# praateekmahajan/moving-mnist-vae

Measured on AMD Instinct MI355X. Metric: frames/sec/GPU VAE train step, 20×64×64 batch; ELBO vs CPU ref, higher is better.
Workload: dtype bf16; 1 GPU; BASELINE configs[1]: 256 clips x 20 frames x 64x64 per GPU per step (=5120 frames), conv-VAE z=128, Gaussian NLL sigma=0.1 + KL (normal_vae_1_kl_0_mmd), Adam, random-init weights, Bernoulli(0.0521) q=2 labels; parallelism=dp1, rccl_ranks=1, grad_exchange=none, bn=per-rank batch statistics

## Files before the change

### include/mmvae.h

```cpp
#ifndef MMVAE_H_
#define MMVAE_H_

#include <stddef.h>
#include <stdint.h>

#ifdef __cplusplus
extern "C" {
#endif

#if defined(__GNUC__)
#define MMVAE_API __attribute__((visibility("default")))
#else
#define MMVAE_API
#endif

#define MMVAE_OK 0
#define MMVAE_ERR_ARG (-1)
#define MMVAE_ERR_HIP (-2)
#define MMVAE_ERR_WORKSPACE (-3)
#define MMVAE_ERR_UNSUPPORTED (-4)

#define MMVAE_F32 0
#define MMVAE_BF16 1
#define MMVAE_FP8 2
// ... 56 lines not shown
MMVAE_API int mmvae_kl_fwd_ex(const float* mu, const float* logvar, int64_t n, double* acc, double* partials, void* stream);
MMVAE_API int mmvae_kl_bwd(const float* mu, const float* logvar, float coef, const float* gscale, float* d_mu, float* d_logvar, int64_t n,
                 void* stream);
MMVAE_API int mmvae_gauss_nll_fwd(const float* recon, const float* target, int64_t n, float sigma, double* acc, void* stream);
MMVAE_API int mmvae_gauss_nll_fwd_ex(const float* recon, const float* target, int64_t n, float sigma, double* acc, double* partials,
                                     void* stream);
MMVAE_API int mmvae_gauss_nll_bwd(const float* recon, const float* target, int64_t n, float sigma, float coef, const float* gscale,
                        float* d_recon, void* stream);
MMVAE_API int mmvae_ce_fwd(const float* recon, const int64_t* target, const float* weight, int N, int Q, int HW, double* acc, void* stream);
MMVAE_API int mmvae_ce_fwd_ex(const float* recon, const int64_t* target, const float* weight, int N, int Q, int HW, double* acc,
                              double* partials, void* stream);
MMVAE_API int mmvae_ce_bwd(const float* recon, const int64_t* target, const float* weight, int N, int Q, int HW, float coef,
                 const float* gscale, float* d_recon, void* stream);
MMVAE_API int mmvae_mmd_fwd(const float* x, const float* y, int n, int d, float* scratch, double* acc, void* stream);
MMVAE_API int mmvae_mmd_fwd_ex(const float* x, const float* y, int n, int d, float* scratch, double* acc, double* partials, void* stream);
MMVAE_API int mmvae_mmd_bwd(const float* x, const float* y, int n, int d, float coef, const float* gscale, float* d_y, void* stream);
MMVAE_API int mmvae_rbf_kernel(const float* x, const float* y, int n, int m, int d, float* out, void* stream);
MMVAE_API int mmvae_loss_finish(const double* acc, float* out, float nll, float kl_coef, float mmd_coef, float n, void* stream);

MMVAE_API int mmvae_normalise_labels(const int64_t* labels, int64_t n, float mean, float stdv, float* image, void* stream);
MMVAE_API int mmvae_quantise_normalise(const uint8_t* frames, int64_t n, const float* centres, int q, float mean, float stdv,
                             int64_t* labels, float* image, void* stream);
MMVAE_API int mmvae_adam_step(float* params, const float* grads, float* exp_avg, float* exp_avg_sq, int64_t n, float lr, float beta1,
                    float beta2, float eps, float weight_decay, float bc1, float bc2_sqrt, float grad_scale, void* stream);

MMVAE_API int mmvae_adam_step_dev(float* params, const float* grads, float* exp_avg, float* exp_avg_sq, int64_t n, float lr, float beta1,
                        float beta2, float eps, float weight_decay, double* step_dev, float grad_scale, void* stream);

MMVAE_API int mmvae_conv2d_fwd(int dtype, int transposed, const void* x, const float* weight, void* y, int N, int H, int W, int Cin, int Cout,
                     int k, int stride, int pad, const float* pro_scale, const float* pro_shift, int pro_relu, float* stats,
                     void* scratch, void* stream);
MMVAE_API int mmvae_conv2d_dgrad(int dtype, int transposed, const void* dy, const float* weight, void* dx, int N, int H, int W, int Cin,
                       int Cout, int k, int stride, int pad, void* scratch, void* stream);
#define MMVAE_WGRAD_SCRATCH_BYTES (64u << 20)
MMVAE_API int mmvae_conv2d_wgrad(int dtype, int transposed, const void* x, const void* dy, float* dweight, int N, int H, int W, int Cin,
                       int Cout, int k, int stride, int pad, const float* pro_scale, const float* pro_shift, int pro_relu,
                       void* scratch, void* stream);
MMVAE_API int mmvae_conv2d_wgrad_pair(int dtype, const void* x, const void* dy, const void* dy_shortcut, float* dweight, float* dweight_sc, int N,
                            int H, int W, int Cin, int Cout, const float* pro_scale, const float* pro_shift, int pro_relu, void* scratch,
                            void* stream);
#define MMVAE_BN_SCRATCH_BYTES (16u << 20)
MMVAE_API int mmvae_batchnorm_fwd(int dtype, const void* y, int64_t npix, int C, const float* gamma, const float* beta, float* running_mean,
                        float* running_var, int64_t* nbt, float momentum, float eps, int relu, void* out, float* save_mean, float* save_istd,
                        void* scratch, void* stream);
MMVAE_API int mmvae_batchnorm_bwd(int dtype, const void* dout, const void* y, const void* out, int64_t npix, int C, const float* gamma,
                        const float* save_mean, const float* save_istd, void* dy, float* dgamma, float* dbeta, void* scratch, void* stream);
MMVAE_API int mmvae_stem_fwd(int dtype, const void* x, const float* weight, void* y, int N, int S, float* stats, void* scratch, void* stream);
MMVAE_API int mmvae_stem_bwd(int dtype, const void* g, const void* y0, const void* x, const float* weight, const float* gamma,
                   const float* bn_scale, const float* bn_shift, const float* save_mean, const float* save_istd, float* dweight,
                   float* dgamma, float* dbeta, int N, int S, void* scratch, void* stream);
MMVAE_API int mmvae_convT_bwd_fused(int dtype, const void* x, const void* dy, const float* weight, float* dweight, void* dx, int N, int H, int W,
                          int Cin, int Cout, int k, int stride, int pad, const float* pro_scale, const float* pro_shift, int pro_relu,
                          const void* x2, const float* w2, float* dw2, void* scratch, void* wscratch, void* stream);
MMVAE_API int mmvae_tail_join_fwd(int dtype, const void* y2, const float* s2, const float* b2, const void* ys, const float* ss, const float* bs,
                        const float* weight, const float* bias, float* r_raw, float* stats, int N, int H, int W, void* stream);
MMVAE_API int mmvae_tail_join_fwd_stream(int dtype, const void* y2, const float* s2, const float* b2, const void* ys, const float* ss, const float* bs,
                               const float* weight, const float* bias, float* r_raw, float* stats, int N, int H, int W, void* stream);
MMVAE_API int mmvae_tail_join_bwd_reduce(int dtype, const float* d_raw, const float* weight, int out_planes, const void* y2, const float* s2,
                               const float* b2, const void* ys, const float* ss, const float* bs, float* partials, float* wpartials,
                               int N, int H, int W, void* stream);
MMVAE_API int mmvae_tail_join_bwd_apply(int dtype, const float* d_raw, const float* weight, int out_planes, const void* y2, const float* s2,
                              const float* b2, const void* ys, const float* ss, const float* bs, const float* A2, const float* B2,
                              const float* C2, const float* As, const float* Bs, const float* Cs, void* dy2, void* dys, int N, int H, int W,
                              void* stream);
MMVAE_API int mmvae_upblock_bwd_fused(const float* d_raw, const float* tail_weight, const void* y2, const float* s2, const float* b2,
                            const void* ys, const float* ss, const float* bs, const float* A2, const float* B2, const float* C2,
// ... 33 lines not shown
```

### moving-mnist-vae_amd/_lib.py

```python
from __future__ import annotations

import ctypes
import os
from ctypes import POINTER, c_char_p, c_double, c_float, c_int, c_int32, c_int64, c_size_t, c_void_p

_HERE = os.path.dirname(os.path.abspath(__file__))
LIB_PATH = os.environ.get("MMVAE_LIB_PATH") or os.path.join(_HERE, "libmmvae_hip.so")
_lib = None
ABI_VERSION = 3
SUM_PARTIALS = 1025

P = c_void_p

PROTOTYPES = {
    "mmvae_abi_version": (c_int, []),
    "mmvae_last_error": (c_char_p, []),
    "mmvae_net_create": (c_int, [POINTER(c_void_p), c_int, c_int, c_int, c_int, c_int, c_int]),
    "mmvae_net_create_ex": (c_int, [POINTER(c_void_p), c_int, c_int, c_int, c_int, c_int, c_int, c_int]),
    "mmvae_net_destroy": (None, [P]),
    "mmvae_net_sizes": (c_int, [P, POINTER(c_int64), POINTER(c_int64), POINTER(c_int32), POINTER(c_int64), POINTER(c_int32)]),
    "mmvae_net_num_entries": (c_int, [P]),
    "mmvae_net_entry": (c_int, [P, c_int, c_char_p, c_int, POINTER(c_int32), POINTER(c_int32), POINTER(c_int32), POINTER(c_int64)]),
    "mmvae_net_workspace_bytes": (c_size_t, [P, c_int]),
    "mmvae_encoder_fwd": (c_int, [P, c_int, P, P, P, P, P, c_size_t, P, P, c_int, P]),
    "mmvae_net_stage_labels": (c_int, [P, c_int, P, c_int, c_float, c_float, P, P, c_size_t, P]),
    "mmvae_encoder_fwd_staged": (c_int, [P, c_int, P, P, P, P, P, c_size_t, P, P, c_int, P]),
    "mmvae_encoder_bwd": (c_int, [P, c_int, P, P, P, P, P, c_size_t, P]),
    "mmvae_decoder_fwd": (c_int, [P, c_int, P, P, P, P, P, c_size_t, P, c_int, P]),
    "mmvae_decoder_bwd": (c_int, [P, c_int, P, P, P, P, c_size_t, P, P]),
    "mmvae_decoder_bwd_gauss": (c_int, [P, c_int, P, c_float, c_float, P, P, P, P, c_size_t, P, P]),
    "mmvae_net_defer_join": (c_int, [P, c_int]),
    "mmvae_net_join": (c_int, [P, P]),
    "mmvae_net_fork": (P, [P, P]),
    "mmvae_net_side_stream": (P, [P]),
    "mmvae_net_set_join_grad": (c_int, [P, c_int]),
    "mmvae_net_set_sync_bn": (c_int, [P, P, P, c_int]),
    "mmvae_rsample_fwd": (c_int, [P, P, P, P, c_int64, P]),
    "mmvae_rsample_bwd": (c_int, [P, P, P, P, P, c_int64, P]),
    "mmvae_kl_fwd": (c_int, [P, P, c_int64, P, P]),
    "mmvae_kl_fwd_ex": (c_int, [P, P, c_int64, P, P, P]),
    "mmvae_kl_bwd": (c_int, [P, P, c_float, P, P, P, c_int64, P]),
    "mmvae_gauss_nll_fwd": (c_int, [P, P, c_int64, c_float, P, P]),
    "mmvae_gauss_nll_fwd_ex": (c_int, [P, P, c_int64, c_float, P, P, P]),
    "mmvae_gauss_nll_bwd": (c_int, [P, P, c_int64, c_float, c_float, P, P, P]),
    "mmvae_ce_fwd": (c_int, [P, P, P, c_int, c_int, c_int, P, P]),
    "mmvae_ce_fwd_ex": (c_int, [P, P, P, c_int, c_int, c_int, P, P, P]),
    "mmvae_ce_bwd": (c_int, [P, P, P, c_int, c_int, c_int, c_float, P, P, P]),
    "mmvae_mmd_fwd": (c_int, [P, P, c_int, c_int, P, P, P]),
    "mmvae_mmd_fwd_ex": (c_int, [P, P, c_int, c_int, P, P, P, P]),
    "mmvae_mmd_bwd": (c_int, [P, P, c_int, c_int, c_float, P, P, P]),
    "mmvae_loss_finish": (c_int, [P, P, c_float, c_float, c_float, c_float, P]),
    "mmvae_normalise_labels": (c_int, [P, c_int64, c_float, c_float, P, P]),
    "mmvae_quantise_normalise": (c_int, [P, c_int64, P, c_int, c_float, c_float, P, P, P]),
    "mmvae_adam_step": (c_int, [P, P, P, P, c_int64, c_float, c_float, c_float, c_float, c_float, c_float, c_float, c_float, P]),
    "mmvae_adam_step_dev": (c_int, [P, P, P, P, c_int64, c_float, c_float, c_float, c_float, c_float, P, c_float, P]),
    "mmvae_conv2d_fwd": (c_int, [c_int, c_int, P, P, P, c_int, c_int, c_int, c_int, c_int, c_int, c_int, c_int, P, P, c_int, P, P, P]),
    "mmvae_conv2d_dgrad": (c_int, [c_int, c_int, P, P, P, c_int, c_int, c_int, c_int, c_int, c_int, c_int, c_int, P, P]),
    "mmvae_conv2d_wgrad": (c_int, [c_int, c_int, P, P, P, c_int, c_int, c_int, c_int, c_int, c_int, c_int, c_int, P, P, c_int, P, P]),
    "mmvae_conv2d_wgrad_pair": (c_int, [c_int, P, P, P, P, P, c_int, c_int, c_int, c_int, c_int, P, P, c_int, P, P]),
    "mmvae_rbf_kernel": (c_int, [P, P, c_int, c_int, c_int, P, P]),
    "mmvae_comm_unique_id": (c_int, [P]),
    "mmvae_comm_init": (c_int, [POINTER(c_void_p), c_int, c_int, P]),
    "mmvae_comm_allreduce": (c_int, [P, P, c_int64, P]),
    "mmvae_comm_destroy": (c_int, [P]),
    "mmvae_net_set_sync_bn_comm": (c_int, [P, P]),
    "mmvae_net_set_sync_bn_comm2": (c_int, [P, P, P]),
    "mmvae_convT_bwd_fused": (c_int, [c_int, P, P, P, P, P, c_int, c_int, c_int, c_int, c_int, c_int, c_int, c_int, P, P, c_int, P, P, P, P, P, P]),
    "mmvae_batchnorm_fwd": (c_int, [c_int, P, c_int64, c_int, P, P, P, P, P, c_float, c_float, c_int, P, P, P, P, P]),
    "mmvae_batchnorm_bwd": (c_int, [c_int, P, P, P, c_int64, c_int, P, P, P, P, P, P, P, P]),
    "mmvae_stem_fwd": (c_int, [c_int, P, P, P, c_int, c_int, P, P, P]),
    "mmvae_stem_bwd": (c_int, [c_int, P, P, P, P, P, P, P, P, P, P, P, P, c_int, c_int, P, P]),
    "mmvae_tail_join_fwd": (c_int, [c_int, P, P, P, P, P, P, P, P, P, P, c_int, c_int, c_int, P]),
    "mmvae_tail_join_fwd_stream": (c_int, [c_int, P, P, P, P, P, P, P, P, P, P, c_int, c_int, c_int, P]),
    "mmvae_tail_join_bwd_reduce": (c_int, [c_int, P, P, c_int, P, P, P, P, P, P, P, P, c_int, c_int, c_int, P]),
    "mmvae_tail_join_bwd_apply": (c_int, [c_int, P, P, c_int, P, P, P, P, P, P, P, P, P, P, P, P, P, P, c_int, c_int, c_int, P]),
    "mmvae_upblock_bwd_fused": (c_int, [P] * 27 + [c_int, P, P]),
    "mmvae_join_conv1x1_fwd": (c_int, [P, P, P, P, P, P, P, c_int, P, P, P, c_int64, P, P]),
    "mmvae_conv1x1_bwd_fused": (c_int, [P] * 13 + [c_int64, P, P]),
    "mmvae_upblock_tail_fwd": (c_int, [P] * 16 + [c_int, P, P]),
    "mmvae_pixelcnn_create": (c_int, [POINTER(c_void_p), c_int, c_int, c_int, c_int, c_int]),
    "mmvae_pixelcnn_destroy": (None, [P]),
    "mmvae_pixelcnn_num_params": (c_int64, [P]),
    "mmvae_pixelcnn_workspace_bytes": (c_size_t, [P, c_int, c_int]),
    "mmvae_pixelcnn_fwd": (c_int, [P, c_int, c_int, P, P, P, c_size_t, P, P]),
    "mmvae_pixelcnn_bwd": (c_int, [P, c_int, c_int, P, P, P, P, P, c_size_t, P, P]),
    "mmvae_pixelcnn_sample_workspace_bytes": (c_size_t, [P, c_int, c_int]),
    "mmvae_pixelcnn_sample": (c_int, [P, c_int, c_int, P, c_int, P, c_int, P, c_float, c_float, P, P, c_size_t, P, P, P, P]),
    "mmvae_convert": (c_int, [c_int, c_int, P, P, c_int64, P]),
}

# ... 52 lines not shown
```

### moving-mnist-vae_amd/csrc/capi.cpp

```cpp
#include <cstring>
#include <new>

#include "../../include/mmvae.h"
#include "conv_ops.hpp"
#include "pixel_net.hpp"
#include "vae_net.hpp"

namespace mmvae { const char* last_error(); }
using namespace mmvae;

struct mmvae_net { Net* net; };
struct mmvae_comm { Comm* c; };

static inline hipStream_t S(void* s) { return static_cast<hipStream_t>(s); }
static inline hipStream_t S_(void* s) { return static_cast<hipStream_t>(s); }

extern "C" {

int mmvae_abi_version(void) { return MMVAE_ABI_VERSION; }
const char* mmvae_last_error(void) { return last_error(); }

int mmvae_net_create(mmvae_net** out, int in_channels, int z, int out_channels, int image_size, int need_logvar, int dtype) {
  return mmvae_net_create_ex(out, in_channels, z, out_channels, image_size, need_logvar, dtype, 1);
}
// ... 290 lines not shown
    q.wfrag = op_deep2_down_ok(dt, g, H, W);
    if (w) { int rc = op_pack_down(dt, g, w, scratch, S(st), 1.f, 0, q.wfrag); if (rc < 0) return rc; }
    return op_run_down(dt, dt, g, scratch, N, x, H, W, y, Ho, Wo, ps, pb, relu, stats, 0, S(st), q);
  }
  if (convT4_stream_ok(dt, Cin, Cout, k, s, p, H, W)) {
    if (w) { int rc = op_pack_up(dt, g, w, scratch, S(st)); if (rc < 0) return rc; }
    return launch_convT4_stream(dt, x, scratch, y, ps, pb, relu, stats, N, H, S(st));
  }
  q.wfrag = op_deep2_up_ok(dt, g, Ho, Wo);
  if (w) { int rc = op_pack_up(dt, g, w, scratch, S(st), 1.f, 0, q.wfrag); if (rc < 0) return rc; }
  return op_run_up(dt, g, scratch, N, x, H, W, y, Ho, Wo, ps, pb, relu, stats, 0, S(st), q);
}
int mmvae_conv2d_dgrad(int dt, int transposed, const void* dy, const float* w, void* dx, int N, int H, int W, int Cin, int Cout, int k,
                       int s, int p, void* scratch, void* st) {
  const ConvGeom g = geom_for(transposed, Cin, Cout, k, s, p);
  const int Ho = out_size(transposed, H, k, s, p), Wo = out_size(transposed, W, k, s, p);
  SecondSrc q;
  if (!transposed && s == 1 && conv3_stream_ok(dt, Cin, Cout, k, s, p, H, W)) {
    PackArgs pf; std::memset(&pf, 0, sizeof(pf));
    pf.src = w; pf.dst = scratch; pf.cols = Cin; pf.K = Cout; pf.ntaps = 9; pf.s_col = 9; pf.s_k = Cin * 9; pf.scale = 1.f;
    for (int t = 0; t < 9; ++t) pf.tap_off[t] = 8 - t;
    int rc = launch_pack(dt, pf, S(st)); if (rc < 0) return rc;
    rc = launch_conv3_stream(dt, 1, dy, scratch, nullptr, dx, nullptr, nullptr, nullptr, 0, nullptr, nullptr, N, H, S(st));
    return rc < 0 ? rc : MMVAE_OK;
  }
  if (!transposed) {
    q.wfrag = op_deep2_up_ok(dt, g, H, W);
    int rc = op_pack_up(dt, g, w, scratch, S(st), 1.f, 0, q.wfrag); if (rc < 0) return rc;
    return op_run_up(dt, g, scratch, N, dy, Ho, Wo, dx, H, W, nullptr, nullptr, 0, nullptr, 0, S(st), q);
  }
  q.wfrag = op_deep2_down_ok(dt, g, Ho, Wo);
  int rc = op_pack_down(dt, g, w, scratch, S(st), 1.f, 0, q.wfrag); if (rc < 0) return rc;
  return op_run_down(dt, dt, g, scratch, N, dy, Ho, Wo, dx, H, W, nullptr, nullptr, 0, nullptr, 0, S(st), q);
}
int mmvae_conv2d_wgrad(int dt, int transposed, const void* x, const void* dy, float* dw, int N, int H, int W, int Cin, int Cout, int k,
                       int s, int p, const float* ps, const float* pb, int relu, void* scratch, void* st) {
  const ConvGeom g = geom_for(transposed, Cin, Cout, k, s, p);
  const int Ho = out_size(transposed, H, k, s, p), Wo = out_size(transposed, W, k, s, p);
  if (!scratch) { set_error("conv2d_wgrad: scratch (MMVAE_WGRAD_SCRATCH_BYTES) required"); return MMVAE_ERR_ARG; }
  static_assert(MMVAE_WGRAD_SCRATCH_BYTES == kWgradScratchBytes, "public scratch size out of sync");
  float* sc = static_cast<float*>(scratch);
  if (!transposed) return op_run_wgrad(dt, g, N, dy, Ho, Wo, nullptr, nullptr, 0, x, H, W, ps, pb, relu, dw, S(st), sc);
  return op_run_wgrad(dt, g, N, x, H, W, ps, pb, relu, dy, Ho, Wo, nullptr, nullptr, 0, dw, S(st), sc);
}
int mmvae_conv2d_wgrad_pair(int dt, const void* x, const void* dy, const void* dy_sc, float* dw, float* dw_sc, int N, int H, int W, int Cin, int Cout,
                            const float* ps, const float* pb, int relu, void* scratch, void* st) {
  if (!scratch || !x || !dy || !dy_sc || !dw || !dw_sc || N < 1) { set_error("conv2d_wgrad_pair: bad argument"); return MMVAE_ERR_ARG; }
  const ConvGeom g = geom_for(0, Cin, Cout, 3, 2, 1), gs = geom_for(0, Cin, Cout, 1, 2, 0);
  const int Ho = out_size(0, H, 3, 2, 1), Wo = out_size(0, W, 3, 2, 1);
  const int rc = op_run_wgrad_pair(dt, g, gs, N, dy, dy_sc, Ho, Wo, x, H, W, ps, pb, relu, dw, dw_sc, S(st), static_cast<float*>(scratch), 1.f, 1.f);
  if (rc == 0) { set_error("conv2d_wgrad_pair: shape not supported (bf16, 32 -> 32 channels, 32x32 -> 16x16)"); return MMVAE_ERR_UNSUPPORTED; }
  return rc < 0 ? rc : MMVAE_OK;
}
int mmvae_convT_bwd_fused(int dt, const void* x, const void* dy, const float* w, float* dw, void* dx, int N, int H, int W, int Cin, int Cout, int k,
                          int s, int p, const float* ps, const float* pb, int relu, const void* x2, const float* w2, float* dw2, void* scratch,
                          void* wscratch, void* st) {
  const ConvGeom g = geom_for(1, Cin, Cout, k, s, p);
  const int Ho = out_size(1, H, k, s, p), Wo = out_size(1, W, k, s, p);
  if (!scratch || !wscratch) { set_error("convT_bwd_fused: scratch buffers required"); return MMVAE_ERR_ARG; }
  if (!op_bwd_fusable(dt, g, N, H, W, Ho, Wo)) { set_error("convT_bwd_fused: shape not supported (bf16, 16 / 32 -> 16 channels, k4 s2 p1, 32x32 -> 64x64 or 16x16 -> 32x32)"); return MMVAE_ERR_UNSUPPORTED; }
  char* sc = static_cast<char*>(scratch);
  int rc = op_pack_down(dt, g, w, sc, S(st)); if (rc < 0) return rc;
  const void* w2p = nullptr;
  if (x2 && w2) {
    PackArgs pa; std::memset(&pa, 0, sizeof(pa));
    pa.src = w2; pa.dst = sc + (size_t)Cin * Cout * k * k * dtype_size(dt); pa.cols = Cin; pa.K = 16; pa.ntaps = 1; pa.s_col = 16; pa.s_k = 1; pa.scale = 1.f; pa.tap_off[0] = 0;
// ... 163 lines not shown
```

### moving-mnist-vae_amd/csrc/conv_deep2.inc

```
#include "kernels.hpp"
#include "tile_common.hpp"

namespace mmvae {

template <typename T, typename TO, int NPT, int CPT, bool ACC, bool LITE, bool F8 = false>
__device__ __forceinline__ void deep2_conv_body(const DeepArgs& a) {
  static_assert(!F8 || (sizeof(T) == 2 && !ACC), "fp8 MFMA: bf16 storage, forward convolutions");
  constexpr int VE = Elem<T>::kVec;
  constexpr int ES = sizeof(T);
  constexpr int TPX = NPT * 16;
  constexpr int kSV = 8;
  constexpr int G = CPT < (LITE ? 2 : 4) ? CPT : (LITE ? 2 : 4);
  constexpr int NB = LITE ? 2 : NPT >= 8 ? 3 : 4;
  constexpr int UPT = CPT / G;
  extern __shared__ __attribute__((aligned(16))) char smem[];
  const int t = threadIdx.x, nthr = blockDim.x, lane = t & 63, wv = __builtin_amdgcn_readfirstlane(t >> 6), gq = lane >> 4, r = lane & 15;
  const int c0 = (blockIdx.y * a.nw + wv) * 32;
  const int cin_vecs = a.Cin / VE;
  constexpr int LES = F8 ? 1 : ES;
  const int pitch = F8 ? a.Cin + 16 : a.Cin * ES + 32;
  const int npix_in = a.ipt * a.Hi * a.Wi;
  char* sPatch = smem;
  unsigned* sOpix = reinterpret_cast<unsigned*>(sPatch + (size_t)(npix_in + 1) * pitch);
  float* sStat = reinterpret_cast<float*>(sOpix + TPX) + wv * 64;
  unsigned short* sTab = reinterpret_cast<unsigned short*>(sOpix + TPX + 64 * a.nw);
  const T* __restrict__ X = reinterpret_cast<const T*>(a.x);
  TO* __restrict__ Y = reinterpret_cast<TO*>(a.y);
  const bool has_pro = a.pro_scale != nullptr, has_bias = a.bias != nullptr, has_stats = a.stats != nullptr;
  const float relu_lo = a.pro_relu ? 0.f : -__builtin_inff();
  const int HqWq = a.Hq * a.Wq;

  const int cv = t % cin_vecs, pix0 = t / cin_vecs, PS = nthr / cin_vecs;
  for (int p = t; p < TPX; p += nthr) {
    unsigned o = ~0u;
    int img = 0, hq = 0, wq = 0;
    const bool live = p < a.ipt * HqWq;
    if (live) {
      img = p / HqWq;
      const int rem = p - img * HqWq;
      hq = rem / a.Wq; wq = rem - hq * a.Wq;
      o = ((unsigned)img << 16) | ((unsigned)hq << 8) | (unsigned)wq;
    }
    sOpix[p] = o;
    const int hb = hq * a.SI, wb = wq * a.SI, ib = img * a.Hi;
#pragma unroll
    for (int tap = 0; tap < kMaxTaps; ++tap)
      if (tap < a.ntaps_all) {
        const int hi = hb + a.taps[tap].dh, wi = wb + a.taps[tap].dw;
        const bool in = live && hi >= 0 && hi < a.Hi && wi >= 0 && wi < a.Wi;
        sTab[tap * TPX + p] = (unsigned short)(in ? (ib + hi) * a.Wi + wi : npix_in);
      }
  }
  for (int i = t; i < pitch / 16; i += nthr) reinterpret_cast<Vec16*>(sPatch + (size_t)npix_in * pitch)[i] = Vec16{{0, 0, 0, 0}};
  sStat[lane] = 0.f;

  for (int tile = blockIdx.x; tile < a.ntiles; tile += gridDim.x) {
    const int n0 = tile * a.ipt;
    const int nimg = min(a.ipt, a.N - n0);
    __syncthreads();
    {
      const T* src = X + (long)n0 * a.Hi * a.Wi * a.Cin + cv * VE;
      const int nvalid = nimg * a.Hi * a.Wi;
      float psc[VE], psh[VE];
// ... 86 lines not shown
#pragma unroll
            for (int pt = 0; pt < NPT; ++pt) bf[pt] = *reinterpret_cast<const Vec16*>(sPatch + pb[pt] + (cc0 + g) * 64);
#pragma unroll
            for (int pt = 0; pt < NPT; ++pt) {
              acc[0][pt] = mma_vec<T>(buf[g][0], bf[pt], acc[0][pt]);
              acc[1][pt] = mma_vec<T>(buf[g][1], bf[pt], acc[1][pt]);
            }
          }
        }
      };
      Vec16 buf[NB][G][2];
      unsigned pb[NPT];
#pragma unroll
      for (int b = 0; b < NB - 1; ++b) load_unit(buf[b], b);
      for (int u = 0; u < nunits; u += NB) {
#pragma unroll
        for (int b = 0; b < NB; ++b) {
          const int uu = u + b;
          load_unit(buf[(b + NB - 1) % NB], uu + NB - 1);
          __builtin_amdgcn_sched_barrier(0);
          if (uu < nunits) {
            if (UPT == 1 || (uu & (UPT - 1)) == 0) tap_pixels(pb, uu / UPT);
            mul_unit(buf[b], pb, (uu & (UPT - 1)) * G);
          }
          __builtin_amdgcn_sched_barrier(0);
        }
      }
      float bv[8], st1[8], st2[8];
#pragma unroll
      for (int j = 0; j < 8; ++j) {
        bv[j] = has_bias ? a.bias[c0 + 8 * gq + j] : 0.f;
        st1[j] = 0.f; st2[j] = 0.f;
      }
#pragma unroll
      for (int pt = 0; pt < NPT; ++pt) {
        const unsigned op = sOpix[pt * 16 + r];
        const int img = (int)(op >> 16), hq = (int)((op >> 8) & 255u), wq = (int)(op & 255u);
        if (op != ~0u && img < nimg && hq < P.Hq && wq < P.Wq) {
          const unsigned ob = ((((unsigned)(n0 + img) * a.Ho + (unsigned)(hq * a.SO + P.ph)) * a.Wo + (unsigned)(wq * a.SO + P.pw)) * (unsigned)a.Cout) +
                              (unsigned)(c0 + 8 * gq);
          float v[8];
#pragma unroll
          for (int j = 0; j < 8; ++j) v[j] = acc[j >> 2][pt][j & 3] + bv[j];
#pragma unroll
          for (int j = 0; j < 8; ++j) { st1[j] += v[j]; st2[j] += v[j] * v[j]; }
          dstore8<TO>(Y + ob, v, ACC);
        }
      }
      if (has_stats) {
#pragma unroll
        for (int j = 0; j < 8; ++j) { st1[j] = row16_sum(st1[j]); st2[j] = row16_sum(st2[j]); }
        if (r == 0) {
#pragma unroll
          for (int j = 0; j < 8; ++j) {
            sStat[8 * gq + j] += st1[j];
            sStat[32 + 8 * gq + j] += st2[j];
          }
        }
      }
    }
  }
  if (has_stats) {
    a.stats[(long)blockIdx.x * 2 * a.Cout + (long)(lane >> 5) * a.Cout + c0 + (lane & 31)] = sStat[lane];
  }
}

template <typename T, typename TO, int NPT, int CPT, bool ACC>
__global__ __launch_bounds__(512, 2) void deep2_conv_kernel(DeepArgs a) { deep2_conv_body<T, TO, NPT, CPT, ACC, false>(a); }
template <typename T, typename TO, int NPT, int CPT, bool ACC>
__global__ __launch_bounds__(512, 3) void deep2_conv_lite_kernel(DeepArgs a) { deep2_conv_body<T, TO, NPT, CPT, ACC, true>(a); }
template <typename T, typename TO, int NPT, int CPT, bool ACC>
__global__ __launch_bounds__(512, 2) void deep2_conv_f8_kernel(DeepArgs a) { deep2_conv_body<T, TO, NPT, CPT, false, false, true>(a); }
template <typename T, typename TO, int NPT, int CPT, bool ACC>
__global__ __launch_bounds__(512, 3) void deep2_conv_f8_lite_kernel(DeepArgs a) { deep2_conv_body<T, TO, NPT, CPT, false, true, true>(a); }

template <typename T, typename TO>
static int launch_deep2_t(const DeepArgs& a, int dt, int gx, hipStream_t s) {
  const size_t lds = deep2_conv_lds_bytes(a, dt);
  dim3 grid(gx, a.Cout / (32 * a.nw)), block(64 * a.nw);
#define MMVAE_D2K(K_, N_, C_, A_) do { \
    static bool attr_set = false; \
    if (!attr_set) { \
      const hipError_t e = hipFuncSetAttribute(reinterpret_cast<const void*>(&K_<T, TO, N_, C_, A_>), hipFuncAttributeMaxDynamicSharedMemorySize, 160 * 1024); \
      if (e != hipSuccess) { set_error("deep2_conv: hipFuncSetAttribute: %s", hipGetErrorString(e)); return MMVAE_ERR_HIP; } \
      attr_set = true; \
    } \
    hipLaunchKernelGGL((K_<T, TO, N_, C_, A_>), grid, block, lds, s, a); } while (0)
#define MMVAE_D2(N_, C_, A_) do { if (a.nw >= 4) MMVAE_D2K(deep2_conv_lite_kernel, N_, C_, A_); else MMVAE_D2K(deep2_conv_kernel, N_, C_, A_); } while (0)
#define MMVAE_D2C(N_, C_) do { if (a.accumulate) MMVAE_D2(N_, C_, true); else MMVAE_D2(N_, C_, false); } while (0)
#define MMVAE_D2N(N_) do { \
    constexpr int kC0 = sizeof(T) == 2 ? 1 : 2;       \
    if (cpt == kC0) MMVAE_D2C(N_, kC0); else if (cpt == 2 * kC0) MMVAE_D2C(N_, 2 * kC0); else if (cpt == 4 * kC0) MMVAE_D2C(N_, 4 * kC0); \
    else if (cpt == 8 * kC0) MMVAE_D2C(N_, 8 * kC0); \
    else { set_error("deep2_conv: Cin=%d unsupported", a.Cin); return MMVAE_ERR_UNSUPPORTED; } } while (0)
  const int cpt = 1 << a.cpt_log2;
  if (a.fp8) {
    if constexpr (sizeof(T) == 2 && sizeof(TO) == 2) {
      if (a.accumulate || !a.wfrag) { set_error("deep2_conv: fp8 needs fragment-major weights and no accumulate"); return MMVAE_ERR_UNSUPPORTED; }
#define MMVAE_D2F(N_, C_) do { if (a.nw >= 4 && N_ < 8) MMVAE_D2K(deep2_conv_f8_lite_kernel, N_, C_, false); else MMVAE_D2K(deep2_conv_f8_kernel, N_, C_, false); } while (0)
#define MMVAE_D2FN(N_) do { if (cpt == 1) MMVAE_D2F(N_, 1); else if (cpt == 2) MMVAE_D2F(N_, 2); else if (cpt == 4) MMVAE_D2F(N_, 4); \
      else { set_error("deep2_conv: fp8 Cin=%d unsupported", a.Cin); return MMVAE_ERR_UNSUPPORTED; } } while (0)
      if (a.npt == 8) MMVAE_D2FN(8); else if (a.npt == 4) MMVAE_D2FN(4); else if (a.npt == 2) MMVAE_D2FN(2);
      else { set_error("deep2_conv: npt=%d unsupported", a.npt); return MMVAE_ERR_UNSUPPORTED; }
#undef MMVAE_D2FN
#undef MMVAE_D2F
      const int rc8 = check_launch("deep2_conv_f8");
      return rc8 ? rc8 : gx;
    } else { set_error("deep2_conv: fp8 needs bf16 storage"); return MMVAE_ERR_UNSUPPORTED; }
  }
  if (a.npt == 8) MMVAE_D2N(8);
  else if (a.npt == 4) MMVAE_D2N(4);
  else if (a.npt == 2) MMVAE_D2N(2);
  else { set_error("deep2_conv: npt=%d unsupported", a.npt); return MMVAE_ERR_UNSUPPORTED; }
#undef MMVAE_D2N
#undef MMVAE_D2C
#undef MMVAE_D2
#undef MMVAE_D2K
  const int rc = check_launch("deep2_conv");
  return rc ? rc : gx;
}

// ... 10 lines not shown
```

### moving-mnist-vae_amd/csrc/conv_gemm.hip

```cpp
#include <stdlib.h>
#include <string.h>

#include <vector>

#include "kernels.hpp"

namespace mmvae {

constexpr int KV = 8;

__device__ __forceinline__ int lds_slot(int row, int kv) { return row * KV + (kv ^ ((row >> 1) & 7)); }

template <typename T> struct Mma;
template <> struct Mma<bf16_t> {
  __device__ static __forceinline__ f32x4 run(const Vec16& a, const Vec16& b, f32x4 c) {
    return __builtin_amdgcn_mfma_f32_16x16x32_bf16(__builtin_bit_cast(bf16x8, a), __builtin_bit_cast(bf16x8, b), c, 0, 0, 0);
  }
};
template <> struct Mma<float> {
  __device__ static __forceinline__ f32x4 run(const Vec16& a, const Vec16& b, f32x4 c) {
#pragma unroll
    for (int j = 0; j < 4; ++j)
      c = __builtin_amdgcn_mfma_f32_16x16x4f32(__uint_as_float(a.w[j]), __uint_as_float(b.w[j]), c, 0, 0, 0);
    return c;
// ... 327 lines not shown
  gx = 256 * occ;
  if (gx > b.g.ntiles) gx = b.g.ntiles;
  if (gx > kGatherMaxGridX) gx = kGatherMaxGridX;
  if (gx >= 8) gx &= ~7;
  b.x_bytes = a.x_planar ? 0u : (unsigned)((long)a.N * a.Hi * a.Wi * a.Cin * (long)dtype_size(dt));
  if (a.x2) {
    if (ct16 > 2) return 0;
    patch_conv_x2_carve(b, dt);
    if (occ > 2 && ct16 == 1 && slots <= 4) { occ = occ_regs - 1 > 1 ? occ_regs - 1 : 1; gx = 256 * occ; if (gx > b.g.ntiles) gx = b.g.ntiles; if (gx > kGatherMaxGridX) gx = kGatherMaxGridX; if (gx >= 8) gx &= ~7; }
  }
  return launch_patch_conv(dt, out_dt, b, gx, s);
}

static size_t deep2_lds_for(int dt, int Cin, int Cout, int hw, int HiWi, int ntaps_all, int npt, int fp8 = 0) {
  DeepArgs b; memset(&b, 0, sizeof(b));
  b.fp8 = fp8;
  b.Cin = Cin; b.Hi = HiWi; b.Wi = 1; b.ipt = npt * 16 / hw; b.npt = npt; b.ntaps_all = ntaps_all; b.nw = Cout / 32 < 8 ? Cout / 32 : 8;
  return deep2_conv_lds_bytes(b, dt);
}
bool deep2_shape_ok(int dt, int Cin, int Cout, int Hq, int Wq, int Hi, int Wi, int ntaps_all, int fp8) {
  if (fp8 && dt != DT_BF16) return false;
  const int ES = fp8 ? 1 : dt == DT_F32 ? 4 : 2;
  const int cpt = Cin * ES / 64;
  const int c0 = ES == 4 ? 2 : 1;
  if (Cin < (fp8 ? 64 : 32) || (Cin * ES) % 64 != 0 || (cpt != c0 && cpt != 2 * c0 && cpt != 4 * c0 && cpt != 8 * c0)) return false;
  if (Cout < 32 || Cout % 32 != 0 || (Cout > 256 && Cout % 256 != 0)) return false;
  if (Cin < 64 && Cout < 64) return false;
  const int hw = Hq * Wq;
  if (hw < 1 || hw > 128 || Hq > 255 || Wq > 255 || ntaps_all < 1 || ntaps_all > kMaxTaps) return false;
  const int npt_min = hw > 64 ? 8 : hw > 32 ? 4 : 2;
  if (fp8 && cpt > 4) return false;
  return deep2_lds_for(dt, Cin, Cout, hw, Hi * Wi, ntaps_all, npt_min, fp8) <= 150 * 1024;
}
static int try_deep2(int dt, int out_dt, const GatherArgs& a, hipStream_t s) {
  if (a.x_planar || a.y_planes || a.x2) return 0;
  if (a.fp8 && (!a.wfrag || a.accumulate || dt != DT_BF16 || out_dt != DT_BF16)) return 0;
  int Hq = 0, Wq = 0, ntaps_all = 0;
  for (int p = 0; p < a.nphase; ++p) {
    const Phase& ph = a.phases[p];
    if (ph.ntaps <= 0) return 0;
    Hq = ph.Hq > Hq ? ph.Hq : Hq; Wq = ph.Wq > Wq ? ph.Wq : Wq;
    ntaps_all = ph.tap0 + ph.ntaps > ntaps_all ? ph.tap0 + ph.ntaps : ntaps_all;
  }
  if (!deep2_shape_ok(dt, a.Cin, a.Cout, Hq, Wq, a.Hi, a.Wi, ntaps_all, a.fp8)) return 0;
  if ((long)a.N * a.Ho * a.Wo * a.Cout >= (1L << 32)) return 0;
  const int ES = dt == DT_F32 ? 4 : 2, VE = 16 / ES;
  const int cpt = a.Cin * (a.fp8 ? 1 : ES) / 64;
  DeepArgs b; memset(&b, 0, sizeof(b));
  b.fp8 = a.fp8;
  b.x = a.x; b.w = a.w; b.y = a.y; b.pro_scale = a.pro_scale; b.pro_shift = a.pro_shift; b.pro_relu = a.pro_relu;
  b.bias = a.bias; b.stats = a.stats; b.accumulate = a.accumulate; b.wfrag = a.wfrag;
  b.N = a.N; b.Hi = a.Hi; b.Wi = a.Wi; b.Cin = a.Cin; b.Ho = a.Ho; b.Wo = a.Wo; b.Cout = a.Cout; b.SI = a.SI; b.SO = a.SO;
  b.nphase = a.nphase; b.Hq = Hq; b.Wq = Wq; b.ntaps_all = ntaps_all;
  for (int p = 0; p < a.nphase; ++p) {
    const Phase& ph = a.phases[p];
    b.phases[p] = DeepPhase{ph.ph, ph.pw, ph.Hq, ph.Wq, ph.ntaps, ph.tap0, ph.w_off};
  }
  for (int t = 0; t < kMaxTaps; ++t) b.taps[t] = a.taps[t];
  for (b.cpt_log2 = 0; (1 << b.cpt_log2) < cpt; ++b.cpt_log2) {}
  b.nw = a.Cout / 32 < 8 ? a.Cout / 32 : 8;
  if ((64 * b.nw) % (a.Cin / VE) != 0) return 0;
  const int gy = a.Cout / (32 * b.nw);
  const int hw = Hq * Wq;
  int best = 0;
  for (int pass = 0; pass < 2 && !best; ++pass)
    for (int npt = 8; npt >= 2 && !best; npt >>= 1) {
      if (hw > npt * 16) break;
      const size_t lds = deep2_lds_for(dt, a.Cin, a.Cout, hw, a.Hi * a.Wi, ntaps_all, npt, a.fp8);
      int ipt = npt * 16 / hw; if (ipt > a.N) ipt = a.N;
      const long ntiles = (a.N + ipt - 1) / ipt;
      if (pass == 0) {
        if (lds > 80 * 1024) continue;
        if (npt > 2 && ntiles * gy * b.nw < 256 * 4) continue;
      } else if (lds > 150 * 1024) continue;
      best = npt;
    }
  if (!best) return 0;
  b.npt = best; b.ipt = best * 16 / hw;
  if (b.ipt > a.N) b.ipt = a.N;
  b.ntiles = (a.N + b.ipt - 1) / b.ipt;
  int gx = b.ntiles < kGatherMaxGridX ? b.ntiles : kGatherMaxGridX;
  return launch_deep2_conv(dt, out_dt, b, gx, s);
}

static int try_pos(int dt, int out_dt, const GatherArgs& a, hipStream_t s) {
  if (dt != DT_BF16 || out_dt != DT_BF16 || !a.wfrag || a.fp8 || a.gup == 0) return 0;
  if (a.x_planar || a.y_planes || a.x2 || a.bias || a.Hi != a.Wi || a.Ho != a.Wo || a.Cout % 32 != 0) return 0;
  const int up = a.gup == 2 ? 1 : 0;
  if (!pos_conv_takes(a.gk, a.gs, a.gp, up, a.Hi, a.Ho, a.Cin)) return 0;
  if (up && a.gs > 1 && a.gk < a.gs && !a.accumulate) return 0;
  if (a.Hi >= 8 && a.Cout < 128) return 0;
  if ((long)a.N * a.Ho * a.Wo * a.Cout >= (1L << 32)) return 0;
  PosArgs b; memset(&b, 0, sizeof(b));
  b.x = a.x; b.w = a.w; b.y = a.y; b.pro_scale = a.pro_scale; b.pro_shift = a.pro_shift; b.pro_relu = a.pro_relu;
  b.stats = a.stats; b.accumulate = a.accumulate; b.N = a.N; b.Cout = a.Cout;
  b.nw = a.Cout / 32 < 8 ? a.Cout / 32 : 8;
  if ((a.Cout / 32) % b.nw != 0 || (64 * b.nw) % (a.Cin / 8) != 0) return 0;
  return launch_pos_conv(a.gk, a.gs, a.gp, up, a.Hi, a.Ho, a.Cin, b, s);
}

static int launch_x2_separately(int dt, int out_dt, const GatherArgs& a, hipStream_t s) {
  GatherArgs b; memset(&b, 0, sizeof(b));
  int Hq = 0, Wq = 0;
  for (int p = 0; p < a.nphase; ++p) if (a.phases[p].ph == a.x2_ph && a.phases[p].pw == a.x2_pw) { Hq = a.phases[p].Hq; Wq = a.phases[p].Wq; }
  if (Hq <= 0) { set_error("gather_gemm: the second source's phase (%d,%d) is not part of the launch", a.x2_ph, a.x2_pw); return MMVAE_ERR_ARG; }
  b.x = a.x2; b.w = a.w2; b.y = a.y; b.accumulate = 1; b.wfrag = a.wfrag2;
  b.N = a.N; b.Hi = Hq; b.Wi = Wq; b.Cin = a.Cin2; b.Ho = a.Ho; b.Wo = a.Wo; b.Cout = a.Cout; b.SI = 1; b.SO = a.SO;
  b.nphase = 1; b.phases[0] = Phase{a.x2_ph, a.x2_pw, Hq, Wq, 1, 0, 0}; b.taps[0] = Tap{0, 0};
  b.gk = 1; b.gs = a.SO; b.gp = 0; b.gup = 2;
  return launch_gather_gemm(dt, out_dt, b, s);
}

int launch_gather_gemm(int dt, int out_dt, GatherArgs a, hipStream_t s) {
  const int VE = dt == DT_F32 ? 4 : 8;
  note_launch_bytes((double)a.N * ((double)a.Hi * a.Wi * (a.x_planar ? a.x_planes : a.Cin) * (a.x_planar == 1 ? 4 : dtype_size(dt)) +
                                   (double)a.Ho * a.Wo * (a.y_planes > 0 ? a.y_planes : a.Cout) * (a.y_planes > 0 ? 4 : dtype_size(out_dt)) +
                                   (a.x2 ? (double)a.phases[0].Hq * a.phases[0].Wq * a.Cin2 * dtype_size(dt) : 0.0)));
  if (a.fp8) {
    if (dt != DT_BF16 || out_dt != DT_BF16 || a.x2 || a.accumulate) { set_error("gather_gemm: fp8 needs the bf16 forward path"); return MMVAE_ERR_UNSUPPORTED; }
    a.cin_vecs = a.Cin / VE;
    const int rc2 = try_deep2(dt, out_dt, a, s);
    if (rc2 != 0) return rc2;
    if (a.wfrag) { set_error("gather_gemm: fragment-major fp8 weights (Cin=%d Cout=%d) need the deep2 kernel", a.Cin, a.Cout); return MMVAE_ERR_UNSUPPORTED; }
    set_error("gather_gemm: fp8 layer Cin=%d Cout=%d is not eligible for the deep-layer kernel", a.Cin, a.Cout); return MMVAE_ERR_UNSUPPORTED;
  }
  if (a.x2) {
    int rc = (!a.wfrag && !a.wfrag2) ? try_patch(dt, out_dt, a, s) : 0;
    if (rc != 0) return rc;
    GatherArgs m = a; m.x2 = nullptr; m.w2 = nullptr; m.Cin2 = 0; m.wfrag2 = 0;
    rc = launch_gather_gemm(dt, out_dt, m, s);
    if (rc < 0) return rc;
    const int rc2 = launch_x2_separately(dt, out_dt, a, s);
    return rc2 < 0 ? rc2 : rc;
  }
  if (a.Cin % VE != 0 || a.Cout % 4 != 0 || a.nphase < 1 || a.nphase > kMaxPhases) {
    set_error("gather_gemm: unsupported Cin=%d Cout=%d nphase=%d", a.Cin, a.Cout, a.nphase);
    return MMVAE_ERR_UNSUPPORTED;
  }
  if (a.pro_scale && a.Cin > 512) { set_error("gather_gemm: prologue needs Cin<=512"); return MMVAE_ERR_UNSUPPORTED; }
  a.cin_vecs = a.Cin / VE;
  int max_tiles = 0, ntap = 0;
  for (int p = 0; p < a.nphase; ++p) {
    const long M = (long)a.N * a.phases[p].Hq * a.phases[p].Wq;
    if (M > 0x7fffffffL / 2) { set_error("gather_gemm: too many pixels"); return MMVAE_ERR_UNSUPPORTED; }
    const int tiles = (int)((M + 127) / 128);
    if (tiles > max_tiles) max_tiles = tiles;
    ntap += a.phases[p].ntaps;
  }
  if (ntap > kMaxTaps) { set_error("gather_gemm: %d taps > %d", ntap, kMaxTaps); return MMVAE_ERR_UNSUPPORTED; }
  if (max_tiles <= 0) return 1;
  const int rcp = a.wfrag ? 0 : try_patch(dt, out_dt, a, s);
  if (rcp != 0) return rcp;
  const int rcq = try_pos(dt, out_dt, a, s);
  if (rcq != 0) return rcq;
  const int rcd2 = try_deep2(dt, out_dt, a, s);
  if (rcd2 != 0) return rcd2;
  if (a.wfrag) { set_error("gather_gemm: fragment-major weights (Cin=%d Cout=%d) need the deep2 kernel, which does not take this launch", a.Cin, a.Cout); return MMVAE_ERR_UNSUPPORTED; }
  {
    constexpr int g3_maxk = 160;
    int maxk = 0;
    for (int p = 0; p < a.nphase; ++p) if (a.phases[p].ntaps * a.Cin > maxk) maxk = a.phases[p].ntaps * a.Cin;
    const bool fits32 = (long)a.N * a.Hi * a.Wi * a.Cin < (1L << 31) && (long)a.N * a.Ho * a.Wo * a.Cout < (1L << 31);
    if (!a.x_planar && !a.y_planes && !a.bias && out_dt == dt && a.Cout <= 64 && maxk <= g3_maxk && fits32) {
      int ct16 = (a.Cout + 15) / 16; if (ct16 == 3) ct16 = 4;
      if (gather3_lds_bytes(a, dt, ct16 * 16) <= kV2MaxLds) {
        long wt = 0;
        for (int p = 0; p < a.nphase; ++p) { const long m = (long)a.N * a.phases[p].Hq * a.phases[p].Wq; if ((m + 31) / 32 > wt) wt = (m + 31) / 32; }
        long gx3 = (wt + 3) / 4; if (gx3 > 2048 / a.nphase) gx3 = 2048 / a.nphase; if (gx3 < 1) gx3 = 1;
        if (gx3 > kGatherMaxGridX) gx3 = kGatherMaxGridX;
        return launch_gather3(dt, out_dt, a, (int)gx3, s);
      }
    }
    if (a.x_planar || a.y_planes) { set_error("gather_gemm: planar boundary layouts need the patch-tile kernel"); return MMVAE_ERR_UNSUPPORTED; }
  }
  const int gx = max_tiles < kGatherMaxGridX ? max_tiles : kGatherMaxGridX;
  if (dt == DT_F32) return launch_gather_t<float, float>(a, gx, s);
  if (out_dt == DT_F32) return launch_gather_t<bf16_t, float>(a, gx, s);
  return launch_gather_t<bf16_t, bf16_t>(a, gx, s);
}

template <typename T>
__global__ __launch_bounds__(256) void wgrad_kernel(WgradArgs a) {
  constexpr int VE = Elem<T>::kVec;
  constexpr int PK = KV * VE;
  __shared__ Vec16 sP[64 * KV];
  __shared__ Vec16 sG[256 * KV];
  __shared__ int sPix[PK * 3];
  __shared__ float sProP[2 * 256];
  __shared__ float sProG[2 * 256];
// ... 364 lines not shown
```

### moving-mnist-vae_amd/csrc/conv_ops.cpp

```cpp
#include "conv_ops.hpp"

#include <cstdlib>
#include <cstring>

namespace mmvae {

#define MM_TRY(expr)            \
  do {                          \
    int rc__ = (expr);          \
    if (rc__ < 0) return rc__;  \
  } while (0)

struct UpPhase { int ph, pw; int ntaps; int kh[16], kw[16], dh[16], dw[16]; };
static int up_phases(int k, int s, int p, UpPhase* out) {
  int n = 0;
  for (int ph = 0; ph < s; ++ph)
    for (int pw = 0; pw < s; ++pw) {
      UpPhase& u = out[n++];
      u.ph = ph; u.pw = pw; u.ntaps = 0;
      for (int kh = 0; kh < k; ++kh) {
        const int th = ph + p - kh;
        if (((th % s) + s) % s != 0) continue;
        for (int kw = 0; kw < k; ++kw) {
          const int tw = pw + p - kw;
// ... 32 lines not shown
    a.cols = g.D1; a.K = g.D0; a.ntaps = ph[i].ntaps; a.s_col = kk; a.s_k = g.D1 * kk; a.scale = scale; a.fp8 = fp8; a.frag = frag;
    for (int t = 0; t < ph[i].ntaps; ++t) a.tap_off[t] = ph[i].kh[t] * g.k + ph[i].kw[t];
    MM_TRY(launch_pack(dt, a, s));
    off += (long)g.D1 * ph[i].ntaps * g.D0;
  }
  return MMVAE_OK;
}

int op_deep2_down_ok(int dt, const ConvGeom& g, int Hl, int Wl, int fp8) {
  const int Hs = conv_down_size(Hl, g.k, g.s, g.p), Ws = conv_down_size(Wl, g.k, g.s, g.p);
  return deep2_shape_ok(dt, g.D1, g.D0, Hs, Ws, Hl, Wl, g.k * g.k, fp8) ? 1 : 0;
}
int op_deep2_up_ok(int dt, const ConvGeom& g, int Hl, int Wl, int allow_empty_phases, int fp8) {
  if (g.s > 2 || g.k * g.k > kMaxTaps) return 0;
  const int Hs = conv_down_size(Hl, g.k, g.s, g.p), Ws = conv_down_size(Wl, g.k, g.s, g.p);
  UpPhase ph[4];
  const int np = up_phases(g.k, g.s, g.p, ph);
  int ntaps = 0;
  for (int i = 0; i < np; ++i) { if (ph[i].ntaps == 0 && !allow_empty_phases) return 0; ntaps += ph[i].ntaps; }
  return deep2_shape_ok(dt, g.D0, g.D1, (Hl + g.s - 1) / g.s, (Wl + g.s - 1) / g.s, Hs, Ws, ntaps, fp8) ? 1 : 0;
}
bool op_pos_fwd_takes(const ConvGeom& g, int Hl, bool transposed) {
  const int Hs = conv_down_size(Hl, g.k, g.s, g.p);
  const int Hi = transposed ? Hs : Hl, Ho = transposed ? Hl : Hs;
  const int Cin = transposed ? g.D0 : g.D1, Cout = transposed ? g.D1 : g.D0;
  if (Cout % 32 != 0 || Cin % 8 != 0 || (Hi >= 8 && Cout < 128)) return false;
  if (transposed && g.s > 1 && g.k < g.s) return false;
  const int nw = Cout / 32 < 8 ? Cout / 32 : 8;
  if ((Cout / 32) % nw != 0 || (64 * nw) % (Cin / 8) != 0) return false;
  return pos_conv_takes(g.k, g.s, g.p, transposed ? 1 : 0, Hi, Ho, Cin);
}

int op_run_down(int dt, int out_dt, const ConvGeom& g, const void* packed, int N, const void* L, int Hl, int Wl, void* S, int Hs, int Ws,
                const float* pro_s, const float* pro_b, int relu, float* stats, int accumulate, hipStream_t s, const SecondSrc& x2) {
  GatherArgs a; std::memset(&a, 0, sizeof(a));
  if (g.k * g.k > kMaxTaps) { set_error("run_down: k=%d too large", g.k); return MMVAE_ERR_UNSUPPORTED; }
  if (x2.x2) { a.x2 = x2.x2; a.w2 = x2.w2; a.Cin2 = x2.Cin2; a.x2_ph = 0; a.x2_pw = 0; }
  a.fp8 = x2.fp8; a.wfrag = x2.wfrag; a.wfrag2 = x2.wfrag2;
  a.x = L; a.w = packed; a.y = S;
  a.pro_scale = pro_s; a.pro_shift = pro_b; a.pro_relu = relu; a.stats = stats; a.accumulate = accumulate;
  a.N = N; a.Hi = Hl; a.Wi = Wl; a.Cin = g.D1; a.Ho = Hs; a.Wo = Ws; a.Cout = g.D0; a.SI = g.s; a.SO = 1;
  a.gk = g.k; a.gs = g.s; a.gp = g.p; a.gup = 1;
  a.nphase = 1;
  a.phases[0] = Phase{0, 0, Hs, Ws, g.k * g.k, 0, 0};
  for (int kh = 0; kh < g.k; ++kh)
    for (int kw = 0; kw < g.k; ++kw) a.taps[kh * g.k + kw] = Tap{kh - g.p, kw - g.p};
  return launch_gather_gemm(dt, out_dt, a, s);
}

int op_run_up(int dt, const ConvGeom& g, const void* packed, int N, const void* S, int Hs, int Ws, void* L, int Hl, int Wl,
              const float* pro_s, const float* pro_b, int relu, float* stats, int accumulate, hipStream_t s, const SecondSrc& x2) {
  if (g.s > 2 || g.k * g.k > kMaxTaps) { set_error("run_up: k=%d s=%d unsupported", g.k, g.s); return MMVAE_ERR_UNSUPPORTED; }
  GatherArgs a; std::memset(&a, 0, sizeof(a));
  if (x2.x2) { a.x2 = x2.x2; a.w2 = x2.w2; a.Cin2 = x2.Cin2; a.x2_ph = 0; a.x2_pw = 0; }
  a.fp8 = x2.fp8; a.wfrag = x2.wfrag; a.wfrag2 = x2.wfrag2;
  a.x = S; a.w = packed; a.y = L;
  a.pro_scale = pro_s; a.pro_shift = pro_b; a.pro_relu = relu; a.stats = stats; a.accumulate = accumulate;
  a.N = N; a.Hi = Hs; a.Wi = Ws; a.Cin = g.D0; a.Ho = Hl; a.Wo = Wl; a.Cout = g.D1; a.SI = 1; a.SO = g.s;
  a.gk = g.k; a.gs = g.s; a.gp = g.p; a.gup = 2;
  UpPhase ph[4];
  const int np = up_phases(g.k, g.s, g.p, ph);
  long off = 0; int tap0 = 0; a.nphase = 0;
  for (int i = 0; i < np; ++i) {
    const int Hq = Hl > ph[i].ph ? (Hl - ph[i].ph + g.s - 1) / g.s : 0;
    const int Wq = Wl > ph[i].pw ? (Wl - ph[i].pw + g.s - 1) / g.s : 0;
    const bool skip = (ph[i].ntaps == 0 && accumulate) || Hq == 0 || Wq == 0;
    if (!skip) {
      a.phases[a.nphase++] = Phase{ph[i].ph, ph[i].pw, Hq, Wq, ph[i].ntaps, tap0, off};
      for (int t = 0; t < ph[i].ntaps; ++t) a.taps[tap0 + t] = Tap{ph[i].dh[t], ph[i].dw[t]};
      tap0 += ph[i].ntaps;
    }
    off += (long)g.D1 * ph[i].ntaps * g.D0;
  }
  if (a.nphase == 0) return 1;
  return launch_gather_gemm(dt, dt, a, s);
}

int op_run_wgrad(int dt, const ConvGeom& g, int N, const void* P, int Hs, int Ws, const float* proP_s, const float* proP_b, int proP_relu,
                 const void* G, int Hl, int Wl, const float* proG_s, const float* proG_b, int proG_relu, float* dW, hipStream_t s,
                 float* scratch, float scale, WgradReduceArgs* defer) {
  WgradArgs a; std::memset(&a, 0, sizeof(a));
  const int kk = g.k * g.k;
  if (kk > 25) { set_error("wgrad: k=%d too large", g.k); return MMVAE_ERR_UNSUPPORTED; }
  if (defer) defer->nparts = 0;
  a.P = P; a.G = G; a.dW = dW; a.scratch = scratch; a.defer = defer;
  a.proP_scale = proP_s; a.proP_shift = proP_b; a.proP_relu = proP_relu;
  a.proG_scale = proG_s; a.proG_shift = proG_b; a.proG_relu = proG_relu;
  a.N = N; a.Hp = Hs; a.Wp = Ws; a.Ca = g.D0; a.Hg = Hl; a.Wg = Wl; a.Cb = g.D1; a.Cb_valid = g.D1;
  a.stride = g.s; a.pad = g.p; a.ksz = g.k; a.sA = g.D1 * kk; a.sB = kk; a.ntaps = kk; a.scale = scale;
  for (int t = 0; t < kk; ++t) a.tap_off[t] = t;
  return launch_wgrad(dt, a, s);
}

static void wgrad_args(WgradArgs& a, const ConvGeom& g, int N, const void* P, int Hs, int Ws, const float* proP_s, const float* proP_b, int proP_relu,
                       const void* G, int Hl, int Wl, const float* proG_s, const float* proG_b, int proG_relu, float* dW, float* scratch, float scale) {
  std::memset(&a, 0, sizeof(a));
  const int kk = g.k * g.k;
  a.P = P; a.G = G; a.dW = dW; a.scratch = scratch;
  a.proP_scale = proP_s; a.proP_shift = proP_b; a.proP_relu = proP_relu;
  a.proG_scale = proG_s; a.proG_shift = proG_b; a.proG_relu = proG_relu;
  a.N = N; a.Hp = Hs; a.Wp = Ws; a.Ca = g.D0; a.Hg = Hl; a.Wg = Wl; a.Cb = g.D1; a.Cb_valid = g.D1; a.Ca_valid = g.D0;
  a.stride = g.s; a.pad = g.p; a.ksz = g.k; a.sA = g.D1 * kk; a.sB = kk; a.ntaps = kk; a.scale = scale;
  for (int t = 0; t < kk && t < 25; ++t) a.tap_off[t] = t;
}

int op_run_wgrad_pair(int dt, const ConvGeom& g, const ConvGeom& gs, int N, const void* P, const void* P2, int Hs, int Ws, const void* G, int Hl, int Wl,
                      const float* proG_s, const float* proG_b, int proG_relu, float* dW, float* dW2, hipStream_t s, float* scratch, float scale,
                      float scale2) {
// ... 43 lines not shown
```

### moving-mnist-vae_amd/csrc/conv_ops.hpp

```cpp
#pragma once
#include "kernels.hpp"

namespace mmvae {

struct ConvGeom { int D0, D1, k, s, p; };

inline int conv_down_size(int H, int k, int s, int p) { return (H + 2 * p - k) / s + 1; }
int op_pack_down(int dt, const ConvGeom& g, const float* w, void* dst, hipStream_t s, float scale = 1.f, int fp8 = 0, int frag = 0);
int op_pack_up(int dt, const ConvGeom& g, const float* w, void* dst, hipStream_t s, float scale = 1.f, int fp8 = 0, int frag = 0);
int op_deep2_down_ok(int dt, const ConvGeom& g, int Hl, int Wl, int fp8 = 0);
int op_deep2_up_ok(int dt, const ConvGeom& g, int Hl, int Wl, int allow_empty_phases = 0, int fp8 = 0);
struct SecondSrc {
  const void* x2 = nullptr; const void* w2 = nullptr; int Cin2 = 0;
  int fp8 = 0;
  int wfrag = 0, wfrag2 = 0;
};
int op_run_down(int dt, int out_dt, const ConvGeom& g, const void* packed, int N, const void* L, int Hl, int Wl, void* S, int Hs, int Ws,
                const float* pro_s, const float* pro_b, int relu, float* stats, int accumulate, hipStream_t s, const SecondSrc& x2 = SecondSrc());
int op_run_up(int dt, const ConvGeom& g, const void* packed, int N, const void* S, int Hs, int Ws, void* L, int Hl, int Wl,
              const float* pro_s, const float* pro_b, int relu, float* stats, int accumulate, hipStream_t s, const SecondSrc& x2 = SecondSrc());
int op_run_wgrad(int dt, const ConvGeom& g, int N, const void* P, int Hs, int Ws, const float* proP_s, const float* proP_b, int proP_relu,
                 const void* G, int Hl, int Wl, const float* proG_s, const float* proG_b, int proG_relu, float* dW, hipStream_t s,
                 float* scratch = nullptr, float scale = 1.f, WgradReduceArgs* defer = nullptr);
bool op_wgrad_is_stream(int dt, const ConvGeom& g, int N, int Hs, int Ws, int Hl, int Wl, bool proP, bool proG);
int op_run_wgrad_pair(int dt, const ConvGeom& g, const ConvGeom& gs, int N, const void* P, const void* P2, int Hs, int Ws, const void* G, int Hl, int Wl,
                      const float* proG_s, const float* proG_b, int proG_relu, float* dW, float* dW2, hipStream_t s, float* scratch, float scale,
                      float scale2);

bool op_pos_fwd_takes(const ConvGeom& g, int Hl, bool transposed);
bool op_bwd_fusable(int dt, const ConvGeom& g, int N, int Hs, int Ws, int Hl, int Wl);
int op_run_bwd_fused(int dt, const ConvGeom& g, int N, const void* P, int Hs, int Ws, const float* proP_s, const float* proP_b, int proP_relu,
                     const void* G, int Hl, int Wl, const void* packed_down, void* dP, const void* x2, const void* w2_packed, float* dW,
                     hipStream_t s, float* scratch, float scale = 1.f, float* bn_part = nullptr, float* dW2 = nullptr, float scale2 = 1.f,
                     const JoinGrad* jg = nullptr);
bool op_bwd_fusable_jg(int dt, const ConvGeom& g, int N, int Hs, int Ws, int Hl, int Wl, bool proP, bool has_x2, bool bn_sums);

}
```

### moving-mnist-vae_amd/csrc/conv_pos.inc

```
#include <type_traits>
#include <utility>

#include "kernels.hpp"
#include "tile_common.hpp"

namespace mmvae {

template <int I0, int I1, typename F>
__device__ __forceinline__ void static_for(F&& f) {
  if constexpr (I0 < I1) {
    f(std::integral_constant<int, I0>{});
    static_for<I0 + 1, I1>(f);
  }
}

template <int K, int S, int P, bool UP>
struct PosTaps {
  static constexpr bool hit(int ph, int k) { return !UP || (((ph + P - k) % S) + S) % S == 0; }
  static constexpr int count(int ph) { int n = 0; for (int k = 0; k < K; ++k) if (hit(ph, k)) ++n; return n; }
  static constexpr int kth(int ph, int i) { int n = 0; for (int k = 0; k < K; ++k) if (hit(ph, k)) { if (n == i) return k; ++n; } return -1; }
  static constexpr int delta(int ph, int k) { return UP ? (ph + P - k) / S : k - P; }
  static constexpr int taps_before(int pi) { int n = 0; for (int q = 0; q < pi; ++q) n += count(q / (UP ? S : 1)) * count(q % (UP ? S : 1)); return n; }
};

// ... 1 lines not shown
template <int K, int S, int P, bool UP, int HI, int HO, int CIN, int IG, int PI>
struct PosPlan {
  using TP = PosTaps<K, S, P, UP>;
  static constexpr int NPH1 = UP ? S : 1, ph = PI / NPH1, pw = PI % NPH1;
  static constexpr int HQ = UP ? HO / S : HO, NPOS = HQ * HQ, NCF = NPOS * IG, CPT = CIN / 32;
  static constexpr int SI = UP ? 1 : S;
  static constexpr int NTH = TP::count(ph), NTW = TP::count(pw), NT = NTH * NTW, NU = NT * CPT;
  static constexpr int pix(int tap, int pos) {
    const int kh = TP::kth(ph, tap / NTW), kw = TP::kth(pw, tap % NTW);
    const int hi = (pos / HQ) * SI + TP::delta(ph, kh), wi = (pos % HQ) * SI + TP::delta(pw, kw);
    return (hi >= 0 && hi < HI && wi >= 0 && wi < HI) ? hi * HI + wi : -1;
  }
  static constexpr int count_items() {
    int n = 0;
    for (int tap = 0; tap < NT; ++tap) for (int pos = 0; pos < NPOS; ++pos) if (pix(tap, pos) >= 0) n += IG * CPT;
    return n;
  }
  static constexpr int W = count_items();
  struct Tab { PosItem it[W > 0 ? W : 1]; };
  static constexpr Tab make() {
    Tab t{};
    int n = 0;
    for (int u = 0; u < NU; ++u)
      for (int cf = 0; cf < NCF; ++cf) {
        const int px = pix(u / CPT, cf / IG);
        if (px >= 0) { t.it[n].u = (short)u; t.it[n].cf = (short)cf; t.it[n].off = px * CIN * 2 + (u % CPT) * 64; ++n; }
      }
    return t;
  }
  static constexpr Tab tab = make();
  static constexpr int first_of(int u) { for (int w = 0; w < W; ++w) if (tab.it[w].u >= u) return w; return W; }
};

template <int K, int S, int P, bool UP, int HI, int HO, int CIN, int IG, int NB, int RB>
__global__ __launch_bounds__(512, 2) void pos_conv_kernel(PosArgs a) {
  using TP = PosTaps<K, S, P, UP>;
  constexpr int NPH1 = UP ? S : 1;
  constexpr int HQ = UP ? HO / S : HO;
  constexpr int NPOS = HQ * HQ, NCF = NPOS * IG, CPT = CIN / 32, IPT = 16 * IG;
  constexpr int SO = UP ? S : 1;
  constexpr int IMGB = HI * HI * CIN * 2, IP = IMGB + 32;
  constexpr int CV = CIN / 8, VPI = HI * HI * CV;
  static_assert(NCF <= 16 && CIN % 32 == 0 && (UP ? HO % S == 0 : true), "pos_conv: geometry");
  static_assert(IMGB < 65536, "pos_conv: ds_read immediate range");
  extern __shared__ __attribute__((aligned(16))) char smem[];
  const int t = threadIdx.x, nthr = blockDim.x, lane = t & 63, wv = __builtin_amdgcn_readfirstlane(t >> 6), gq = lane >> 4, r = lane & 15;
  const int nw = nthr >> 6;
  const int c0 = (blockIdx.y * nw + wv) * 32;
  char* sPatch = smem;
  float* sStat = reinterpret_cast<float*>(smem + IPT * IP) + wv * 64;
  const bf16_t* __restrict__ X = reinterpret_cast<const bf16_t*>(a.x);
  bf16_t* __restrict__ Y = reinterpret_cast<bf16_t*>(a.y);
  const bool has_pro = a.pro_scale != nullptr, has_stats = a.stats != nullptr, accum = a.accumulate != 0;
  const float relu_lo = a.pro_relu ? 0.f : -__builtin_inff();
  const char* lb[IG];
#pragma unroll
  for (int ig = 0; ig < IG; ++ig) lb[ig] = sPatch + (ig * 16 + r) * IP + gq * 16;
  sStat[lane] = 0.f;

  for (int tile = blockIdx.x; tile < a.ntiles; tile += gridDim.x) {
    const int n0 = tile * IPT;
    const int nimg = min(IPT, a.N - n0);
    __syncthreads();
    {
      const int cv = t % CV;
      float psc[8], psh[8];
#pragma unroll
      for (int j = 0; j < 8; j += 4) {
        const float4 sc = has_pro ? *reinterpret_cast<const float4*>(a.pro_scale + cv * 8 + j) : make_float4(1.f, 1.f, 1.f, 1.f);
        const float4 sh = has_pro ? *reinterpret_cast<const float4*>(a.pro_shift + cv * 8 + j) : make_float4(0.f, 0.f, 0.f, 0.f);
        psc[j] = sc.x; psc[j + 1] = sc.y; psc[j + 2] = sc.z; psc[j + 3] = sc.w;
        psh[j] = sh.x; psh[j + 1] = sh.y; psh[j + 2] = sh.z; psh[j + 3] = sh.w;
      }
      const Vec16* src = reinterpret_cast<const Vec16*>(X + (long)n0 * (HI * HI * CIN));
      const int nvalid = nimg * VPI;
      constexpr int kSV = 8;
      for (int v0 = t; v0 < IPT * VPI; v0 += kSV * nthr) {
        Vec16 q[kSV];
#pragma unroll
        for (int k = 0; k < kSV; ++k) {
          const int v = v0 + k * nthr;
          q[k] = Vec16{{0, 0, 0, 0}};
          if (v < nvalid) q[k] = src[v];
        }
#pragma unroll
        for (int k = 0; k < kSV; ++k) {
// ... 30 lines not shown
#pragma unroll
        for (int m = 0; m < 2; ++m)
#pragma unroll
          for (int cf = 0; cf < NCF; ++cf) acc[m][cf] = (f32x4){0, 0, 0, 0};
        using PL = PosPlan<K, S, P, UP, HI, HO, CIN, IG, pi>;
        constexpr int W = PL::W;
        Vec16 abuf[NB][2];
        Vec16 bbuf[RB];
        static_for<0, (NB - 1 < NU ? NB - 1 : NU)>([&](auto U) {
          constexpr int u = decltype(U)::value;
          load_a(abuf[u % NB], u);
        });
        static_for<0, (RB - 1 < W ? RB - 1 : W)>([&](auto I) {
          constexpr int w = decltype(I)::value;
          bbuf[w % RB] = *reinterpret_cast<const Vec16*>(lb[PL::tab.it[w].cf % IG] + PL::tab.it[w].off);
        });
        static_for<0, NU>([&](auto U) {
          constexpr int u = decltype(U)::value;
          constexpr int w0 = PL::first_of(u), w1 = PL::first_of(u + 1);
          if constexpr (u + NB - 1 < NU) load_a(abuf[(u + NB - 1) % NB], u + NB - 1);
          __builtin_amdgcn_sched_barrier(0);
          static_for<w0, w1>([&](auto I) {
            constexpr int w = decltype(I)::value, cf = PL::tab.it[w].cf;
            if constexpr (w + RB - 1 < W)
              bbuf[(w + RB - 1) % RB] = *reinterpret_cast<const Vec16*>(lb[PL::tab.it[w + RB - 1].cf % IG] + PL::tab.it[w + RB - 1].off);
            acc[0][cf] = mma_bf16(abuf[u % NB][0], bbuf[w % RB], acc[0][cf]);
            acc[1][cf] = mma_bf16(abuf[u % NB][1], bbuf[w % RB], acc[1][cf]);
            __builtin_amdgcn_sched_barrier(0);
          });
        });
        float st1[8], st2[8];
#pragma unroll
        for (int j = 0; j < 8; ++j) { st1[j] = 0.f; st2[j] = 0.f; }
        static_for<0, NCF>([&](auto CF) {
          constexpr int cf = decltype(CF)::value, pos = cf / IG, ig = cf % IG;
          constexpr int ho = (pos / HQ) * SO + ph, wo = (pos % HQ) * SO + pw;
          if (ig * 16 + r < nimg) {
            const unsigned ob = ((unsigned)(n0 + ig * 16 + r) * (HO * HO) + (unsigned)(ho * HO + wo)) * (unsigned)a.Cout + (unsigned)(c0 + 8 * gq);
            float v[8];
#pragma unroll
            for (int j = 0; j < 8; ++j) v[j] = acc[j >> 2][cf][j & 3];
#pragma unroll
            for (int j = 0; j < 8; ++j) { st1[j] += v[j]; st2[j] += v[j] * v[j]; }
            dstore8<bf16_t>(Y + ob, v, accum);
          }
        });
        if (has_stats) {
#pragma unroll
          for (int j = 0; j < 8; ++j) { st1[j] = row16_sum(st1[j]); st2[j] = row16_sum(st2[j]); }
          if (r == 0) {
#pragma unroll
            for (int j = 0; j < 8; ++j) {
              sStat[8 * gq + j] += st1[j];
              sStat[32 + 8 * gq + j] += st2[j];
            }
          }
        }
      }
    });
  }
  if (has_stats) a.stats[(long)blockIdx.x * 2 * a.Cout + (long)(lane >> 5) * a.Cout + c0 + (lane & 31)] = sStat[lane];
}

#ifndef POS_NB16
#define POS_NB16 4
#endif
#ifndef POS_NB8
#define POS_NB8 4
#endif
#ifndef POS_RB16
#define POS_RB16 6
#endif
#ifndef POS_RB8
#define POS_RB8 6
#endif
template <int K, int S, int P, bool UP, int HI, int HO, int CIN, int IG>
static int pos_launch(const PosArgs& a, hipStream_t s) {
  constexpr int IP = HI * HI * CIN * 2 + 32;
  constexpr int HQ = UP ? HO / S : HO, NCF = HQ * HQ * IG;
  constexpr int NB = NCF > 8 ? POS_NB16 : POS_NB8, RB = NCF > 8 ? POS_RB16 : POS_RB8;
  auto* kern = &pos_conv_kernel<K, S, P, UP, HI, HO, CIN, IG, NB, RB>;
  const size_t lds = (size_t)16 * IG * IP + (size_t)a.nw * 256;
  static bool attr_set = false;
  if (!attr_set) {
    const hipError_t e = hipFuncSetAttribute(reinterpret_cast<const void*>(kern), hipFuncAttributeMaxDynamicSharedMemorySize, 160 * 1024);
    if (e != hipSuccess) { set_error("pos_conv: hipFuncSetAttribute: %s", hipGetErrorString(e)); return MMVAE_ERR_HIP; }
    attr_set = true;
  }
  if (lds > 160 * 1024 || (64 * a.nw) % (CIN / 8) != 0) { set_error("pos_conv: tile does not fit (lds %zu, nw %d)", lds, a.nw); return MMVAE_ERR_UNSUPPORTED; }
  const int ntiles = (a.N + 16 * IG - 1) / (16 * IG);
  PosArgs b = a; b.ntiles = ntiles;
  const int gx = ntiles < kGatherMaxGridX ? ntiles : kGatherMaxGridX;
  dim3 grid(gx, a.Cout / (32 * a.nw)), block(64 * a.nw);
  hipLaunchKernelGGL(kern, grid, block, lds, s, b);
  const int rc = check_launch("pos_conv");
  return rc ? rc : gx;
}

}
```

### moving-mnist-vae_amd/csrc/kernels.hpp

```cpp
#pragma once
#include "common.hpp"

namespace mmvae {

enum DType : int { DT_F32 = 0, DT_BF16 = 1 };
inline size_t dtype_size(int dt) { return dt == DT_F32 ? 4 : 2; }

struct Tap { int dh, dw; };
constexpr int kMaxTaps = 25;
constexpr int kMaxPhases = 4;
struct Phase { int ph, pw, Hq, Wq, ntaps, tap0; long w_off;  };
struct GatherArgs {
  const void* x; const void* w; void* y;
  const float* pro_scale; const float* pro_shift; int pro_relu;
  const float* bias;
  float* stats;
  int accumulate;
  int N, Hi, Wi, Cin, Ho, Wo, Cout;
  int SI, SO;
  int nphase; Phase phases[kMaxPhases]; Tap taps[kMaxTaps];
  int cin_vecs;
  int x_planar, x_planes;
  int y_planes;
  const void* x2; const void* w2; int Cin2, x2_ph, x2_pw;
  int fp8;
  int wfrag, wfrag2;
  int gk, gs, gp, gup;
};
bool deep2_shape_ok(int dt, int Cin, int Cout, int Hq, int Wq, int Hi, int Wi, int ntaps_all, int fp8 = 0);
int launch_gather_gemm(int dt, int out_dt, GatherArgs a, hipStream_t s);
constexpr int kGatherMaxGridX = 1024;

struct WgradArgs {
  const void* P; const void* G; float* dW;
  const float* proP_scale; const float* proP_shift; int proP_relu;
  const float* proG_scale; const float* proG_shift; int proG_relu;
  int N, Hp, Wp, Ca, Hg, Wg, Cb;
  int Cb_valid;
  int Ca_valid;
  int P_planar, P_planes;
  float* scratch;
  int stride, pad, ksz;
  int sA, sB; int ntaps; int tap_off[25];
  float scale;
  int M, pix_per_block;
  int TA16, TB16, TG;
  struct WgradReduceArgs* defer;
};
int launch_wgrad(int dt, WgradArgs a, hipStream_t s);
int try_wgrad_pos(int dt, const WgradArgs& a, hipStream_t s);
bool wgrad_stream_shape(int dt, const WgradArgs& a);
int try_wgrad_stream(int dt, const WgradArgs& a, hipStream_t s);
int try_wgrad_stream_pair(int dt, const WgradArgs& a, const void* P2, float* dW2, float scale2, hipStream_t s);
bool dgrad_wgrad_stream_shape(int dt, const WgradArgs& a);
struct JoinGrad { const void* y; const float* A; const float* B; const float* C; };
bool dgrad_wgrad_stream_jg_shape(int dt, const WgradArgs& a, bool has_x2, bool bn_sums);
int try_dgrad_wgrad_stream(int dt, const WgradArgs& a, const void* wd, void* dx, const void* x2, const void* w2, float* bn_part, hipStream_t s,
                           float* dW2 = nullptr, float scale2 = 1.f, const JoinGrad* jg = nullptr);

struct JoinBwdLaunch {
  const float* d_raw; const float* w_tail; const void* y2; const void* ys;
  const float* ms2; const float* mb2; const float* mss; const float* mbs;
  const float* A2; const float* B2; const float* C2; const float* As; const float* Bs; const float* Cs;
// ... 41 lines not shown
struct PatchPhase { int ph, pw, Hq, Wq, ntaps, tap0; long w_off; int w_vec0, koff0; };
struct PatchArgs {
  const void* x; const void* w; void* y;
  const float* pro_scale; const float* pro_shift; int pro_relu;
  const float* bias; float* stats; int accumulate;
  int Cin, Cout, Ho, Wo, SO;
  TileGeom g;
  int nphase; PatchPhase phases[kMaxPhases]; Tap taps[kMaxTaps];
  int w_vecs, koff_total;
  int x_planar, x_planes, y_planes;
  int npt, wq_shift;
  int uni, out_wave_bytes;
  int phase_of[4];
  unsigned x_bytes;
  const void* x2; const void* w2; int Cin2, x2_phase, kvp2, w2_vec0, x2_vec0, x2_slots; unsigned x2_bytes;
};
size_t patch_conv_lds_bytes(const PatchArgs& a, int dt);
void patch_conv_x2_carve(PatchArgs& a, int dt);
int patch_conv_slots(const PatchArgs& a, int dt);
int launch_patch_conv(int dt, int out_dt, const PatchArgs& a, int gx, hipStream_t s);
struct DeepPhase { int ph, pw, Hq, Wq, ntaps, tap0; long w_off; };
struct DeepArgs {
  const void* x; const void* w; void* y;
  const float* pro_scale; const float* pro_shift; int pro_relu;
  const float* bias; float* stats; int accumulate;
  int N, Hi, Wi, Cin, Ho, Wo, Cout, SI, SO;
  int Hq, Wq;
  int nphase; DeepPhase phases[kMaxPhases]; Tap taps[kMaxTaps]; int ntaps_all;
  int ipt, ntiles;
  int ct16, npt;
  int fp8;
  int nw, cpt_log2;
  int wfrag;
};
size_t deep2_conv_lds_bytes(const DeepArgs& a, int dt);
int launch_deep2_conv(int dt, int out_dt, const DeepArgs& a, int gx, hipStream_t s);
struct PosArgs {
  const void* x; const void* w; void* y;
  const float* pro_scale; const float* pro_shift; int pro_relu;
  float* stats; int accumulate;
  int N, Cout;
  int nw;
  int ntiles;
};
int launch_pos_conv(int K, int S, int P, int up, int HI, int HO, int CIN, const PosArgs& a, hipStream_t s);
bool pos_conv_takes(int K, int S, int P, int up, int HI, int HO, int CIN);

struct PackArgs {
  const float* src; void* dst; int cols, K, ntaps; int s_col, s_k; int tap_off[kMaxTaps]; float scale;
  int cols_valid, K_valid;
  int fp8;
  int frag;
};
int launch_pack(int dt, const PackArgs& a, hipStream_t s);
void pack_batch_begin();
int pack_batch_flush(int dt, hipStream_t s);

int launch_stem_im2col(int dt, const void* x, void* col, int N, int H, int W, int Ho, int Wo, hipStream_t s);

bool stem_bwd_fusable(int S);
bool conv3_stream_ok(int dt, int Cin, int Cout, int k, int s, int p, int Hin, int Win);
int launch_conv3_stream_bwd(int dt, const void* dy, const void* w_flipped, void* dx, const void* ym, const float* ms, const float* mb, float* sums,
                            int N, int H, hipStream_t s);
int launch_conv3_stream(int dt, int stride, const void* x, const void* w, const void* wsc, void* y, void* ysc, const float* pro_scale,
                        const float* pro_shift, int pro_relu, float* stats, float* stats_sc, int N, int Ho, hipStream_t s);
bool convT4_stream_ok(int dt, int Cin, int Cout, int k, int s, int p, int Hin, int Win);
int launch_convT4_stream(int dt, const void* x, const void* w_up, void* y, const float* pro_scale, const float* pro_shift, int pro_relu, float* stats,
                         int N, int Hin, hipStream_t s, int f8out = 0);
bool tail_fwd_stream_ok(int dt, int OC, int H, int W);
int launch_tail_fwd_stream(int dt, const void* y2, const float* s2, const float* b2, const void* ys, const float* ss, const float* bs, const float* w,
                           const float* bias, float* r_raw, float* stats, int N, int H, int W, hipStream_t s, int f8in = 0);
bool up5_tail_fwd_ok(int dt, int OC, int C, int Cin, int Hin, int Hout);
int launch_up5_tail_fwd(const void* y1, const float* p1s, const float* p1b, const void* w2_up, const void* xin, const float* pxs, const float* pxb,
                        const void* wu_up, const float* s2, const float* b2, const float* ss, const float* bs, const float* w, const float* bias,
                        float* r_raw, float* stats, int N, hipStream_t s);
bool stem_fwd_stream_ok(int dt, int S);
// ... 114 lines not shown
```

### moving-mnist-vae_amd/csrc/tile_common.hpp

```cpp
#pragma once
#include "kernels.hpp"

namespace mmvae {

typedef __attribute__((ext_vector_type(4))) short s16x4;

__device__ __forceinline__ f32x4 mma_bf16(const Vec16& a, const Vec16& b, f32x4 c) {
  return __builtin_amdgcn_mfma_f32_16x16x32_bf16(__builtin_bit_cast(bf16x8, a), __builtin_bit_cast(bf16x8, b), c, 0, 0, 0);
}
__device__ __forceinline__ f32x4 mma_f32v(const Vec16& a, const Vec16& b, f32x4 c) {
#pragma unroll
  for (int j = 0; j < 4; ++j)
    c = __builtin_amdgcn_mfma_f32_16x16x4f32(__uint_as_float(a.w[j]), __uint_as_float(b.w[j]), c, 0, 0, 0);
  return c;
}
template <typename T> __device__ __forceinline__ f32x4 mma_vec(const Vec16& a, const Vec16& b, f32x4 c);
template <> __device__ __forceinline__ f32x4 mma_vec<bf16_t>(const Vec16& a, const Vec16& b, f32x4 c) { return mma_bf16(a, b, c); }
template <> __device__ __forceinline__ f32x4 mma_vec<float>(const Vec16& a, const Vec16& b, f32x4 c) { return mma_f32v(a, b, c); }

template <typename TO> __device__ __forceinline__ void dstore4(TO* p, const float* v, bool acc);
template <> __device__ __forceinline__ void dstore4<float>(float* p, const float* v, bool acc) {
  float4 o = make_float4(v[0], v[1], v[2], v[3]);
  if (acc) { const float4 e = *reinterpret_cast<const float4*>(p); o.x += e.x; o.y += e.y; o.z += e.z; o.w += e.w; }
  *reinterpret_cast<float4*>(p) = o;
// ... 26 lines not shown
__device__ __forceinline__ uint32_t pack4_fp8(float f0, float f1, float f2, float f3) {
  uint32_t o = 0;
  o = __builtin_amdgcn_cvt_pk_fp8_f32(fminf(fmaxf(f0, -448.f), 448.f), fminf(fmaxf(f1, -448.f), 448.f), o, false);
  o = __builtin_amdgcn_cvt_pk_fp8_f32(fminf(fmaxf(f2, -448.f), 448.f), fminf(fmaxf(f3, -448.f), 448.f), o, true);
  return o;
}
__device__ __forceinline__ void unpack4_fp8(uint32_t v, float* f) {
  const auto lo = __builtin_amdgcn_cvt_pk_f32_fp8(v, false), hi = __builtin_amdgcn_cvt_pk_f32_fp8(v, true);
  f[0] = lo[0]; f[1] = lo[1]; f[2] = hi[0]; f[3] = hi[1];
}
__device__ __forceinline__ void unpack4_bf16(uint2 v, float* f) {
  f[0] = __uint_as_float(v.x << 16); f[1] = __uint_as_float(v.x & 0xffff0000u); f[2] = __uint_as_float(v.y << 16); f[3] = __uint_as_float(v.y & 0xffff0000u);
}

template <typename TO> __device__ __forceinline__ void dstore8(TO* p, const float* v, bool acc);
template <> __device__ __forceinline__ void dstore8<float>(float* p, const float* v, bool acc) {
  dstore4<float>(p, v, acc);
  dstore4<float>(p + 4, v + 4, acc);
}
template <> __device__ __forceinline__ void dstore8<bf16_t>(bf16_t* p, const float* v, bool acc) {
  float f[8];
#pragma unroll
  for (int j = 0; j < 8; ++j) f[j] = v[j];
  if (acc) {
    const uint4 e = *reinterpret_cast<const uint4*>(p);
    const unsigned w[4] = {e.x, e.y, e.z, e.w};
#pragma unroll
    for (int j = 0; j < 4; ++j) { f[2 * j] += __uint_as_float(w[j] << 16); f[2 * j + 1] += __uint_as_float(w[j] & 0xffff0000u); }
  }
  uint4 o;
  o.x = pack2_bf16(f[0], f[1]); o.y = pack2_bf16(f[2], f[3]); o.z = pack2_bf16(f[4], f[5]); o.w = pack2_bf16(f[6], f[7]);
  *reinterpret_cast<uint4*>(p) = o;
}
__device__ __forceinline__ float row16_sum(float v) {
  v += __builtin_bit_cast(float, __builtin_amdgcn_mov_dpp(__builtin_bit_cast(int, v), 0x128, 0xf, 0xf, true));
  v += __builtin_bit_cast(float, __builtin_amdgcn_mov_dpp(__builtin_bit_cast(int, v), 0x124, 0xf, 0xf, true));
  v += __builtin_bit_cast(float, __builtin_amdgcn_mov_dpp(__builtin_bit_cast(int, v), 0x4e, 0xf, 0xf, true));
  v += __builtin_bit_cast(float, __builtin_amdgcn_mov_dpp(__builtin_bit_cast(int, v), 0xb1, 0xf, 0xf, true));
  return v;
}
template <typename T> struct FragOps;
template <> struct FragOps<bf16_t> {
  __device__ static __forceinline__ Vec16 load(const char* base, int off0, int off1) {
    const s16x4 lo = __builtin_amdgcn_ds_read_tr16_b64_v4i16((__attribute__((address_space(3))) s16x4*)(base + off0));
    const s16x4 hi = __builtin_amdgcn_ds_read_tr16_b64_v4i16((__attribute__((address_space(3))) s16x4*)(base + off1));
    Vec16 v;
    v.w[0] = (uint32_t)(uint16_t)lo[0] | ((uint32_t)(uint16_t)lo[1] << 16);
    v.w[1] = (uint32_t)(uint16_t)lo[2] | ((uint32_t)(uint16_t)lo[3] << 16);
    v.w[2] = (uint32_t)(uint16_t)hi[0] | ((uint32_t)(uint16_t)hi[1] << 16);
    v.w[3] = (uint32_t)(uint16_t)hi[2] | ((uint32_t)(uint16_t)hi[3] << 16);
    return v;
  }
};

__device__ __forceinline__ void tile_origin(const TileGeom& g, int tile, int seg, int& n, int& hq0) {
  if (g.tiles_per_img > 0) {
    n = tile / g.tiles_per_img;
    hq0 = (tile - n * g.tiles_per_img) * g.qr;
  } else {
    n = tile * g.segs + seg;
    hq0 = 0;
  }
}

__device__ __forceinline__ int patch_index(const TileGeom& g, int p) {
  const int per_seg = g.qr * g.Wq;
// ... 16 lines not shown
```

### moving-mnist-vae_amd/csrc/vae_net.cpp

```cpp
#include "vae_net.hpp"

#include <algorithm>
#include <cmath>
#include <cstdlib>
#include <cstring>

#include "conv_ops.hpp"

namespace mmvae {

#define MM_TRY(expr)            \
  do {                          \
    int rc__ = (expr);          \
    if (rc__ < 0) return rc__;  \
  } while (0)

static inline long align_up(long v, long a) { return (v + a - 1) / a * a; }
static inline int down_size(int H, int k, int s, int p) { return conv_down_size(H, k, s, p); }

void Net::add_entry(const std::string& name, std::initializer_list<int> shape, int kind, long off) {
  Entry e; e.name = name; e.ndim = (int)shape.size(); e.kind = kind; e.offset = off;
  int i = 0; for (int d : shape) e.shape[i++] = d;
  for (; i < 4; ++i) e.shape[i] = 1;
  entries.push_back(e);
// ... 173 lines not shown
  P.wscratch = take((long)kWgradScratchBytes);
  P.wscratch2 = take(2L * 1024 * 4096 * 4);
  P.stem_R = take(1024 * 8);
  P.stem_gram = take(1024L * stem_bwd_part_floats() * 4);
  P.bytes = (size_t)cur;
  plan_ = P;
  return plan_;
}

int Net::fill_consts(char* base, hipStream_t s) {
  float* c = reinterpret_cast<float*>(base + plan_.cvec);
  MM_TRY(launch_fill_f32(c, 1.f, 256, s));
  return launch_fill_f32(c + 256, 0.f, 256, s);
}

float* Net::bnf(const Bn& bn, char* base, int which) const {
  return reinterpret_cast<float*>(base + plan_.bnws) + bn.ws + (long)which * align_up(bn.C, 4);
}

static inline ConvGeom geom(const ConvW& w) { return ConvGeom{w.D0, w.D1, w.k, w.s, w.p}; }

int Net::frag_down(const ConvW& w) const { return w.Hl > 0 ? op_deep2_down_ok(dt(), geom(w), w.Hl, w.Hl, (w.fp8 && !w.tr) ? 1 : 0) : 0; }
int Net::frag_up(const ConvW& w) const { return w.Hl > 0 ? op_deep2_up_ok(dt(), geom(w), w.Hl, w.Hl, 1, (w.fp8 && w.tr) ? 1 : 0) : 0; }
int Net::pack_down(const ConvW& w, const float* params, char* base, hipStream_t s) {
  return op_pack_down(dt(), geom(w), params + w.off, base + plan_.packed + w.packD * (long)esz(), s, w.wscale, (w.fp8 && !w.tr) ? 1 : 0,
                      frag_down(w));
}
int Net::pack_up(const ConvW& w, const float* params, char* base, hipStream_t s) {
  return op_pack_up(dt(), geom(w), params + w.off, base + plan_.packed + w.packU * (long)esz(), s, w.wscale, (w.fp8 && w.tr) ? 1 : 0,
                    frag_up(w));
}
int Net::run_down(const ConvW& w, char* base, int N, const void* L, int Hl, int Wl, void* S, int Hs, int Ws,
                  const float* pro_s, const float* pro_b, int relu, float* stats, int accumulate, int out_dt, hipStream_t s,
                  const ConvW* w2, const void* x2) {
  SecondSrc q;
  if (w2) { q.x2 = x2; q.w2 = base + plan_.packed + w2->packU * (long)esz(); q.Cin2 = w2->D0; }
  q.fp8 = (w.fp8 && !w.tr) ? 1 : 0;
  q.wfrag = frag_down(w); q.wfrag2 = w2 ? frag_up(*w2) : 0;
  return op_run_down(dt(), out_dt, geom(w), base + plan_.packed + w.packD * (long)esz(), N, L, Hl, Wl, S, Hs, Ws, pro_s, pro_b, relu,
                     stats, accumulate, s, q);
}
int Net::run_up(const ConvW& w, char* base, int N, const void* S, int Hs, int Ws, void* L, int Hl, int Wl,
                const float* pro_s, const float* pro_b, int relu, float* stats, int accumulate, hipStream_t s,
                const ConvW* w2, const void* x2) {
  SecondSrc q;
  if (w2) { q.x2 = x2; q.w2 = base + plan_.packed + w2->packU * (long)esz(); q.Cin2 = w2->D0; }
  q.fp8 = (w.fp8 && w.tr) ? 1 : 0;
  q.wfrag = frag_up(w); q.wfrag2 = w2 ? frag_up(*w2) : 0;
  return op_run_up(dt(), geom(w), base + plan_.packed + w.packU * (long)esz(), N, S, Hs, Ws, L, Hl, Wl, pro_s, pro_b, relu, stats,
                   accumulate, s, q);
}
hipStream_t Net::wgrad_stream(hipStream_t s) {
  if (side_state_ == 0) {
    side_state_ = 1;
    bool ok = hipStreamCreateWithFlags(&side_, hipStreamNonBlocking) == hipSuccess;
    for (int i = 0; i < kForkEvents && ok; ++i) ok = hipEventCreateWithFlags(&ev_[i], hipEventDisableTiming) == hipSuccess;
    for (int i = 0; i < 16 && ok; ++i) ok = hipEventCreateWithFlags(&blk_ev_[i], hipEventDisableTiming) == hipSuccess;
    if (ok) ok = hipEventCreateWithFlags(&gram_ev_, hipEventDisableTiming) == hipSuccess;
    if (!ok) { (void)hipGetLastError(); side_state_ = -1; }
  }
  return side_state_ == 1 ? side_ : s;
}
int Net::side_fork(hipStream_t s) {
  if (wgrad_stream(s) == s) return MMVAE_OK;
  hipEvent_t e = ev_[evi_++ % kForkEvents];
  bool ok = hipEventRecord(e, s) == hipSuccess && hipStreamWaitEvent(side_, e, 0) == hipSuccess;
  if (!ok) { set_error("side stream fork failed"); return MMVAE_ERR_HIP; }
  return MMVAE_OK;
}
int Net::side_join(hipStream_t s) {
  if (wgrad_stream(s) == s) return MMVAE_OK;
  hipEvent_t e = ev_[evi_++ % kForkEvents];
  bool ok = hipEventRecord(e, side_) == hipSuccess && hipStreamWaitEvent(s, e, 0) == hipSuccess;
  if (!ok) { set_error("side stream join failed"); return MMVAE_ERR_HIP; }
  return MMVAE_OK;
}

bool Net::stem_bwd_fused() const {
  return cfg.in_ch == 1 && stem_bwd_fusable(cfg.S);
}

int Net::side_mark(int slot) {
  if (side_state_ != 1) return MMVAE_OK;
// ... 69 lines not shown
  auto add = [&](const Bn& bn, float in_scale) {
    BnFoldEntry e;
    e.g_off = (int)bn.g_off; e.b_off = (int)bn.b_off; e.rm_off = (int)bn.rm_off; e.rv_off = (int)bn.rv_off;
    e.scale_off = (int)(bn.ws + 2L * align_up(bn.C, 4)); e.shift_off = (int)(bn.ws + 3L * align_up(bn.C, 4)); e.C = bn.C; e.in_scale = in_scale;
    tab.push_back(e);
  };
  if (which == 0) add(bn0, 1.f); else add(dbn0, dstem.wscale);
  for (const Block& B : which == 0 ? enc : dec) {
    add(B.b1, B.c1.wscale); add(B.b2, B.c2.wscale);
    if (!B.identity) add(B.bs, B.cs.wscale);
  }
  if (which == 1) add(bn_out, 1.f);
  MM_TRY(launch_bn_fold_eval(tab.data(), (int)tab.size(), params, bnbuf, reinterpret_cast<float*>(base + plan_.bnws), 1e-5f, s));
  eval_folded_ = true;
  return MMVAE_OK;
}

int Net::bn_eval(const Bn&, const float*, const float*, char*, hipStream_t, float) {
  if (eval_folded_) return MMVAE_OK;
  set_error("bn_eval: the entry point did not fold its BatchNorms"); return MMVAE_ERR_ARG;
}

BnBwdFinalizeArgs Net::bwd_finalize_args(const Bn& bn, const float* params, float* grads, char* base, const float* partials, int nparts, int ny,
                                         int which, double count) const {
  const Net& net = *this;
  BnBwdFinalizeArgs a;
  a.partials = partials; a.nparts = nparts; a.C = bn.C; a.which = which; a.ny = ny;
  a.count = count; a.gamma = params + bn.g_off; a.mean = net.bnf(bn, base, 0); a.istd = net.bnf(bn, base, 1);
  a.dgamma = grads + bn.g_off; a.dbeta = grads + bn.b_off;
  a.coefA = net.bnf(bn, base, 4); a.coefB = net.bnf(bn, base, 5); a.coefC = net.bnf(bn, base, 6);
  return a;
}
int Net::bn_backward_coefs(const Bn& bn, const float* params, float* grads, char* base, int nparts, int ny, int which, double count,
                           hipStream_t s, float* dbias_conv) {
  const float* part = reinterpret_cast<const float*>(base + plan_.partials);
  BnBwdFinalizeArgs l = bwd_finalize_args(bn, params, grads, base, part, nparts, ny, which, count);
  if (!sync_bn_on()) l.dbias_conv = dbias_conv;
  MM_TRY(launch_bn_bwd_finalize(l, s));
  if (!sync_bn_on()) return MMVAE_OK;
  float* row = nullptr;
  MM_TRY(sync_rows(base, part, nparts, (1 + ny) * bn.C, s, &row));
  BnBwdFinalizeArgs g = bwd_finalize_args(bn, params, grads, base, row, 1, ny, which, count * ar_world_);
  g.dgamma = nullptr; g.dbeta = nullptr;
  g.dbias_conv = dbias_conv; g.dbias_scale = 1.f / (float)ar_world_;
  return launch_bn_bwd_finalize(g, s);
}
int Net::bn_backward_coefs_join(const Bn& b2, const Bn& bs, const float* params, float* grads, char* base, int nparts, double count,
                                hipStream_t s) {
  const float* part = reinterpret_cast<const float*>(base + plan_.partials);
  MM_TRY(launch_bn_bwd_finalize2(bwd_finalize_args(b2, params, grads, base, part, nparts, 2, 0, count),
                                 bwd_finalize_args(bs, params, grads, base, part, nparts, 2, 1, count), s));
  if (!sync_bn_on()) return MMVAE_OK;
  float* row = nullptr;
  MM_TRY(sync_rows(base, part, nparts, 3 * b2.C, s, &row));
  BnBwdFinalizeArgs g2 = bwd_finalize_args(b2, params, grads, base, row, 1, 2, 0, count * ar_world_);
  BnBwdFinalizeArgs gs = bwd_finalize_args(bs, params, grads, base, row, 1, 2, 1, count * ar_world_);
  g2.dgamma = g2.dbeta = gs.dgamma = gs.dbeta = nullptr;
  return launch_bn_bwd_finalize2(g2, gs, s);
}

int Net::packs_enc_fwd(const float* params, char* base, hipStream_t s) {
  const Plan& P = plan_;
  {
    const int cpad = dt() == DT_F32 ? 4 : 8;
    PackArgs pa; std::memset(&pa, 0, sizeof(pa));
    pa.src = params + stem.off; pa.dst = base + P.packed + stem_pack * (long)esz();
    pa.cols = 32; pa.K = cpad; pa.K_valid = cfg.in_ch; pa.ntaps = 25; pa.s_col = 25 * cfg.in_ch; pa.s_k = 25; pa.scale = 1.f;
    for (int t = 0; t < 25; ++t) pa.tap_off[t] = t;
    MM_TRY(launch_pack(dt(), pa, s));
  }
  for (const Block& B : enc) {
    MM_TRY(pack_down(B.c1, params, base, s));
    MM_TRY(pack_down(B.c2, params, base, s));
    if (!B.identity) MM_TRY(pack_down(B.cs, params, base, s));
  }
  const int nt = Hf * Wf;
  for (int h = 0; h < (cfg.need_logvar ? 2 : 1); ++h) {
    const ConvW& hw = h == 0 ? head_mu : head_lv;
    const long poff = h == 0 ? head_pack_mu : head_pack_lv;
    PackArgs pa; std::memset(&pa, 0, sizeof(pa));
    pa.src = params + hw.off; pa.dst = base + P.packed + poff * (long)esz();
    pa.cols = cfg.z; pa.K = 256; pa.ntaps = nt; pa.s_col = 256; pa.s_k = 1; pa.scale = 1.0f / nt;
// ... 170 lines not shown
  const int Ch = cfg.need_logvar ? 2 * cfg.z : cfg.z;
  const int nt = Hf * Wf;
  pack_batch_begin();
  MM_TRY(packs_enc_bwd(params, base, s));
  MM_TRY(pack_batch_flush(dt(), s));
  MM_TRY(launch_concat2_to_t(dt(), d_mu, cfg.need_logvar ? d_logvar : nullptr, N, cfg.z, cfg.need_logvar ? cfg.z : 0, base + P.dh, s));
  {
    WgradArgs a; std::memset(&a, 0, sizeof(a));
    a.P = base + P.dh; a.G = base + enc.back().out; a.dW = grads + head_mu.off; a.proP_relu = a.proG_relu = 0;
    a.N = N; a.Hp = 1; a.Wp = 1; a.Ca = Ch; a.Hg = Hf; a.Wg = Wf; a.Cb = 256; a.Cb_valid = 256;
    a.stride = Hf; a.pad = 0; a.ksz = Hf; a.sA = 256; a.sB = 1; a.ntaps = nt; a.scale = 1.0f / nt;
    a.scratch = wscratch_;
    MM_TRY(side_fork(s));
    MM_TRY(launch_wgrad(dt(), a, wgrad_stream(s)));
    if (stem_bwd_fused() && !(gram_ready_ && gram_fwd_N_ == N && gram_fwd_ws_ == ws)) {
      MM_TRY(launch_stem_gram(dt(), base + P.x_t, reinterpret_cast<float*>(base + P.stem_gram), 1024L * stem_bwd_part_floats(),
                              reinterpret_cast<double*>(base + P.stem_R), N, cfg.S, H1, W1, wgrad_stream(s)));
      if (side_state_ == 1 && hipEventRecord(gram_ev_, side_) != hipSuccess) { set_error("side stream mark failed"); return MMVAE_ERR_HIP; }
    }
    gram_ready_ = false;
    if (!stem_bwd_fused() && cfg.in_ch == 1 && wgrad_stream(s) != s) MM_TRY(launch_stem_im2col(dt(), base + P.x_t, base + P.col, N, cfg.S, cfg.S, H1, W1, wgrad_stream(s)));
    PackArgs pa; std::memset(&pa, 0, sizeof(pa));
    pa.src = params + head_mu.off; pa.dst = base + P.packed + head_pack_dg * (long)esz();
    pa.cols = 256; pa.K = Ch; pa.ntaps = 1; pa.s_col = 1; pa.s_k = 256; pa.scale = 1.0f / nt;
    GatherArgs g; std::memset(&g, 0, sizeof(g));
    g.x = base + P.dh; g.w = pa.dst; g.y = base + P.g[0];
    g.N = N; g.Hi = 1; g.Wi = 1; g.Cin = Ch; g.Ho = Hf; g.Wo = Wf; g.Cout = 256; g.SI = 1; g.SO = Hf;
    g.nphase = nt;
    for (int i = 0; i < nt; ++i) { g.phases[i] = Phase{i / Wf, i % Wf, 1, 1, 1, i, 0}; g.taps[i] = Tap{0, 0}; }
    MM_TRY(launch_gather_gemm(dt(), dt(), g, s));
  }
  int cur = 0;
  const int ne = (int)enc.size();
  for (int i = ne - 1; i >= 0; --i) {
    Block& B = enc[i];
    const long npix = (long)N * B.Hout * B.Wout;
    const double cnt = (double)npix;
    const void* xin = i == 0 ? base + P.y0 : base + enc[i - 1].out;
    const float* xs = i == 0 ? bnf(bn0, base, 2) : nullptr;
    const float* xb = i == 0 ? bnf(bn0, base, 3) : nullptr;
    const int ds = i & 1;
    const bool priv = i >= ne - 2;
    const long dy1o = priv ? P.edy1[i - (ne - 2)] : P.dy1[ds], dy2o = priv ? P.edy2[i - (ne - 2)] : P.dy2[ds];
    const long dyso = B.identity ? P.g[cur ^ 1] : (priv ? P.edys[i - (ne - 2)] : P.dys[ds]);
    if (i + 2 <= ne - 1) MM_TRY(side_wait_mark(i + 2, s));
    const void* ysp = B.identity ? xin : base + B.ys;
    const float* ssc = B.identity ? ones(base) : bnf(B.bs, base, 2);
    const float* ssh = B.identity ? zeros(base) : bnf(B.bs, base, 3);
    int np = launch_bn_bwd_reduce(dt(), base + P.g[cur], nullptr, bnf(B.b2, base, 2), bnf(B.b2, base, 3), base + B.y2, ysp, npix, B.C, part, s, ssc, ssh);
    MM_TRY(np);
    if (B.identity) MM_TRY(bn_backward_coefs(B.b2, params, grads, base, np, 2, 0, cnt, s));
    else MM_TRY(bn_backward_coefs_join(B.b2, B.bs, params, grads, base, np, cnt, s));
    MM_TRY(launch_bn_bwd_apply(dt(), base + P.g[cur], nullptr, bnf(B.b2, base, 2), bnf(B.b2, base, 3), base + B.y2, bnf(B.b2, base, 4), bnf(B.b2, base, 5),
                               bnf(B.b2, base, 6), base + dy2o, ysp, B.identity ? ones(base) : bnf(B.bs, base, 4),
                               B.identity ? zeros(base) : bnf(B.bs, base, 5), B.identity ? zeros(base) : bnf(B.bs, base, 6), base + dyso, npix, B.C, s,
                               ssc, ssh));
    hipStream_t wsm = wgrad_stream(s);
    MM_TRY(side_fork(s));
    WgradReduceArgs late; late.nparts = 0;
    if (i == 0 && wsm != s && !B.c2.fp8 && op_wgrad_is_stream(dt(), geom(B.c2), N, B.Hout, B.Wout, B.Hout, B.Wout, false, true))
      MM_TRY(op_run_wgrad(dt(), geom(B.c2), N, base + dy2o, B.Hout, B.Wout, nullptr, nullptr, 1, base + B.y1, B.Hout, B.Wout, bnf(B.b1, base, 2),
                          bnf(B.b1, base, 3), 1, grads + B.c2.off, wsm, reinterpret_cast<float*>(base + P.wscratch2), B.c2.wscale, &late));
    else
      MM_TRY(run_wgrad(B.c2, N, base + dy2o, B.Hout, B.Wout, nullptr, nullptr, base + B.y1, B.Hout, B.Wout, bnf(B.b1, base, 2),
                       bnf(B.b1, base, 3), grads, wsm));
    const bool pair = !B.identity && !B.c1.fp8 && !B.cs.fp8 && wgrad_pair_ok(dt(), geom(B.c1), geom(B.cs), B.Hout, B.Hin);
    if (!B.identity && !pair) MM_TRY(run_wgrad(B.cs, N, base + dyso, B.Hout, B.Wout, nullptr, nullptr, xin, B.Hin, B.Win, xs, xb, grads, wsm));
    if (i == 0 && l1_dgrad_stream()) {
      np = launch_conv3_stream_bwd(dt(), base + dy2o, base + plan_.packed + l1c2_flip * (long)esz(), base + P.da1, base + B.y1, bnf(B.b1, base, 2),
                                   bnf(B.b1, base, 3), part, N, B.Hout, s);
    } else {
      MM_TRY(run_up(B.c2, base, N, base + dy2o, B.Hout, B.Wout, base + P.da1, B.Hout, B.Wout, nullptr, nullptr, 0, nullptr, 0, s));
      np = launch_bn_bwd_reduce(dt(), base + P.da1, nullptr, bnf(B.b1, base, 2), bnf(B.b1, base, 3), base + B.y1, nullptr, npix, B.C, part, s);
    }
    MM_TRY(np);
    MM_TRY(bn_backward_coefs(B.b1, params, grads, base, np, 1, 0, cnt, s));
    MM_TRY(launch_bn_bwd_apply(dt(), base + P.da1, nullptr, bnf(B.b1, base, 2), bnf(B.b1, base, 3), base + B.y1, bnf(B.b1, base, 4),
                               bnf(B.b1, base, 5), bnf(B.b1, base, 6), base + dy1o, nullptr, nullptr, nullptr, nullptr, nullptr, npix,
                               B.C, s));
    MM_TRY(side_fork(s));
    int taken = 0;
    if (pair) {
      taken = op_run_wgrad_pair(dt(), geom(B.c1), geom(B.cs), N, base + dy1o, base + dyso, B.Hout, B.Wout, xin, B.Hin, B.Win, xs, xb, 1,
                                grads + B.c1.off, grads + B.cs.off, wsm, wscratch_, B.c1.wscale, B.cs.wscale);
      MM_TRY(taken);
      if (!taken) MM_TRY(run_wgrad(B.cs, N, base + dyso, B.Hout, B.Wout, nullptr, nullptr, xin, B.Hin, B.Win, xs, xb, grads, wsm));
    }
    if (!taken) MM_TRY(run_wgrad(B.c1, N, base + dy1o, B.Hout, B.Wout, nullptr, nullptr, xin, B.Hin, B.Win, xs, xb, grads, wsm));
    if (late.nparts > 0) MM_TRY(launch_wgrad_reduce(late, wsm));
    MM_TRY(side_mark(i));
    if (i == 0 && stem_dg_fused()) {
      stem_dy1_ = dy1o; stem_dys_ = dyso;
    } else if (B.identity)
      MM_TRY(run_up(B.c1, base, N, base + dy1o, B.Hout, B.Wout, base + P.g[cur ^ 1], B.Hin, B.Win, nullptr, nullptr, 0, nullptr, 1, s));
    else
      MM_TRY(run_up(B.c1, base, N, base + dy1o, B.Hout, B.Wout, base + P.g[cur ^ 1], B.Hin, B.Win, nullptr, nullptr, 0, nullptr, 0, s, &B.cs,
                    base + dyso));
    cur ^= 1;
  }
  if (stem_bwd_fused()) {
    const long npix = (long)N * H1 * W1;
    const Block& B0 = enc[0];
    const int np = stem_dg_fused()
        ? launch_stem_bwd_dg(base + stem_dy1_, base + stem_dys_, base + P.packed + B0.c1.packU * (long)esz(), base + P.packed + B0.cs.packU * (long)esz(),
                             base + P.y0, base + P.x_t, bnf(bn0, base, 2), bnf(bn0, base, 3), part, kPartialFloats, N, cfg.S, H1, W1, s)
        : launch_stem_bwd(dt(), base + P.g[cur], base + P.y0, base + P.x_t, bnf(bn0, base, 2), bnf(bn0, base, 3), part, kPartialFloats,
                          N, cfg.S, H1, W1, s);
    MM_TRY(np);
    const float* gsum = nullptr; double cnt = (double)npix;
    if (sync_bn_on()) {
      float* row = nullptr;
      MM_TRY(sync_rows(base, part, np, 64, s, &row, stem_bwd_part_floats()));
      gsum = row; cnt *= ar_world_;
    }
    if (side_state_ == 1 && hipStreamWaitEvent(s, gram_ev_, 0) != hipSuccess) { set_error("side stream wait failed"); return MMVAE_ERR_HIP; }
    MM_TRY(launch_stem_bwd_finalize(part, np, reinterpret_cast<const double*>(base + P.stem_R), params + stem.off, gsum, cnt,
                                    params + bn0.g_off, bnf(bn0, base, 0), bnf(bn0, base, 1), grads + bn0.g_off, grads + bn0.b_off,
                                    grads + stem.off, s));
    return side_join(s);
  }
  MM_TRY(side_wait_mark(1, s));
  const int ds = 1;
  {
    const long npix = (long)N * H1 * W1;
    int np = launch_bn_bwd_reduce(dt(), base + P.g[cur], nullptr, bnf(bn0, base, 2), bnf(bn0, base, 3), base + P.y0, nullptr, npix, 32, part, s);
    MM_TRY(np);
    MM_TRY(bn_backward_coefs(bn0, params, grads, base, np, 1, 0, (double)npix, s));
    MM_TRY(launch_bn_bwd_apply(dt(), base + P.g[cur], nullptr, bnf(bn0, base, 2), bnf(bn0, base, 3), base + P.y0, bnf(bn0, base, 4),
                               bnf(bn0, base, 5), bnf(bn0, base, 6), base + P.dy1[ds], nullptr, nullptr, nullptr, nullptr, nullptr, npix, 32, s));
    MM_TRY(side_fork(s));
// ... 159 lines not shown
  if (store8 && !tail_wg_in_reduce) { set_error("fp8 storage of the last up-block needs the fused tail backward"); return MMVAE_ERR_UNSUPPORTED; }
  if (!tail_wg_in_reduce) {
    if (tail_fwd_fused()) { set_error("decoder_bwd: the fused tail forward (no stored join) needs the fused tail backward"); return MMVAE_ERR_UNSUPPORTED; }
    WgradArgs a; std::memset(&a, 0, sizeof(a));
    a.P = d_raw; a.P_planar = 1; a.P_planes = cfg.out_ch; a.G = base + dec.back().out; a.dW = grads + tail.off; a.scratch = wscratch_;
    a.N = N; a.Hp = Sd; a.Wp = Sd; a.Ca = 16; a.Ca_valid = cfg.out_ch; a.Hg = Sd; a.Wg = Sd; a.Cb = 16; a.Cb_valid = 16;
    a.stride = 1; a.pad = 1; a.ksz = 3; a.sA = 16 * 9; a.sB = 9; a.ntaps = 9; a.scale = 1.f;
    for (int t = 0; t < 9; ++t) a.tap_off[t] = t;
    MM_TRY(side_fork(s));
    MM_TRY(launch_wgrad(dt(), a, wgrad_stream(s)));
  }
  int cur = 0;
  if (!tail_fused) {
    PackArgs pa; std::memset(&pa, 0, sizeof(pa));
    pa.src = params + tail.off; pa.dst = base + P.packed + tail_pack_d * (long)esz();
    pa.cols = 16; pa.K = 8; pa.K_valid = cfg.out_ch; pa.ntaps = 9; pa.s_col = 9; pa.s_k = 144; pa.scale = 1.f;
    for (int t = 0; t < 9; ++t) pa.tap_off[t] = t;
    GatherArgs a; std::memset(&a, 0, sizeof(a));
    a.x = d_raw; a.w = pa.dst; a.y = base + P.g[cur]; a.x_planar = 1; a.x_planes = cfg.out_ch;
    a.N = N; a.Hi = Sd; a.Wi = Sd; a.Cin = 8; a.Ho = Sd; a.Wo = Sd; a.Cout = 16; a.SI = 1; a.SO = 1;
    a.nphase = 1; a.phases[0] = Phase{0, 0, Sd, Sd, 9, 0, 0};
    for (int kh = 0; kh < 3; ++kh) for (int kw = 0; kw < 3; ++kw) a.taps[kh * 3 + kw] = Tap{1 - kh, 1 - kw};
    MM_TRY(launch_gather_gemm(dt(), dt(), a, s));
  }
  const int nd = (int)dec.size();
  auto jg_block = [&](int j) {
    if (j < 0 || j >= nd || dt() != DT_BF16 || !join_grad_) return false;
    const Block& Bj = dec[j];
    if (Bj.identity || Bj.C != 16 || Bj.c2.fp8 || Bj.cs.fp8 || Bj.c1.fp8 || (j == 0 && cfg.blocks <= 1)) return false;
    return op_bwd_fusable_jg(dt(), geom(Bj.c2), N, Bj.Hin, Bj.Win, Bj.Hout, Bj.Wout, true, false, true) &&
           op_bwd_fusable_jg(dt(), geom(Bj.cs), N, Bj.Hin, Bj.Win, Bj.Hout, Bj.Wout, false, true, false);
  };
  bool g_masked = false;
  for (int i = nd - 1; i >= 0; --i) {
    Block& B = dec[i];
    const bool jg = g_masked;
    g_masked = false;
    const long npo = (long)N * B.Hout * B.Wout, npi = (long)N * B.Hin * B.Win;
    const void* xin = i == 0 ? (cfg.blocks > 1 ? base + P.act0d : base + P.y0d) : base + dec[i - 1].out;
    const float* xs = (i == 0 && cfg.blocks <= 1) ? bnf(dbn0, base, 2) : nullptr;
    const float* xb = (i == 0 && cfg.blocks <= 1) ? bnf(dbn0, base, 3) : nullptr;
    const int ds = i & 1;
    if (i + 2 <= nd - 1) MM_TRY(side_wait_mark(i + 2, s));
    const bool from_tail = tail_fused && i == nd - 1;
    const void* ysp = B.identity ? xin : base + B.ys;
    const float* ssc = B.identity ? ones(base) : bnf(B.bs, base, 2);
    const float* ssh = B.identity ? zeros(base) : bnf(B.bs, base, 3);
    const long dyso = B.identity ? P.g[cur ^ 1] : P.dys[ds];
    if (from_tail) {
      np = launch_tail_join_bwd_reduce(dt(), d_raw, params + tail.off, cfg.out_ch, N, Sd, Sd, bnf(B.b2, base, 2), bnf(B.b2, base, 3), bnf(B.bs, base, 2),
                                       bnf(B.bs, base, 3), base + B.y2, base + B.ys, part, s, tail_wg_in_reduce ? wscratch_ : nullptr, store8 ? 1 : 0);
      if (tail_wg_in_reduce && np > 0) {
        MM_TRY(side_fork(s));
        MM_TRY(launch_tail_wgrad_finalize(wscratch_, np, grads + tail.off, wgrad_stream(s)));
      }
    } else if (jg)
      np = launch_bn_bwd_reduce(dt(), base + P.g[cur], nullptr, nullptr, nullptr, base + B.y2, ysp, npo, B.C, part, s, nullptr, nullptr);
    else
      np = launch_bn_bwd_reduce(dt(), base + P.g[cur], nullptr, bnf(B.b2, base, 2), bnf(B.b2, base, 3), base + B.y2, ysp, npo, B.C, part, s, ssc, ssh);
    MM_TRY(np);
    if (B.identity) MM_TRY(bn_backward_coefs(B.b2, params, grads, base, np, 2, 0, (double)npo, s));
    else MM_TRY(bn_backward_coefs_join(B.b2, B.bs, params, grads, base, np, (double)npo, s));
    if (from_tail && !B.identity && !B.c2.fp8 && !B.cs.fp8 && !B.c1.fp8 && B.Cin == 16 && join_bwd_stream_ok(dt(), cfg.out_ch, B.C, B.Hin, B.Hout)) {
      float* ws2 = reinterpret_cast<float*>(base + P.wscratch2);
      JoinBwdLaunch L;
      L.d_raw = d_raw; L.w_tail = params + tail.off; L.y2 = base + B.y2; L.ys = base + B.ys;
      L.ms2 = bnf(B.b2, base, 2); L.mb2 = bnf(B.b2, base, 3); L.mss = bnf(B.bs, base, 2); L.mbs = bnf(B.bs, base, 3);
      L.A2 = bnf(B.b2, base, 4); L.B2 = bnf(B.b2, base, 5); L.C2 = bnf(B.b2, base, 6);
      L.As = bnf(B.bs, base, 4); L.Bs = bnf(B.bs, base, 5); L.Cs = bnf(B.bs, base, 6);
      L.y1 = base + B.y1; L.p1s = bnf(B.b1, base, 2); L.p1b = bnf(B.b1, base, 3);
      L.wd2 = base + plan_.packed + B.c2.packD * (long)esz(); L.da1 = base + P.da1; L.part2 = ws2; L.bn_part = part;
      L.xin = xin; L.pxs = xs; L.pxb = xb; L.wds = base + plan_.packed + B.cs.packD * (long)esz(); L.gin = base + P.g[cur ^ 1];
      L.parts = ws2 + 1024L * 4096;
      L.N = N; L.f8in = store8 ? 1 : 0;
      const int nb = launch_join_bwd_stream(L, s);
      MM_TRY(nb);
      auto reduce16 = [&](const float* parts, int nparts, const ConvW& w, int ntaps) {
        WgradReduceArgs u; std::memset(&u, 0, sizeof(u));
        u.part = parts; u.dW = grads + w.off; u.Ca = w.D0; u.Cb = w.D1; u.ntaps = ntaps; u.nparts = nparts;
        u.Ca_valid = w.D0; u.Cb_valid = w.D1; u.sA = w.D1 * ntaps; u.sB = ntaps; u.scale = w.wscale;
        for (int t = 0; t < ntaps; ++t) u.tap_off[t] = t;
        return launch_wgrad_reduce(u, s);
      };
      MM_TRY(reduce16(L.part2, nb, B.c2, 16));
      MM_TRY(reduce16(L.parts, nb, B.cs, 16));
      MM_TRY(bn_backward_coefs(B.b1, params, grads, base, nb, 1, 0, (double)npi, s));
      Conv1BwdLaunch C1;
      C1.da1 = base + P.da1; C1.y1 = base + B.y1; C1.ms = bnf(B.b1, base, 2); C1.mb = bnf(B.b1, base, 3);
      C1.A = bnf(B.b1, base, 4); C1.B = bnf(B.b1, base, 5); C1.C = bnf(B.b1, base, 6);
      C1.xin = xin; C1.pxs = xs; C1.pxb = xb; C1.w1u = base + plan_.packed + B.c1.packU * (long)esz();
      C1.gin = base + P.g[cur ^ 1]; C1.part = ws2; C1.nrows = (long)N * B.Hin;
      C1.mask_out = jg_block(i - 1) ? 1 : 0;
      g_masked = C1.mask_out != 0;
      const int nb1 = launch_conv1_bwd_stream(C1, s);
      MM_TRY(nb1);
      {
        WgradReduceArgs u; std::memset(&u, 0, sizeof(u));
        u.part = ws2; u.dW = grads + B.c1.off; u.Ca = B.c1.D0; u.Cb = B.c1.D1; u.ntaps = 1; u.nparts = nb1;
        u.Ca_valid = B.c1.D0; u.Cb_valid = B.c1.D1; u.sA = B.c1.D1; u.sB = 1; u.scale = B.c1.wscale;
        MM_TRY(launch_wgrad_reduce(u, s));
      }
      MM_TRY(side_mark(i));
      cur ^= 1;
      continue;
    }
    if (store8 && i == nd - 1) { set_error("fp8 storage of the last up-block needs join_bwd_stream"); return MMVAE_ERR_UNSUPPORTED; }
    if (jg) {
    } else if (from_tail)
      MM_TRY(launch_tail_join_bwd_apply(dt(), d_raw, params + tail.off, cfg.out_ch, N, Sd, Sd, bnf(B.b2, base, 2), bnf(B.b2, base, 3), bnf(B.bs, base, 2),
                                        bnf(B.bs, base, 3), base + B.y2, bnf(B.b2, base, 4), bnf(B.b2, base, 5), bnf(B.b2, base, 6), base + P.dy2[ds],
                                        base + B.ys, bnf(B.bs, base, 4), bnf(B.bs, base, 5), bnf(B.bs, base, 6), base + P.dys[ds], s));
    else
      MM_TRY(launch_bn_bwd_apply(dt(), base + P.g[cur], nullptr, bnf(B.b2, base, 2), bnf(B.b2, base, 3), base + B.y2, bnf(B.b2, base, 4), bnf(B.b2, base, 5),
                                 bnf(B.b2, base, 6), base + P.dy2[ds], ysp, B.identity ? ones(base) : bnf(B.bs, base, 4),
                                 B.identity ? zeros(base) : bnf(B.bs, base, 5), B.identity ? zeros(base) : bnf(B.bs, base, 6), base + dyso, npo, B.C, s,
                                 ssc, ssh));
    hipStream_t wsm = wgrad_stream(s);
    MM_TRY(side_fork(s));
    bool fuse_c2 = false, fuse_cs = false;
    int np_b1 = 0;
    if (B.identity) {
      MM_TRY(run_wgrad(B.c2, N, base + P.dy2[ds], B.Hout, B.Wout, nullptr, nullptr, base + B.y1, B.Hin, B.Win, bnf(B.b1, base, 2), bnf(B.b1, base, 3),
                       grads, wsm));
      MM_TRY(run_up(B.c2, base, N, base + P.dy2[ds], B.Hout, B.Wout, base + P.da1, B.Hin, B.Win, nullptr, nullptr, 0, nullptr, 0, s));
    } else {
      fuse_c2 = !B.c2.fp8 && op_bwd_fusable(dt(), geom(B.c2), N, B.Hin, B.Win, B.Hout, B.Wout);
      fuse_cs = !B.cs.fp8 && op_bwd_fusable(dt(), geom(B.cs), N, B.Hin, B.Win, B.Hout, B.Wout) && B.C == 16;
      float* wsc2 = reinterpret_cast<float*>(base + P.wscratch2);
      if (!fuse_c2)
        MM_TRY(run_wgrad(B.c2, N, base + B.y1, B.Hin, B.Win, bnf(B.b1, base, 2), bnf(B.b1, base, 3), base + P.dy2[ds], B.Hout, B.Wout, nullptr,
                         nullptr, grads, wsm));
      if (!fuse_cs) MM_TRY(run_wgrad(B.cs, N, xin, B.Hin, B.Win, xs, xb, base + P.dys[ds], B.Hout, B.Wout, nullptr, nullptr, grads, wsm));
      if (jg && !(fuse_c2 && fuse_cs)) { set_error("decoder_bwd: the join-gradient form needs both fused passes"); return MMVAE_ERR_UNSUPPORTED; }
      if (fuse_c2) {
        const JoinGrad j2{base + B.y2, bnf(B.b2, base, 4), bnf(B.b2, base, 5), bnf(B.b2, base, 6)};
        const int rcf = op_run_bwd_fused(dt(), geom(B.c2), N, base + B.y1, B.Hin, B.Win, bnf(B.b1, base, 2), bnf(B.b1, base, 3), 1,
                                         jg ? base + P.g[cur] : base + P.dy2[ds],
                                         B.Hout, B.Wout, base + plan_.packed + B.c2.packD * (long)esz(), base + P.da1, nullptr, nullptr,
                                         grads + B.c2.off, s, wsc2, B.c2.wscale, B.C == 16 ? part : nullptr, nullptr, 1.f, jg ? &j2 : nullptr);
        if (rcf <= 0) { if (rcf == 0) set_error("decoder_bwd: fused backward of %s not taken", "conv2"); return rcf < 0 ? rcf : MMVAE_ERR_UNSUPPORTED; }
        if (B.C == 16) np_b1 = rcf;
      } else
        MM_TRY(run_down(B.c2, base, N, base + P.dy2[ds], B.Hout, B.Wout, base + P.da1, B.Hin, B.Win, nullptr, nullptr, 0, nullptr, 0, dt(), s));
    }
    np = np_b1 > 0 ? np_b1 : launch_bn_bwd_reduce(dt(), base + P.da1, nullptr, bnf(B.b1, base, 2), bnf(B.b1, base, 3), base + B.y1, nullptr, npi, B.C, part, s);
    MM_TRY(np);
    MM_TRY(bn_backward_coefs(B.b1, params, grads, base, np, 1, 0, (double)npi, s));
    MM_TRY(launch_bn_bwd_apply(dt(), base + P.da1, nullptr, bnf(B.b1, base, 2), bnf(B.b1, base, 3), base + B.y1, bnf(B.b1, base, 4),
                               bnf(B.b1, base, 5), bnf(B.b1, base, 6), base + P.dy1[ds], nullptr, nullptr, nullptr, nullptr, nullptr, npi,
                               B.C, s));
    MM_TRY(side_fork(s));
    if (!fuse_cs) MM_TRY(run_wgrad(B.c1, N, base + P.dy1[ds], B.Hin, B.Win, nullptr, nullptr, xin, B.Hin, B.Win, xs, xb, grads, wsm));
    MM_TRY(side_mark(i));
    if (B.identity)
      MM_TRY(run_up(B.c1, base, N, base + P.dy1[ds], B.Hin, B.Win, base + P.g[cur ^ 1], B.Hin, B.Win, nullptr, nullptr, 0, nullptr, 1, s));
    else if (fuse_cs) {
      const JoinGrad js{base + B.ys, bnf(B.bs, base, 4), bnf(B.bs, base, 5), bnf(B.bs, base, 6)};
      const int rcf = op_run_bwd_fused(dt(), geom(B.cs), N, xin, B.Hin, B.Win, xs, xb, 1, jg ? base + P.g[cur] : base + P.dys[ds], B.Hout, B.Wout,
                                       base + plan_.packed + B.cs.packD * (long)esz(), base + P.g[cur ^ 1], base + P.dy1[ds],
                                       base + plan_.packed + B.c1.packU * (long)esz(), grads + B.cs.off, s,
                                       reinterpret_cast<float*>(base + P.wscratch2), B.cs.wscale, nullptr, grads + B.c1.off, B.c1.wscale, jg ? &js : nullptr);
      if (rcf <= 0) { if (rcf == 0) set_error("decoder_bwd: fused backward of %s not taken", "upsample"); return rcf < 0 ? rcf : MMVAE_ERR_UNSUPPORTED; }
    } else
      MM_TRY(run_down(B.cs, base, N, base + P.dys[ds], B.Hout, B.Wout, base + P.g[cur ^ 1], B.Hin, B.Win, nullptr, nullptr, 0, nullptr, 0, dt(), s,
                      &B.c1, base + P.dy1[ds]));
    cur ^= 1;
  }
  if (dec.size() >= 2) MM_TRY(side_wait_mark(1, s));
  const int ds = 1;
  {
    const long npix = (long)N * 4;
    np = launch_bn_bwd_reduce(dt(), base + P.g[cur], nullptr, bnf(dbn0, base, 2), bnf(dbn0, base, 3), base + P.y0d, nullptr, npix, 128, part, s);
    MM_TRY(np);
    MM_TRY(bn_backward_coefs(dbn0, params, grads, base, np, 1, 0, (double)npix, s));
    MM_TRY(launch_bn_bwd_apply(dt(), base + P.g[cur], nullptr, bnf(dbn0, base, 2), bnf(dbn0, base, 3), base + P.y0d, bnf(dbn0, base, 4),
                               bnf(dbn0, base, 5), bnf(dbn0, base, 6), base + P.dy1[ds], nullptr, nullptr, nullptr, nullptr, nullptr, npix, 128, s));
    MM_TRY(side_fork(s));
    MM_TRY(run_wgrad(dstem, N, base + P.enc_t, 1, 1, nullptr, nullptr, base + P.dy1[ds], 2, 2, nullptr, nullptr, grads, wgrad_stream(s)));
    if (d_enc) {
      MM_TRY(run_down(dstem, base, N, base + P.dy1[ds], 2, 2, base + P.dh, 1, 1, nullptr, nullptr, 0, nullptr, 0, dt(), s));
      MM_TRY(launch_convert(dt(), DT_F32, base + P.dh, d_enc, (long)N * cfg.z, s));
    }
    if (!defer_join_) MM_TRY(side_join(s));
  }
  return MMVAE_OK;
}

}
```

### moving-mnist-vae_amd/csrc/vae_net.hpp

```cpp
#pragma once
#include <string>
#include <vector>

#include "comm.hpp"
#include "conv_ops.hpp"
#include "kernels.hpp"

namespace mmvae {

struct NetCfg { int in_ch, z, out_ch, S, need_logvar, dtype, blocks, fp8; };

enum EntryKind : int { EK_PARAM = 0, EK_BN_F32 = 1, EK_BN_I64 = 2 };
struct Entry { std::string name; int ndim; int shape[4]; int kind; long offset; };

struct ConvW { long off; int D0, D1, k, s, p; long packD, packU; int Hl = 0;  bool tr = false;  bool fp8 = false; float wscale = 1.f; };
struct Bn { long g_off, b_off, rm_off, rv_off; int nbt_idx; int C; long ws;  };

struct Block {
  ConvW c1, c2, cs; Bn b1, b2, bs;
  int Cin, C, Hin, Win, Hmid, Wmid, Hout, Wout;
  long y1, y2, ys, out;
  bool identity = false;
};

// ... 53 lines not shown
  int decoder_bwd(int N, const float* d_recon, const float* params, float* grads, void* ws, size_t ws_bytes, float* d_enc,
                  hipStream_t s, const GaussTail* gauss = nullptr);

 private:
  Plan plan_;
  float* wscratch_ = nullptr;
  static constexpr int kForkEvents = 192;
  hipStream_t side_ = nullptr; hipEvent_t ev_[kForkEvents] = {}; int evi_ = 0; int side_state_ = 0;
  hipStream_t wgrad_stream(hipStream_t s);
  int side_fork(hipStream_t s);
  int side_join(hipStream_t s);
  hipEvent_t gram_ev_ = nullptr;
  bool gram_ready_ = false; int gram_fwd_N_ = 0; const void* gram_fwd_ws_ = nullptr;
  hipEvent_t blk_ev_[16] = {};
  int side_mark(int slot);
  int side_wait_mark(int slot, hipStream_t s);
  int dt() const { return cfg.dtype; }
  size_t esz() const { return dtype_size(cfg.dtype); }
  ConvW add_conv(const std::string& name, int D0, int D1, int k, int s, int p, bool pack, bool transposed = false);
  void settle_fp8(ConvW& w) const;
  Bn add_bn(const std::string& prefix, int C);
  void add_entry(const std::string& name, std::initializer_list<int> shape, int kind, long off);

  int packs_enc_fwd(const float* params, char* base, hipStream_t s);
  int packs_enc_bwd(const float* params, char* base, hipStream_t s);
  int packs_dec_fwd(const float* params, char* base, hipStream_t s);
  int packs_dec_bwd(const float* params, char* base, bool need_denc, hipStream_t s);
  int frag_down(const ConvW& w) const;
  int frag_up(const ConvW& w) const;
  int pack_down(const ConvW& w, const float* params, char* base, hipStream_t s);
  int pack_up(const ConvW& w, const float* params, char* base, hipStream_t s);
  int run_down(const ConvW& w, char* base, int N, const void* L, int Hl, int Wl, void* S, int Hs, int Ws,
               const float* pro_s, const float* pro_b, int relu, float* stats, int accumulate, int out_dt, hipStream_t s,
               const ConvW* w2 = nullptr, const void* x2 = nullptr);
  int run_up(const ConvW& w, char* base, int N, const void* S, int Hs, int Ws, void* L, int Hl, int Wl,
             const float* pro_s, const float* pro_b, int relu, float* stats, int accumulate, hipStream_t s,
             const ConvW* w2 = nullptr, const void* x2 = nullptr);
  int run_wgrad(const ConvW& w, int N, const void* P, int Hs, int Ws, const float* proP_s, const float* proP_b,
                const void* G, int Hl, int Wl, const float* proG_s, const float* proG_b, float* grads, hipStream_t s);
  bool tail_fwd_fused() const;
  bool stem_bwd_fused() const;
  bool stem_dg_fused() const;
  long stem_dy1_ = 0, stem_dys_ = 0;
  bool defer_join_ = false;
  int (*ar_fn_)(float*, long long, void*, void*) = nullptr; void* ar_user_ = nullptr; int ar_world_ = 1;
  Comm* comm_ = nullptr; Comm* comm_side_ = nullptr;
  int sync_rows(char* base, const float* partials, int nparts, int width, hipStream_t s, float** out, int row_stride = 0);
 public:
  void set_defer_join(bool v) { defer_join_ = v; }
  bool join_grad_ = true;
  void set_join_grad(bool v) { join_grad_ = v; }
  typedef int (*AllReduceFn)(float* buf, long long n, void* stream, void* user);
  void set_sync_bn(AllReduceFn fn, void* user, int world) { ar_fn_ = fn; ar_user_ = user; ar_world_ = fn ? world : 1; comm_ = comm_side_ = nullptr; }
  void set_sync_bn_comm(Comm* c, Comm* side = nullptr) { comm_ = c; comm_side_ = c ? side : nullptr; ar_fn_ = nullptr; ar_user_ = nullptr; ar_world_ = c ? comm_world(c) : 1; }
  bool sync_bn_on() const { return ar_fn_ != nullptr || comm_ != nullptr; }
  int join(hipStream_t s) { return side_join(s); }
  hipStream_t side() const { return side_state_ == 1 ? side_ : nullptr; }
  hipStream_t fork(hipStream_t s) { return side_fork(s) == MMVAE_OK ? wgrad_stream(s) : s; }
 private:
  int bn_train(const Bn& bn, const float* params, float* bnbuf, long long* nbt, char* base, int nparts, double count, hipStream_t s, long part_off = 0,
               float in_scale = 1.f);
  int bn_eval(const Bn& bn, const float* params, const float* bnbuf, char* base, hipStream_t s, float in_scale = 1.f);
  int fold_bn_eval(int which, const float* params, const float* bnbuf, char* base, hipStream_t s);
  bool l1_dgrad_stream() const;
  long l1c2_flip = 0;
  bool eval_folded_ = false;
  bool store8 = false;
  float* bnf(const Bn& bn, char* base, int which) const;
  const float* ones(char* base) const { return reinterpret_cast<const float*>(base + plan_.cvec); }
  const float* zeros(char* base) const { return reinterpret_cast<const float*>(base + plan_.cvec) + 256; }
  int fill_consts(char* base, hipStream_t s);
  int bn_backward_coefs(const Bn& bn, const float* params, float* grads, char* base, int nparts, int ny, int which, double count,
                        hipStream_t s, float* dbias_conv = nullptr);
  BnBwdFinalizeArgs bwd_finalize_args(const Bn& bn, const float* params, float* grads, char* base, const float* partials, int nparts, int ny,
                                      int which, double count) const;
  int bn_backward_coefs_join(const Bn& b2, const Bn& bs, const float* params, float* grads, char* base, int nparts, double count, hipStream_t s);
};

}
```

Measured before the change: 852,300 frames/s.

## Fuse BatchNorm-backward partial sums into data-gradient conv epilogues

Adds a BnSums epilogue to the deep2 and position data-gradient convolution kernels so that, while storing dx, they also accumulate the per-channel sums that the next BatchNorm backward needs. The decoder backward then skips the separate launch_bn_bwd_reduce pass over the gradient and saved activations. It uses double-buffered partial slots so the sums for the next block survive. The cost is extra register pressure and global reads of y0/y1 inside the conv epilogue, plus a query pass to check which kernel shapes support the fusion.

Result: no change. 848,900 frames/s (-0.4%).

```diff
diff --git a/include/mmvae.h b/include/mmvae.h
--- a/include/mmvae.h
+++ b/include/mmvae.h
@@ -112,6 +112,9 @@
                      void* scratch, void* stream);
 MMVAE_API int mmvae_conv2d_dgrad(int dtype, int transposed, const void* dy, const float* weight, void* dx, int N, int H, int W, int Cin,
                        int Cout, int k, int stride, int pad, void* scratch, void* stream);
+MMVAE_API int mmvae_conv2d_dgrad_bnsums(int dtype, int transposed, const void* dy, const float* weight, void* dx, int N, int H, int W, int Cin,
+                              int Cout, int k, int stride, int pad, const void* dy2, const float* weight2, const void* y0, const float* s0,
+                              const float* b0, const void* y1, const float* s1, const float* b1, float* part, void* scratch, void* stream);
 #define MMVAE_WGRAD_SCRATCH_BYTES (64u << 20)
 MMVAE_API int mmvae_conv2d_wgrad(int dtype, int transposed, const void* x, const void* dy, float* dweight, int N, int H, int W, int Cin,
                        int Cout, int k, int stride, int pad, const float* pro_scale, const float* pro_shift, int pro_relu,
diff --git a/moving-mnist-vae_amd/_lib.py b/moving-mnist-vae_amd/_lib.py
--- a/moving-mnist-vae_amd/_lib.py
+++ b/moving-mnist-vae_amd/_lib.py
@@ -56,6 +56,8 @@
     "mmvae_adam_step_dev": (c_int, [P, P, P, P, c_int64, c_float, c_float, c_float, c_float, c_float, P, c_float, P]),
     "mmvae_conv2d_fwd": (c_int, [c_int, c_int, P, P, P, c_int, c_int, c_int, c_int, c_int, c_int, c_int, c_int, P, P, c_int, P, P, P]),
     "mmvae_conv2d_dgrad": (c_int, [c_int, c_int, P, P, P, c_int, c_int, c_int, c_int, c_int, c_int, c_int, c_int, P, P]),
+    "mmvae_conv2d_dgrad_bnsums": (c_int, [c_int, c_int, P, P, P, c_int, c_int, c_int, c_int, c_int, c_int, c_int, c_int, P, P, P, P, P, P, P, P, P,
+                                          P, P]),
     "mmvae_conv2d_wgrad": (c_int, [c_int, c_int, P, P, P, c_int, c_int, c_int, c_int, c_int, c_int, c_int, c_int, P, P, c_int, P, P]),
     "mmvae_conv2d_wgrad_pair": (c_int, [c_int, P, P, P, P, P, c_int, c_int, c_int, c_int, c_int, P, P, c_int, P, P]),
     "mmvae_rbf_kernel": (c_int, [P, P, c_int, c_int, c_int, P, P]),
diff --git a/moving-mnist-vae_amd/csrc/capi.cpp b/moving-mnist-vae_amd/csrc/capi.cpp
--- a/moving-mnist-vae_amd/csrc/capi.cpp
+++ b/moving-mnist-vae_amd/csrc/capi.cpp
@@ -346,6 +346,48 @@
   q.wfrag = op_deep2_down_ok(dt, g, Ho, Wo);
   int rc = op_pack_down(dt, g, w, scratch, S(st), 1.f, 0, q.wfrag); if (rc < 0) return rc;
   return op_run_down(dt, dt, g, scratch, N, dy, Ho, Wo, dx, H, W, nullptr, nullptr, 0, nullptr, 0, S(st), q);
+}
+int mmvae_conv2d_dgrad_bnsums(int dt, int transposed, const void* dy, const float* w, void* dx, int N, int H, int W, int Cin, int Cout, int k,
+                              int s, int p, const void* dy2, const float* w2, const void* y0, const float* s0, const float* b0, const void* y1,
+                              const float* s1, const float* b1, float* part, void* scratch, void* st) {
+  const ConvGeom g = geom_for(transposed, Cin, Cout, k, s, p);
+  const int Ho = out_size(transposed, H, k, s, p), Wo = out_size(transposed, W, k, s, p);
+  if ((dy2 != nullptr) != (w2 != nullptr) || (dy2 && transposed)) { set_error("conv2d_dgrad_bnsums: dy2 and weight2 come together, Conv2d only"); return MMVAE_ERR_ARG; }
+  if (part && (!y0 || !s0 || !b0 || (y1 && (!s1 || !b1)))) { set_error("conv2d_dgrad_bnsums: y0 / s0 / b0 (and s1 / b1 with y1) required"); return MMVAE_ERR_ARG; }
+  BnSums q; std::memset(&q, 0, sizeof(q));
+  q.y0 = y0; q.s0 = s0; q.b0 = b0; q.y1 = y1; q.s1 = y1 ? s1 : nullptr; q.b1 = y1 ? b1 : nullptr; q.part = part;
+  auto run = [&](const BnSums* bns, int* rows) -> int {
+    SecondSrc ss;
+    if (!transposed) {
+      ss.wfrag = op_deep2_up_ok(dt, g, H, W);
+      if (dy2) {
+        const ConvGeom g2 = geom_for(0, Cin, Cout, 1, s, 0);
+        char* w2p = static_cast<char*>(scratch) + numel_w(Cin, Cout, k) * (long)dtype_size(dt);
+        ss.wfrag2 = op_deep2_up_ok(dt, g2, H, W, 1);
+        int rc = op_pack_up(dt, g2, w2, w2p, S(st), 1.f, 0, ss.wfrag2); if (rc < 0) return rc;
+        ss.x2 = dy2; ss.w2 = w2p; ss.Cin2 = Cout;
+      }
+      int rc = op_pack_up(dt, g, w, scratch, S(st), 1.f, 0, ss.wfrag); if (rc < 0) return rc;
+      return op_run_up(dt, g, scratch, N, dy, Ho, Wo, dx, H, W, nullptr, nullptr, 0, nullptr, 0, S(st), ss, bns, rows);
+    }
+    ss.wfrag = op_deep2_down_ok(dt, g, Ho, Wo);
+    int rc = op_pack_down(dt, g, w, scratch, S(st), 1.f, 0, ss.wfrag); if (rc < 0) return rc;
+    return op_run_down(dt, dt, g, scratch, N, dy, Ho, Wo, dx, H, W, nullptr, nullptr, 0, nullptr, 0, S(st), ss, bns, rows);
+  };
+  if (!part) { const int rc = run(nullptr, nullptr); return rc < 0 ? rc : 0; }
+  if (!transposed && s == 1 && !dy2 && conv3_stream_ok(dt, Cin, Cout, k, s, p, H, W)) {
+    set_error("conv2d_dgrad_bnsums: this shape runs on the stream kernel (launch_conv3_stream_bwd has its own sums)"); return MMVAE_ERR_UNSUPPORTED;
+  }
+  BnSums probe = q; probe.query = 1;
+  int rows = 0;
+  int rc = run(&probe, &rows);
+  if (rc < 0) return rc;
+  if (rows <= 0) { set_error("conv2d_dgrad_bnsums: the kernel of this shape has no BatchNorm-backward sums epilogue"); return MMVAE_ERR_UNSUPPORTED; }
+  rows = 0;
+  rc = run(&q, &rows);
+  if (rc < 0) return rc;
+  if (rows <= 0) { set_error("conv2d_dgrad_bnsums: sums not taken"); return MMVAE_ERR_UNSUPPORTED; }
+  return rows;
 }
 int mmvae_conv2d_wgrad(int dt, int transposed, const void* x, const void* dy, float* dw, int N, int H, int W, int Cin, int Cout, int k,
                        int s, int p, const float* ps, const float* pb, int relu, void* scratch, void* st) {
diff --git a/moving-mnist-vae_amd/csrc/conv_deep2.inc b/moving-mnist-vae_amd/csrc/conv_deep2.inc
--- a/moving-mnist-vae_amd/csrc/conv_deep2.inc
+++ b/moving-mnist-vae_amd/csrc/conv_deep2.inc
@@ -3,7 +3,7 @@
 
 namespace mmvae {
 
-template <typename T, typename TO, int NPT, int CPT, bool ACC, bool LITE, bool F8 = false>
+template <typename T, typename TO, int NPT, int CPT, bool ACC, bool LITE, bool F8 = false, bool BNS = false>
 __device__ __forceinline__ void deep2_conv_body(const DeepArgs& a) {
   static_assert(!F8 || (sizeof(T) == 2 && !ACC), "fp8 MFMA: bf16 storage, forward convolutions");
   constexpr int VE = Elem<T>::kVec;
@@ -29,6 +29,9 @@
   const bool has_pro = a.pro_scale != nullptr, has_bias = a.bias != nullptr, has_stats = a.stats != nullptr;
   const float relu_lo = a.pro_relu ? 0.f : -__builtin_inff();
   const int HqWq = a.Hq * a.Wq;
+  constexpr bool kBns = BNS && sizeof(T) == 2 && sizeof(TO) == 2 && !F8;
+  [[maybe_unused]] const bool bns2 = a.bns.y1 != nullptr;
+  [[maybe_unused]] float bns_a = 0.f, bns_b = 0.f;
 
   const int cv = t % cin_vecs, pix0 = t / cin_vecs, PS = nthr / cin_vecs;
   for (int p = t; p < TPX; p += nthr) {
@@ -181,6 +184,41 @@
         bv[j] = has_bias ? a.bias[c0 + 8 * gq + j] : 0.f;
         st1[j] = 0.f; st2[j] = 0.f;
       }
+      bool bns_done = false;
+      if constexpr (kBns) {
+        if (!(a.bns.skip && P.ph == a.bns.skip_ph && P.pw == a.bns.skip_pw)) {
+          bns_done = true;
+          const bf16_t* __restrict__ BY0 = reinterpret_cast<const bf16_t*>(a.bns.y0);
+          const bf16_t* __restrict__ BY1 = reinterpret_cast<const bf16_t*>(a.bns.y1);
+          BnSumsCoef bc;
+          bns_load_coef(bc, a.bns, c0 + 8 * gq, bns2);
+          float bsum[3][8];
+#pragma unroll
+          for (int q = 0; q < 3; ++q)
+#pragma unroll
+            for (int j = 0; j < 8; ++j) bsum[q][j] = 0.f;
+#pragma unroll
+          for (int pt = 0; pt < NPT; ++pt) {
+            const unsigned op = sOpix[pt * 16 + r];
+            const int img = (int)(op >> 16), hq = (int)((op >> 8) & 255u), wq = (int)(op & 255u);
+            if (op != ~0u && img < nimg && hq < P.Hq && wq < P.Wq) {
+              const unsigned ob = ((((unsigned)(n0 + img) * a.Ho + (unsigned)(hq * a.SO + P.ph)) * a.Wo + (unsigned)(wq * a.SO + P.pw)) * (unsigned)a.Cout) +
+                                  (unsigned)(c0 + 8 * gq);
+              const Vec16 q0 = *reinterpret_cast<const Vec16*>(BY0 + ob);
+              Vec16 q1 = Vec16{{0, 0, 0, 0}};
+              if (bns2) q1 = *reinterpret_cast<const Vec16*>(BY1 + ob);
+              float v[8];
+#pragma unroll
+              for (int j = 0; j < 8; ++j) v[j] = acc[j >> 2][pt][j & 3] + bv[j];
+              dstore8_stored(reinterpret_cast<bf16_t*>(Y) + ob, v, ACC);
+              bns_add(bsum, v, q0, q1, bc, bns2);
+            }
+            if constexpr (NPT == 2) __builtin_amdgcn_sched_barrier(0);
+          }
+          bns_fold(bsum, r, bns2, bns_a, bns_b);
+        }
+      }
+      if (!bns_done) {
 #pragma unroll
       for (int pt = 0; pt < NPT; ++pt) {
         const unsigned op = sOpix[pt * 16 + r];
@@ -196,6 +234,7 @@
           dstore8<TO>(Y + ob, v, ACC);
         }
       }
+      }
       if (has_stats) {
 #pragma unroll
         for (int j = 0; j < 8; ++j) { st1[j] = row16_sum(st1[j]); st2[j] = row16_sum(st2[j]); }
@@ -212,12 +251,15 @@
   if (has_stats) {
     a.stats[(long)blockIdx.x * 2 * a.Cout + (long)(lane >> 5) * a.Cout + c0 + (lane & 31)] = sStat[lane];
   }
+  if constexpr (kBns) bns_store(a.bns, blockIdx.x, a.Cout, c0 + 8 * gq, r, bns2, bns_a, bns_b);
 }
 
 template <typename T, typename TO, int NPT, int CPT, bool ACC>
 __global__ __launch_bounds__(512, 2) void deep2_conv_kernel(DeepArgs a) { deep2_conv_body<T, TO, NPT, CPT, ACC, false>(a); }
 template <typename T, typename TO, int NPT, int CPT, bool ACC>
 __global__ __launch_bounds__(512, 3) void deep2_conv_lite_kernel(DeepArgs a) { deep2_conv_body<T, TO, NPT, CPT, ACC, true>(a); }
+template <typename T, typename TO, int NPT, int CPT, bool ACC>
+__global__ __launch_bounds__(512, 2) void deep2_conv_bns_kernel(DeepArgs a) { deep2_conv_body<T, TO, NPT, CPT, ACC, false, false, true>(a); }
 template <typename T, typename TO, int NPT, int CPT, bool ACC>
 __global__ __launch_bounds__(512, 2) void deep2_conv_f8_kernel(DeepArgs a) { deep2_conv_body<T, TO, NPT, CPT, false, false, true>(a); }
 template <typename T, typename TO, int NPT, int CPT, bool ACC>
@@ -227,6 +269,7 @@
 static int launch_deep2_t(const DeepArgs& a, int dt, int gx, hipStream_t s) {
   const size_t lds = deep2_conv_lds_bytes(a, dt);
   dim3 grid(gx, a.Cout / (32 * a.nw)), block(64 * a.nw);
+  if (a.bns.part && (sizeof(T) != 2 || sizeof(TO) != 2 || a.fp8 || a.bias || a.stats || a.nw >= 4)) { set_error("deep2_conv: BatchNorm-backward sums need the bf16 data-gradient form of the 1-2 wave blocks"); return MMVAE_ERR_UNSUPPORTED; }
 #define MMVAE_D2K(K_, N_, C_, A_) do { \
     static bool attr_set = false; \
     if (!attr_set) { \
@@ -235,7 +278,11 @@
       attr_set = true; \
     } \
     hipLaunchKernelGGL((K_<T, TO, N_, C_, A_>), grid, block, lds, s, a); } while (0)
-#define MMVAE_D2(N_, C_, A_) do { if (a.nw >= 4) MMVAE_D2K(deep2_conv_lite_kernel, N_, C_, A_); else MMVAE_D2K(deep2_conv_kernel, N_, C_, A_); } while (0)
+#define MMVAE_D2(N_, C_, A_) do { \
+    if constexpr (sizeof(T) == 2 && sizeof(TO) == 2) { \
+      if (a.bns.part) { MMVAE_D2K(deep2_conv_bns_kernel, N_, C_, A_); break; } \
+    } \
+    if (a.nw >= 4) MMVAE_D2K(deep2_conv_lite_kernel, N_, C_, A_); else MMVAE_D2K(deep2_conv_kernel, N_, C_, A_); } while (0)
 #define MMVAE_D2C(N_, C_) do { if (a.accumulate) MMVAE_D2(N_, C_, true); else MMVAE_D2(N_, C_, false); } while (0)
 #define MMVAE_D2N(N_) do { \
     constexpr int kC0 = sizeof(T) == 2 ? 1 : 2;       \
diff --git a/moving-mnist-vae_amd/csrc/conv_gemm.hip b/moving-mnist-vae_amd/csrc/conv_gemm.hip
--- a/moving-mnist-vae_amd/csrc/conv_gemm.hip
+++ b/moving-mnist-vae_amd/csrc/conv_gemm.hip
@@ -383,7 +383,7 @@
   if (fp8 && cpt > 4) return false;
   return deep2_lds_for(dt, Cin, Cout, hw, Hi * Wi, ntaps_all, npt_min, fp8) <= 150 * 1024;
 }
-static int try_deep2(int dt, int out_dt, const GatherArgs& a, hipStream_t s) {
+static int try_deep2(int dt, int out_dt, const GatherArgs& a, hipStream_t s, const BnSums* bns = nullptr, bool dry = false) {
   if (a.x_planar || a.y_planes || a.x2) return 0;
   if (a.fp8 && (!a.wfrag || a.accumulate || dt != DT_BF16 || out_dt != DT_BF16)) return 0;
   int Hq = 0, Wq = 0, ntaps_all = 0;
@@ -431,10 +431,12 @@
   if (b.ipt > a.N) b.ipt = a.N;
   b.ntiles = (a.N + b.ipt - 1) / b.ipt;
   int gx = b.ntiles < kGatherMaxGridX ? b.ntiles : kGatherMaxGridX;
+  if (dry) return b.nw < 4 ? 1 : 0;
+  if (bns) b.bns = *bns;
   return launch_deep2_conv(dt, out_dt, b, gx, s);
 }
 
-static int try_pos(int dt, int out_dt, const GatherArgs& a, hipStream_t s) {
+static int try_pos(int dt, int out_dt, const GatherArgs& a, hipStream_t s, const BnSums* bns = nullptr, bool dry = false) {
   if (dt != DT_BF16 || out_dt != DT_BF16 || !a.wfrag || a.fp8 || a.gup == 0) return 0;
   if (a.x_planar || a.y_planes || a.x2 || a.bias || a.Hi != a.Wi || a.Ho != a.Wo || a.Cout % 32 != 0) return 0;
   const int up = a.gup == 2 ? 1 : 0;
@@ -447,11 +449,19 @@
   b.stats = a.stats; b.accumulate = a.accumulate; b.N = a.N; b.Cout = a.Cout;
   b.nw = a.Cout / 32 < 8 ? a.Cout / 32 : 8;
   if ((a.Cout / 32) % b.nw != 0 || (64 * b.nw) % (a.Cin / 8) != 0) return 0;
+  if (dry) return 1;
+  if (bns) b.bns = *bns;
   return launch_pos_conv(a.gk, a.gs, a.gp, up, a.Hi, a.Ho, a.Cin, b, s);
 }
 
-static int launch_x2_separately(int dt, int out_dt, const GatherArgs& a, hipStream_t s) {
-  GatherArgs b; memset(&b, 0, sizeof(b));
+static bool bns_kernel_takes(int dt, int out_dt, const GatherArgs& a) {
+  if (dt != DT_BF16 || out_dt != DT_BF16 || !a.wfrag || a.fp8 || a.x2 || a.bias || a.stats || a.x_planar || a.y_planes) return false;
+  if (a.Cin % 8 != 0 || a.Cout % 32 != 0 || a.nphase < 1 || a.nphase > kMaxPhases) return false;
+  return try_pos(dt, out_dt, a, nullptr, nullptr, true) > 0 || try_deep2(dt, out_dt, a, nullptr, nullptr, true) > 0;
+}
+
+static int x2_launch_args(const GatherArgs& a, GatherArgs& b) {
+  memset(&b, 0, sizeof(b));
   int Hq = 0, Wq = 0;
   for (int p = 0; p < a.nphase; ++p) if (a.phases[p].ph == a.x2_ph && a.phases[p].pw == a.x2_pw) { Hq = a.phases[p].Hq; Wq = a.phases[p].Wq; }
   if (Hq <= 0) { set_error("gather_gemm: the second source's phase (%d,%d) is not part of the launch", a.x2_ph, a.x2_pw); return MMVAE_ERR_ARG; }
@@ -459,11 +469,23 @@
   b.N = a.N; b.Hi = Hq; b.Wi = Wq; b.Cin = a.Cin2; b.Ho = a.Ho; b.Wo = a.Wo; b.Cout = a.Cout; b.SI = 1; b.SO = a.SO;
   b.nphase = 1; b.phases[0] = Phase{a.x2_ph, a.x2_pw, Hq, Wq, 1, 0, 0}; b.taps[0] = Tap{0, 0};
   b.gk = 1; b.gs = a.SO; b.gp = 0; b.gup = 2;
-  return launch_gather_gemm(dt, out_dt, b, s);
-}
-
-int launch_gather_gemm(int dt, int out_dt, GatherArgs a, hipStream_t s) {
+  return MMVAE_OK;
+}
+
+int launch_gather_gemm(int dt, int out_dt, GatherArgs a, hipStream_t s, const BnSums* bns, int* bns_rows) {
   const int VE = dt == DT_F32 ? 4 : 8;
+  if (bns_rows) *bns_rows = 0;
+  if (bns && bns_rows && bns->query) {
+    bool yes;
+    if (a.x2) {
+      GatherArgs m = a; m.x2 = nullptr; m.w2 = nullptr; m.Cin2 = 0; m.wfrag2 = 0;
+      GatherArgs x;
+      yes = (a.wfrag || a.wfrag2) && x2_launch_args(a, x) == MMVAE_OK && bns_kernel_takes(dt, out_dt, m) && bns_kernel_takes(dt, out_dt, x);
+    } else yes = bns_kernel_takes(dt, out_dt, a);
+    *bns_rows = yes ? 1 : 0;
+    return MMVAE_OK;
+  }
+  if (bns && (!bns_rows || !bns->part)) bns = nullptr;
   note_launch_bytes((double)a.N * ((double)a.Hi * a.Wi * (a.x_planar ? a.x_planes : a.Cin) * (a.x_planar == 1 ? 4 : dtype_size(dt)) +
                                    (double)a.Ho * a.Wo * (a.y_planes > 0 ? a.y_planes : a.Cout) * (a.y_planes > 0 ? 4 : dtype_size(out_dt)) +
                                    (a.x2 ? (double)a.phases[0].Hq * a.phases[0].Wq * a.Cin2 * dtype_size(dt) : 0.0)));
@@ -479,10 +501,27 @@
     int rc = (!a.wfrag && !a.wfrag2) ? try_patch(dt, out_dt, a, s) : 0;
     if (rc != 0) return rc;
     GatherArgs m = a; m.x2 = nullptr; m.w2 = nullptr; m.Cin2 = 0; m.wfrag2 = 0;
-    rc = launch_gather_gemm(dt, out_dt, m, s);
+    GatherArgs x;
+    rc = x2_launch_args(a, x);
     if (rc < 0) return rc;
-    const int rc2 = launch_x2_separately(dt, out_dt, a, s);
-    return rc2 < 0 ? rc2 : rc;
+    const bool both = bns && bns_kernel_takes(dt, out_dt, m) && bns_kernel_takes(dt, out_dt, x);
+    BnSums b1, b2;
+    int r1 = 0, r2 = 0;
+    if (both) {
+      b1 = *bns; b1.skip = 1; b1.skip_ph = a.x2_ph; b1.skip_pw = a.x2_pw;
+      b2 = *bns; b2.skip = 0;
+    }
+    const bool first_sums = both && m.nphase > 1;
+    rc = launch_gather_gemm(dt, out_dt, m, s, first_sums ? &b1 : nullptr, &r1);
+    if (rc < 0) return rc;
+    if (both) b2.part += (long)r1 * (bns->y1 ? 3 : 2) * a.Cout;
+    const int rc2 = launch_gather_gemm(dt, out_dt, x, s, both ? &b2 : nullptr, &r2);
+    if (rc2 < 0) return rc2;
+    if (both) {
+      if ((first_sums && r1 <= 0) || r2 <= 0) { set_error("gather_gemm: the two-launch form lost its BatchNorm-backward sums (%d, %d rows)", r1, r2); return MMVAE_ERR_UNSUPPORTED; }
+      *bns_rows = r1 + r2;
+    }
+    return rc;
   }
   if (a.Cin % VE != 0 || a.Cout % 4 != 0 || a.nphase < 1 || a.nphase > kMaxPhases) {
     set_error("gather_gemm: unsupported Cin=%d Cout=%d nphase=%d", a.Cin, a.Cout, a.nphase);
@@ -502,10 +541,11 @@
   if (max_tiles <= 0) return 1;
   const int rcp = a.wfrag ? 0 : try_patch(dt, out_dt, a, s);
   if (rcp != 0) return rcp;
-  const int rcq = try_pos(dt, out_dt, a, s);
-  if (rcq != 0) return rcq;
-  const int rcd2 = try_deep2(dt, out_dt, a, s);
-  if (rcd2 != 0) return rcd2;
+  if (bns && !bns_kernel_takes(dt, out_dt, a)) bns = nullptr;
+  const int rcq = try_pos(dt, out_dt, a, s, bns);
+  if (rcq != 0) { if (bns && rcq > 0) *bns_rows = rcq; return rcq; }
+  const int rcd2 = try_deep2(dt, out_dt, a, s, bns);
+  if (rcd2 != 0) { if (bns && rcd2 > 0) *bns_rows = rcd2; return rcd2; }
   if (a.wfrag) { set_error("gather_gemm: fragment-major weights (Cin=%d Cout=%d) need the deep2 kernel, which does not take this launch", a.Cin, a.Cout); return MMVAE_ERR_UNSUPPORTED; }
   {
     constexpr int g3_maxk = 160;
diff --git a/moving-mnist-vae_amd/csrc/conv_ops.cpp b/moving-mnist-vae_amd/csrc/conv_ops.cpp
--- a/moving-mnist-vae_amd/csrc/conv_ops.cpp
+++ b/moving-mnist-vae_amd/csrc/conv_ops.cpp
@@ -88,8 +88,10 @@
 }
 
 int op_run_down(int dt, int out_dt, const ConvGeom& g, const void* packed, int N, const void* L, int Hl, int Wl, void* S, int Hs, int Ws,
-                const float* pro_s, const float* pro_b, int relu, float* stats, int accumulate, hipStream_t s, const SecondSrc& x2) {
+                const float* pro_s, const float* pro_b, int relu, float* stats, int accumulate, hipStream_t s, const SecondSrc& x2,
+                const BnSums* bns, int* bns_rows) {
   GatherArgs a; std::memset(&a, 0, sizeof(a));
+  if (bns_rows) *bns_rows = 0;
   if (g.k * g.k > kMaxTaps) { set_error("run_down: k=%d too large", g.k); return MMVAE_ERR_UNSUPPORTED; }
   if (x2.x2) { a.x2 = x2.x2; a.w2 = x2.w2; a.Cin2 = x2.Cin2; a.x2_ph = 0; a.x2_pw = 0; }
   a.fp8 = x2.fp8; a.wfrag = x2.wfrag; a.wfrag2 = x2.wfrag2;
@@ -101,11 +103,13 @@
   a.phases[0] = Phase{0, 0, Hs, Ws, g.k * g.k, 0, 0};
   for (int kh = 0; kh < g.k; ++kh)
     for (int kw = 0; kw < g.k; ++kw) a.taps[kh * g.k + kw] = Tap{kh - g.p, kw - g.p};
-  return launch_gather_gemm(dt, out_dt, a, s);
+  return launch_gather_gemm(dt, out_dt, a, s, bns, bns_rows);
 }
 
 int op_run_up(int dt, const ConvGeom& g, const void* packed, int N, const void* S, int Hs, int Ws, void* L, int Hl, int Wl,
-              const float* pro_s, const float* pro_b, int relu, float* stats, int accumulate, hipStream_t s, const SecondSrc& x2) {
+              const float* pro_s, const float* pro_b, int relu, float* stats, int accumulate, hipStream_t s, const SecondSrc& x2,
+              const BnSums* bns, int* bns_rows) {
+  if (bns_rows) *bns_rows = 0;
   if (g.s > 2 || g.k * g.k > kMaxTaps) { set_error("run_up: k=%d s=%d unsupported", g.k, g.s); return MMVAE_ERR_UNSUPPORTED; }
   GatherArgs a; std::memset(&a, 0, sizeof(a));
   if (x2.x2) { a.x2 = x2.x2; a.w2 = x2.w2; a.Cin2 = x2.Cin2; a.x2_ph = 0; a.x2_pw = 0; }
@@ -129,7 +133,7 @@
     off += (long)g.D1 * ph[i].ntaps * g.D0;
   }
   if (a.nphase == 0) return 1;
-  return launch_gather_gemm(dt, dt, a, s);
+  return launch_gather_gemm(dt, dt, a, s, bns, bns_rows);
 }
 
 int op_run_wgrad(int dt, const ConvGeom& g, int N, const void* P, int Hs, int Ws, const float* proP_s, const float* proP_b, int proP_relu,
diff --git a/moving-mnist-vae_amd/csrc/conv_ops.hpp b/moving-mnist-vae_amd/csrc/conv_ops.hpp
--- a/moving-mnist-vae_amd/csrc/conv_ops.hpp
+++ b/moving-mnist-vae_amd/csrc/conv_ops.hpp
@@ -16,9 +16,11 @@
   int wfrag = 0, wfrag2 = 0;
 };
 int op_run_down(int dt, int out_dt, const ConvGeom& g, const void* packed, int N, const void* L, int Hl, int Wl, void* S, int Hs, int Ws,
-                const float* pro_s, const float* pro_b, int relu, float* stats, int accumulate, hipStream_t s, const SecondSrc& x2 = SecondSrc());
+                const float* pro_s, const float* pro_b, int relu, float* stats, int accumulate, hipStream_t s, const SecondSrc& x2 = SecondSrc(),
+                const BnSums* bns = nullptr, int* bns_rows = nullptr);
 int op_run_up(int dt, const ConvGeom& g, const void* packed, int N, const void* S, int Hs, int Ws, void* L, int Hl, int Wl,
-              const float* pro_s, const float* pro_b, int relu, float* stats, int accumulate, hipStream_t s, const SecondSrc& x2 = SecondSrc());
+              const float* pro_s, const float* pro_b, int relu, float* stats, int accumulate, hipStream_t s, const SecondSrc& x2 = SecondSrc(),
+              const BnSums* bns = nullptr, int* bns_rows = nullptr);
 int op_run_wgrad(int dt, const ConvGeom& g, int N, const void* P, int Hs, int Ws, const float* proP_s, const float* proP_b, int proP_relu,
                  const void* G, int Hl, int Wl, const float* proG_s, const float* proG_b, int proG_relu, float* dW, hipStream_t s,
                  float* scratch = nullptr, float scale = 1.f, WgradReduceArgs* defer = nullptr);
diff --git a/moving-mnist-vae_amd/csrc/conv_pos.inc b/moving-mnist-vae_amd/csrc/conv_pos.inc
--- a/moving-mnist-vae_amd/csrc/conv_pos.inc
+++ b/moving-mnist-vae_amd/csrc/conv_pos.inc
@@ -57,7 +57,7 @@
   static constexpr int first_of(int u) { for (int w = 0; w < W; ++w) if (tab.it[w].u >= u) return w; return W; }
 };
 
-template <int K, int S, int P, bool UP, int HI, int HO, int CIN, int IG, int NB, int RB>
+template <int K, int S, int P, bool UP, int HI, int HO, int CIN, int IG, int NB, int RB, bool BNS>
 __global__ __launch_bounds__(512, 2) void pos_conv_kernel(PosArgs a) {
   using TP = PosTaps<K, S, P, UP>;
   constexpr int NPH1 = UP ? S : 1;
@@ -77,6 +77,10 @@
   const bf16_t* __restrict__ X = reinterpret_cast<const bf16_t*>(a.x);
   bf16_t* __restrict__ Y = reinterpret_cast<bf16_t*>(a.y);
   const bool has_pro = a.pro_scale != nullptr, has_stats = a.stats != nullptr, accum = a.accumulate != 0;
+  [[maybe_unused]] const bool bns2 = a.bns.y1 != nullptr;
+  [[maybe_unused]] const bf16_t* __restrict__ BY0 = reinterpret_cast<const bf16_t*>(a.bns.y0);
+  [[maybe_unused]] const bf16_t* __restrict__ BY1 = reinterpret_cast<const bf16_t*>(a.bns.y1);
+  [[maybe_unused]] float bns_a = 0.f, bns_b = 0.f;
   const float relu_lo = a.pro_relu ? 0.f : -__builtin_inff();
   const char* lb[IG];
 #pragma unroll
@@ -173,6 +177,37 @@
         float st1[8], st2[8];
 #pragma unroll
         for (int j = 0; j < 8; ++j) { st1[j] = 0.f; st2[j] = 0.f; }
+        bool bns_done = false;
+        if constexpr (BNS) {
+        if (!(a.bns.skip && ph == a.bns.skip_ph && pw == a.bns.skip_pw)) {
+          bns_done = true;
+          BnSumsCoef bc;
+          bns_load_coef(bc, a.bns, c0 + 8 * gq, bns2);
+          float bsum[3][8];
+#pragma unroll
+          for (int q = 0; q < 3; ++q)
+#pragma unroll
+            for (int j = 0; j < 8; ++j) bsum[q][j] = 0.f;
+          static_for<0, NCF>([&](auto CF) {
+            constexpr int cf = decltype(CF)::value, pos = cf / IG, ig = cf % IG;
+            constexpr int ho = (pos / HQ) * SO + ph, wo = (pos % HQ) * SO + pw;
+            if (ig * 16 + r < nimg) {
+              const unsigned ob = ((unsigned)(n0 + ig * 16 + r) * (HO * HO) + (unsigned)(ho * HO + wo)) * (unsigned)a.Cout + (unsigned)(c0 + 8 * gq);
+              const Vec16 q0 = *reinterpret_cast<const Vec16*>(BY0 + ob);
+              Vec16 q1 = Vec16{{0, 0, 0, 0}};
+              if (bns2) q1 = *reinterpret_cast<const Vec16*>(BY1 + ob);
+              float v[8];
+#pragma unroll
+              for (int j = 0; j < 8; ++j) v[j] = acc[j >> 2][cf][j & 3];
+              dstore8_stored(Y + ob, v, accum);
+              bns_add(bsum, v, q0, q1, bc, bns2);
+            }
+            if constexpr (NCF > 8) __builtin_amdgcn_sched_barrier(0);
+          });
+          bns_fold(bsum, r, bns2, bns_a, bns_b);
+        }
+        }
+        if (!bns_done)
         static_for<0, NCF>([&](auto CF) {
           constexpr int cf = decltype(CF)::value, pos = cf / IG, ig = cf % IG;
           constexpr int ho = (pos / HQ) * SO + ph, wo = (pos % HQ) * SO + pw;
@@ -201,6 +236,7 @@
     });
   }
   if (has_stats) a.stats[(long)blockIdx.x * 2 * a.Cout + (long)(lane >> 5) * a.Cout + c0 + (lane & 31)] = sStat[lane];
+  if constexpr (BNS) bns_store(a.bns, blockIdx.x, a.Cout, c0 + 8 * gq, r, bns2, bns_a, bns_b);
 }
 
 #ifndef POS_NB16
@@ -215,12 +251,12 @@
 #ifndef POS_RB8
 #define POS_RB8 6
 #endif
-template <int K, int S, int P, bool UP, int HI, int HO, int CIN, int IG>
-static int pos_launch(const PosArgs& a, hipStream_t s) {
+template <int K, int S, int P, bool UP, int HI, int HO, int CIN, int IG, bool BNS>
+static int pos_launch_t(const PosArgs& a, hipStream_t s) {
   constexpr int IP = HI * HI * CIN * 2 + 32;
   constexpr int HQ = UP ? HO / S : HO, NCF = HQ * HQ * IG;
   constexpr int NB = NCF > 8 ? POS_NB16 : POS_NB8, RB = NCF > 8 ? POS_RB16 : POS_RB8;
-  auto* kern = &pos_conv_kernel<K, S, P, UP, HI, HO, CIN, IG, NB, RB>;
+  auto* kern = &pos_conv_kernel<K, S, P, UP, HI, HO, CIN, IG, NB, RB, BNS>;
   const size_t lds = (size_t)16 * IG * IP + (size_t)a.nw * 256;
   static bool attr_set = false;
   if (!attr_set) {
@@ -237,5 +273,10 @@
   const int rc = check_launch("pos_conv");
   return rc ? rc : gx;
 }
-
-}
+template <int K, int S, int P, bool UP, int HI, int HO, int CIN, int IG>
+static int pos_launch(const PosArgs& a, hipStream_t s) {
+  if (a.bns.part && a.stats) { set_error("pos_conv: BatchNorm-backward sums are a data-gradient epilogue (no forward statistics)"); return MMVAE_ERR_UNSUPPORTED; }
+  return a.bns.part ? pos_launch_t<K, S, P, UP, HI, HO, CIN, IG, true>(a, s) : pos_launch_t<K, S, P, UP, HI, HO, CIN, IG, false>(a, s);
+}
+
+}
diff --git a/moving-mnist-vae_amd/csrc/kernels.hpp b/moving-mnist-vae_amd/csrc/kernels.hpp
--- a/moving-mnist-vae_amd/csrc/kernels.hpp
+++ b/moving-mnist-vae_amd/csrc/kernels.hpp
@@ -28,7 +28,14 @@
   int gk, gs, gp, gup;
 };
 bool deep2_shape_ok(int dt, int Cin, int Cout, int Hq, int Wq, int Hi, int Wi, int ntaps_all, int fp8 = 0);
-int launch_gather_gemm(int dt, int out_dt, GatherArgs a, hipStream_t s);
+struct BnSums {
+  const void* y0; const float* s0; const float* b0;
+  const void* y1; const float* s1; const float* b1;
+  float* part;
+  int skip, skip_ph, skip_pw;
+  int query;
+};
+int launch_gather_gemm(int dt, int out_dt, GatherArgs a, hipStream_t s, const BnSums* bns = nullptr, int* bns_rows = nullptr);
 constexpr int kGatherMaxGridX = 1024;
 
 struct WgradArgs {
@@ -136,6 +143,7 @@
   int fp8;
   int nw, cpt_log2;
   int wfrag;
+  BnSums bns;
 };
 size_t deep2_conv_lds_bytes(const DeepArgs& a, int dt);
 int launch_deep2_conv(int dt, int out_dt, const DeepArgs& a, int gx, hipStream_t s);
@@ -146,6 +154,7 @@
   int N, Cout;
   int nw;
   int ntiles;
+  BnSums bns;
 };
 int launch_pos_conv(int K, int S, int P, int up, int HI, int HO, int CIN, const PosArgs& a, hipStream_t s);
 bool pos_conv_takes(int K, int S, int P, int up, int HI, int HO, int CIN);
diff --git a/moving-mnist-vae_amd/csrc/tile_common.hpp b/moving-mnist-vae_amd/csrc/tile_common.hpp
--- a/moving-mnist-vae_amd/csrc/tile_common.hpp
+++ b/moving-mnist-vae_amd/csrc/tile_common.hpp
@@ -82,6 +82,65 @@
   o.x = pack2_bf16(f[0], f[1]); o.y = pack2_bf16(f[2], f[3]); o.z = pack2_bf16(f[4], f[5]); o.w = pack2_bf16(f[6], f[7]);
   *reinterpret_cast<uint4*>(p) = o;
 }
+__device__ __forceinline__ float row16_sum(float v);
+__device__ __forceinline__ void dstore8_stored(bf16_t* p, float* v, bool acc) {
+  if (acc) {
+    const uint4 e = *reinterpret_cast<const uint4*>(p);
+    const unsigned w[4] = {e.x, e.y, e.z, e.w};
+#pragma unroll
+    for (int j = 0; j < 4; ++j) { v[2 * j] += __uint_as_float(w[j] << 16); v[2 * j + 1] += __uint_as_float(w[j] & 0xffff0000u); }
+  }
+  uint4 o;
+  o.x = pack2_bf16(v[0], v[1]); o.y = pack2_bf16(v[2], v[3]); o.z = pack2_bf16(v[4], v[5]); o.w = pack2_bf16(v[6], v[7]);
+  *reinterpret_cast<uint4*>(p) = o;
+  const unsigned w[4] = {o.x, o.y, o.z, o.w};
+#pragma unroll
+  for (int j = 0; j < 4; ++j) { v[2 * j] = __uint_as_float(w[j] << 16); v[2 * j + 1] = __uint_as_float(w[j] & 0xffff0000u); }
+}
+struct BnSumsCoef { float s0[8], b0[8], s1[8], b1[8]; };
+__device__ __forceinline__ void bns_load_coef(BnSumsCoef& c, const BnSums& b, int ch, bool two) {
+#pragma unroll
+  for (int j = 0; j < 8; j += 4) {
+    const float4 s0 = *reinterpret_cast<const float4*>(b.s0 + ch + j), b0 = *reinterpret_cast<const float4*>(b.b0 + ch + j);
+    const float4 s1 = two ? *reinterpret_cast<const float4*>(b.s1 + ch + j) : make_float4(0.f, 0.f, 0.f, 0.f);
+    const float4 b1 = two ? *reinterpret_cast<const float4*>(b.b1 + ch + j) : make_float4(0.f, 0.f, 0.f, 0.f);
+    c.s0[j] = s0.x; c.s0[j + 1] = s0.y; c.s0[j + 2] = s0.z; c.s0[j + 3] = s0.w;
+    c.b0[j] = b0.x; c.b0[j + 1] = b0.y; c.b0[j + 2] = b0.z; c.b0[j + 3] = b0.w;
+    c.s1[j] = s1.x; c.s1[j + 1] = s1.y; c.s1[j + 2] = s1.z; c.s1[j + 3] = s1.w;
+    c.b1[j] = b1.x; c.b1[j + 1] = b1.y; c.b1[j + 2] = b1.z; c.b1[j + 3] = b1.w;
+  }
+}
+__device__ __forceinline__ void bns_add(float (&sum)[3][8], const float* g, const Vec16& q0, const Vec16& q1, const BnSumsCoef& c, bool two) {
+  float a0[8], a1[8];
+  Elem<bf16_t>::unpack(q0, a0);
+  Elem<bf16_t>::unpack(q1, a1);
+#pragma unroll
+  for (int j = 0; j < 8; ++j) {
+    float x = a0[j] * c.s0[j] + c.b0[j];
+    if (two) x += a1[j] * c.s1[j] + c.b1[j];
+    const float gg = x > 0.f ? g[j] : 0.f;
+    sum[0][j] += gg;
+    sum[1][j] += gg * a0[j];
+    sum[2][j] += gg * a1[j];
+  }
+}
+__device__ __forceinline__ void bns_fold(float (&sum)[3][8], int r, bool two, float& tot_a, float& tot_b) {
+  float pa = 0.f, pb = 0.f;
+#pragma unroll
+  for (int j = 0; j < 8; ++j) {
+    const float t0 = row16_sum(sum[0][j]), t1 = row16_sum(sum[1][j]);
+    pa = r == j ? t0 : pa;
+    pa = r == 8 + j ? t1 : pa;
+    if (two) { const float t2 = row16_sum(sum[2][j]); pb = r == j ? t2 : pb; }
+  }
+  tot_a += pa; tot_b += pb;
+}
+__device__ __forceinline__ void bns_store(const BnSums& b, long row, int C, int ch8, int r, bool two, float tot_a, float tot_b) {
+  const int ny1 = two ? 3 : 2;
+  float* p = b.part + row * ny1 * C + ch8 + (r & 7);
+  p[(long)(r >> 3) * C] = tot_a;
+  if (two && r < 8) p[2L * C] = tot_b;
+}
 __device__ __forceinline__ float row16_sum(float v) {
   v += __builtin_bit_cast(float, __builtin_amdgcn_mov_dpp(__builtin_bit_cast(int, v), 0x128, 0xf, 0xf, true));
   v += __builtin_bit_cast(float, __builtin_amdgcn_mov_dpp(__builtin_bit_cast(int, v), 0x124, 0xf, 0xf, true));
diff --git a/moving-mnist-vae_amd/csrc/vae_net.cpp b/moving-mnist-vae_amd/csrc/vae_net.cpp
--- a/moving-mnist-vae_amd/csrc/vae_net.cpp
+++ b/moving-mnist-vae_amd/csrc/vae_net.cpp
@@ -229,23 +229,35 @@
 }
 int Net::run_down(const ConvW& w, char* base, int N, const void* L, int Hl, int Wl, void* S, int Hs, int Ws,
                   const float* pro_s, const float* pro_b, int relu, float* stats, int accumulate, int out_dt, hipStream_t s,
-                  const ConvW* w2, const void* x2) {
+                  const ConvW* w2, const void* x2, const BnSums* bns, int* bns_rows) {
   SecondSrc q;
   if (w2) { q.x2 = x2; q.w2 = base + plan_.packed + w2->packU * (long)esz(); q.Cin2 = w2->D0; }
   q.fp8 = (w.fp8 && !w.tr) ? 1 : 0;
   q.wfrag = frag_down(w); q.wfrag2 = w2 ? frag_up(*w2) : 0;
   return op_run_down(dt(), out_dt, geom(w), base + plan_.packed + w.packD * (long)esz(), N, L, Hl, Wl, S, Hs, Ws, pro_s, pro_b, relu,
-                     stats, accumulate, s, q);
+                     stats, accumulate, s, q, bns, bns_rows);
 }
 int Net::run_up(const ConvW& w, char* base, int N, const void* S, int Hs, int Ws, void* L, int Hl, int Wl,
                 const float* pro_s, const float* pro_b, int relu, float* stats, int accumulate, hipStream_t s,
-                const ConvW* w2, const void* x2) {
+                const ConvW* w2, const void* x2, const BnSums* bns, int* bns_rows) {
   SecondSrc q;
   if (w2) { q.x2 = x2; q.w2 = base + plan_.packed + w2->packU * (long)esz(); q.Cin2 = w2->D0; }
   q.fp8 = (w.fp8 && w.tr) ? 1 : 0;
   q.wfrag = frag_up(w); q.wfrag2 = w2 ? frag_up(*w2) : 0;
   return op_run_up(dt(), geom(w), base + plan_.packed + w.packU * (long)esz(), N, S, Hs, Ws, L, Hl, Wl, pro_s, pro_b, relu, stats,
-                   accumulate, s, q);
+                   accumulate, s, q, bns, bns_rows);
+}
+BnSums Net::bn_sums(char* base, const Bn& b0, const void* y0, float* part) const {
+  BnSums q; std::memset(&q, 0, sizeof(q));
+  q.y0 = y0; q.s0 = bnf(b0, base, 2); q.b0 = bnf(b0, base, 3); q.part = part;
+  return q;
+}
+BnSums Net::bn_sums_join(char* base, const Block& B, const void* xin, float* part) const {
+  BnSums q = bn_sums(base, B.b2, base + B.y2, part);
+  q.y1 = B.identity ? xin : base + B.ys;
+  q.s1 = B.identity ? ones(base) : bnf(B.bs, base, 2);
+  q.b1 = B.identity ? zeros(base) : bnf(B.bs, base, 3);
+  return q;
 }
 hipStream_t Net::wgrad_stream(hipStream_t s) {
   if (side_state_ == 0) {
@@ -381,8 +393,8 @@
   return a;
 }
 int Net::bn_backward_coefs(const Bn& bn, const float* params, float* grads, char* base, int nparts, int ny, int which, double count,
-                           hipStream_t s, float* dbias_conv) {
-  const float* part = reinterpret_cast<const float*>(base + plan_.partials);
+                           hipStream_t s, float* dbias_conv, long part_off) {
+  const float* part = reinterpret_cast<const float*>(base + plan_.partials) + part_off;
   BnBwdFinalizeArgs l = bwd_finalize_args(bn, params, grads, base, part, nparts, ny, which, count);
   if (!sync_bn_on()) l.dbias_conv = dbias_conv;
   MM_TRY(launch_bn_bwd_finalize(l, s));
@@ -395,8 +407,8 @@
   return launch_bn_bwd_finalize(g, s);
 }
 int Net::bn_backward_coefs_join(const Bn& b2, const Bn& bs, const float* params, float* grads, char* base, int nparts, double count,
-                                hipStream_t s) {
-  const float* part = reinterpret_cast<const float*>(base + plan_.partials);
+                                hipStream_t s, long part_off) {
+  const float* part = reinterpret_cast<const float*>(base + plan_.partials) + part_off;
   MM_TRY(launch_bn_bwd_finalize2(bwd_finalize_args(b2, params, grads, base, part, nparts, 2, 0, count),
                                  bwd_finalize_args(bs, params, grads, base, part, nparts, 2, 1, count), s));
   if (!sync_bn_on()) return MMVAE_OK;
@@ -633,6 +645,8 @@
   }
   int cur = 0;
   const int ne = (int)enc.size();
+  float* part2 = part + kPartialFloats;
+  int join_rows = 0;
   for (int i = ne - 1; i >= 0; --i) {
     Block& B = enc[i];
     const long npix = (long)N * B.Hout * B.Wout;
@@ -648,10 +662,13 @@
     const void* ysp = B.identity ? xin : base + B.ys;
     const float* ssc = B.identity ? ones(base) : bnf(B.bs, base, 2);
     const float* ssh = B.identity ? zeros(base) : bnf(B.bs, base, 3);
-    int np = launch_bn_bwd_reduce(dt(), base + P.g[cur], nullptr, bnf(B.b2, base, 2), bnf(B.b2, base, 3), base + B.y2, ysp, npix, B.C, part, s, ssc, ssh);
-    MM_TRY(np);
-    if (B.identity) MM_TRY(bn_backward_coefs(B.b2, params, grads, base, np, 2, 0, cnt, s));
-    else MM_TRY(bn_backward_coefs_join(B.b2, B.bs, params, grads, base, np, cnt, s));
+    const long joff = join_rows > 0 ? kPartialFloats : 0;
+    int np = join_rows > 0 ? join_rows
+                           : launch_bn_bwd_reduce(dt(), base + P.g[cur], nullptr, bnf(B.b2, base, 2), bnf(B.b2, base, 3), base + B.y2, ysp, npix, B.C, part, s, ssc, ssh);
+    MM_TRY(np);
+    join_rows = 0;
+    if (B.identity) MM_TRY(bn_backward_coefs(B.b2, params, grads, base, np, 2, 0, cnt, s, nullptr, joff));
+    else MM_TRY(bn_backward_coefs_join(B.b2, B.bs, params, grads, base, np, cnt, s, joff));
     MM_TRY(launch_bn_bwd_apply(dt(), base + P.g[cur], nullptr, bnf(B.b2, base, 2), bnf(B.b2, base, 3), base + B.y2, bnf(B.b2, base, 4), bnf(B.b2, base, 5),
                                bnf(B.b2, base, 6), base + dy2o, ysp, B.identity ? ones(base) : bnf(B.bs, base, 4),
                                B.identity ? zeros(base) : bnf(B.bs, base, 5), B.identity ? zeros(base) : bnf(B.bs, base, 6), base + dyso, npix, B.C, s,
@@ -671,8 +688,11 @@
       np = launch_conv3_stream_bwd(dt(), base + dy2o, base + plan_.packed + l1c2_flip * (long)esz(), base + P.da1, base + B.y1, bnf(B.b1, base, 2),
                                    bnf(B.b1, base, 3), part, N, B.Hout, s);
     } else {
-      MM_TRY(run_up(B.c2, base, N, base + dy2o, B.Hout, B.Wout, base + P.da1, B.Hout, B.Wout, nullptr, nullptr, 0, nullptr, 0, s));
-      np = launch_bn_bwd_reduce(dt(), base + P.da1, nullptr, bnf(B.b1, base, 2), bnf(B.b1, base, 3), base + B.y1, nullptr, npix, B.C, part, s);
+      const BnSums q1 = bn_sums(base, B.b1, base + B.y1, part);
+      int r1 = 0;
+      MM_TRY(run_up(B.c2, base, N, base + dy2o, B.Hout, B.Wout, base + P.da1, B.Hout, B.Wout, nullptr, nullptr, 0, nullptr, 0, s, nullptr, nullptr,
+                    B.Hout <= 4 ? &q1 : nullptr, &r1));
+      np = r1 > 0 ? r1 : launch_bn_bwd_reduce(dt(), base + P.da1, nullptr, bnf(B.b1, base, 2), bnf(B.b1, base, 3), base + B.y1, nullptr, npix, B.C, part, s);
     }
     MM_TRY(np);
     MM_TRY(bn_backward_coefs(B.b1, params, grads, base, np, 1, 0, cnt, s));
@@ -692,11 +712,17 @@
     MM_TRY(side_mark(i));
     if (i == 0 && stem_dg_fused()) {
       stem_dy1_ = dy1o; stem_dys_ = dyso;
-    } else if (B.identity)
-      MM_TRY(run_up(B.c1, base, N, base + dy1o, B.Hout, B.Wout, base + P.g[cur ^ 1], B.Hin, B.Win, nullptr, nullptr, 0, nullptr, 1, s));
-    else
-      MM_TRY(run_up(B.c1, base, N, base + dy1o, B.Hout, B.Wout, base + P.g[cur ^ 1], B.Hin, B.Win, nullptr, nullptr, 0, nullptr, 0, s, &B.cs,
-                    base + dyso));
+    } else {
+      BnSums qn; std::memset(&qn, 0, sizeof(qn));
+      const bool join_sums = false;
+      if (i > 0 && join_sums) qn = bn_sums_join(base, enc[i - 1], i - 1 == 0 ? base + P.y0 : base + enc[i - 2].out, part2);
+      if (B.identity)
+        MM_TRY(run_up(B.c1, base, N, base + dy1o, B.Hout, B.Wout, base + P.g[cur ^ 1], B.Hin, B.Win, nullptr, nullptr, 0, nullptr, 1, s, nullptr, nullptr,
+                      qn.part ? &qn : nullptr, &join_rows));
+      else
+        MM_TRY(run_up(B.c1, base, N, base + dy1o, B.Hout, B.Wout, base + P.g[cur ^ 1], B.Hin, B.Win, nullptr, nullptr, 0, nullptr, 0, s, &B.cs,
+                      base + dyso, qn.part ? &qn : nullptr, &join_rows));
+    }
     cur ^= 1;
   }
   if (stem_bwd_fused()) {
@@ -922,6 +948,8 @@
            op_bwd_fusable_jg(dt(), geom(Bj.cs), N, Bj.Hin, Bj.Win, Bj.Hout, Bj.Wout, false, true, false);
   };
   bool g_masked = false;
+  float* part2 = part + kPartialFloats;
+  int next_rows = 0;
   for (int i = nd - 1; i >= 0; --i) {
     Block& B = dec[i];
     const bool jg = g_masked;
@@ -946,11 +974,15 @@
       }
     } else if (jg)
       np = launch_bn_bwd_reduce(dt(), base + P.g[cur], nullptr, nullptr, nullptr, base + B.y2, ysp, npo, B.C, part, s, nullptr, nullptr);
+    else if (next_rows > 0)
+      np = next_rows;
     else
       np = launch_bn_bwd_reduce(dt(), base + P.g[cur], nullptr, bnf(B.b2, base, 2), bnf(B.b2, base, 3), base + B.y2, ysp, npo, B.C, part, s, ssc, ssh);
     MM_TRY(np);
-    if (B.identity) MM_TRY(bn_backward_coefs(B.b2, params, grads, base, np, 2, 0, (double)npo, s));
-    else MM_TRY(bn_backward_coefs_join(B.b2, B.bs, params, grads, base, np, (double)npo, s));
+    const long joff = (!from_tail && !jg && next_rows > 0) ? kPartialFloats : 0;
+    next_rows = 0;
+    if (B.identity) MM_TRY(bn_backward_coefs(B.b2, params, grads, base, np, 2, 0, (double)npo, s, nullptr, joff));
+    else MM_TRY(bn_backward_coefs_join(B.b2, B.bs, params, grads, base, np, (double)npo, s, joff));
     if (from_tail && !B.identity && !B.c2.fp8 && !B.cs.fp8 && !B.c1.fp8 && B.Cin == 16 && join_bwd_stream_ok(dt(), cfg.out_ch, B.C, B.Hin, B.Hout)) {
       float* ws2 = reinterpret_cast<float*>(base + P.wscratch2);
       JoinBwdLaunch L;
@@ -1009,10 +1041,12 @@
     MM_TRY(side_fork(s));
     bool fuse_c2 = false, fuse_cs = false;
     int np_b1 = 0;
+    const BnSums q1 = bn_sums(base, B.b1, base + B.y1, part);
     if (B.identity) {
       MM_TRY(run_wgrad(B.c2, N, base + P.dy2[ds], B.Hout, B.Wout, nullptr, nullptr, base + B.y1, B.Hin, B.Win, bnf(B.b1, base, 2), bnf(B.b1, base, 3),
                        grads, wsm));
-      MM_TRY(run_up(B.c2, base, N, base + P.dy2[ds], B.Hout, B.Wout, base + P.da1, B.Hin, B.Win, nullptr, nullptr, 0, nullptr, 0, s));
+      MM_TRY(run_up(B.c2, base, N, base + P.dy2[ds], B.Hout, B.Wout, base + P.da1, B.Hin, B.Win, nullptr, nullptr, 0, nullptr, 0, s, nullptr, nullptr,
+                    &q1, &np_b1));
     } else {
       fuse_c2 = !B.c2.fp8 && op_bwd_fusable(dt(), geom(B.c2), N, B.Hin, B.Win, B.Hout, B.Wout);
       fuse_cs = !B.cs.fp8 && op_bwd_fusable(dt(), geom(B.cs), N, B.Hin, B.Win, B.Hout, B.Wout) && B.C == 16;
@@ -1031,7 +1065,8 @@
         if (rcf <= 0) { if (rcf == 0) set_error("decoder_bwd: fused backward of %s not taken", "conv2"); return rcf < 0 ? rcf : MMVAE_ERR_UNSUPPORTED; }
         if (B.C == 16) np_b1 = rcf;
       } else
-        MM_TRY(run_down(B.c2, base, N, base + P.dy2[ds], B.Hout, B.Wout, base + P.da1, B.Hin, B.Win, nullptr, nullptr, 0, nullptr, 0, dt(), s));
+        MM_TRY(run_down(B.c2, base, N, base + P.dy2[ds], B.Hout, B.Wout, base + P.da1, B.Hin, B.Win, nullptr, nullptr, 0, nullptr, 0, dt(), s,
+                        nullptr, nullptr, &q1, &np_b1));
     }
     np = np_b1 > 0 ? np_b1 : launch_bn_bwd_reduce(dt(), base + P.da1, nullptr, bnf(B.b1, base, 2), bnf(B.b1, base, 3), base + B.y1, nullptr, npi, B.C, part, s);
     MM_TRY(np);
@@ -1042,8 +1077,13 @@
     MM_TRY(side_fork(s));
     if (!fuse_cs) MM_TRY(run_wgrad(B.c1, N, base + P.dy1[ds], B.Hin, B.Win, nullptr, nullptr, xin, B.Hin, B.Win, xs, xb, grads, wsm));
     MM_TRY(side_mark(i));
+    BnSums qn; std::memset(&qn, 0, sizeof(qn));
+    if (B.Hin < 8) {}
+    else if (i > 0) qn = bn_sums_join(base, dec[i - 1], i - 1 == 0 ? (cfg.blocks > 1 ? base + P.act0d : base + P.y0d) : base + dec[i - 2].out, part2);
+    else qn = bn_sums(base, dbn0, base + P.y0d, part2);
     if (B.identity)
-      MM_TRY(run_up(B.c1, base, N, base + P.dy1[ds], B.Hin, B.Win, base + P.g[cur ^ 1], B.Hin, B.Win, nullptr, nullptr, 0, nullptr, 1, s));
+      MM_TRY(run_up(B.c1, base, N, base + P.dy1[ds], B.Hin, B.Win, base + P.g[cur ^ 1], B.Hin, B.Win, nullptr, nullptr, 0, nullptr, 1, s, nullptr, nullptr,
+                    qn.part ? &qn : nullptr, &next_rows));
     else if (fuse_cs) {
       const JoinGrad js{base + B.ys, bnf(B.bs, base, 4), bnf(B.bs, base, 5), bnf(B.bs, base, 6)};
       const int rcf = op_run_bwd_fused(dt(), geom(B.cs), N, xin, B.Hin, B.Win, xs, xb, 1, jg ? base + P.g[cur] : base + P.dys[ds], B.Hout, B.Wout,
@@ -1053,16 +1093,17 @@
       if (rcf <= 0) { if (rcf == 0) set_error("decoder_bwd: fused backward of %s not taken", "upsample"); return rcf < 0 ? rcf : MMVAE_ERR_UNSUPPORTED; }
     } else
       MM_TRY(run_down(B.cs, base, N, base + P.dys[ds], B.Hout, B.Wout, base + P.g[cur ^ 1], B.Hin, B.Win, nullptr, nullptr, 0, nullptr, 0, dt(), s,
-                      &B.c1, base + P.dy1[ds]));
+                      &B.c1, base + P.dy1[ds], qn.part ? &qn : nullptr, &next_rows));
     cur ^= 1;
   }
   if (dec.size() >= 2) MM_TRY(side_wait_mark(1, s));
   const int ds = 1;
   {
     const long npix = (long)N * 4;
-    np = launch_bn_bwd_reduce(dt(), base + P.g[cur], nullptr, bnf(dbn0, base, 2), bnf(dbn0, base, 3), base + P.y0d, nullptr, npix, 128, part, s);
-    MM_TRY(np);
-    MM_TRY(bn_backward_coefs(dbn0, params, grads, base, np, 1, 0, (double)npix, s));
+    np = next_rows > 0 ? next_rows
+                       : launch_bn_bwd_reduce(dt(), base + P.g[cur], nullptr, bnf(dbn0, base, 2), bnf(dbn0, base, 3), base + P.y0d, nullptr, npix, 128, part, s);
+    MM_TRY(np);
+    MM_TRY(bn_backward_coefs(dbn0, params, grads, base, np, 1, 0, (double)npix, s, nullptr, next_rows > 0 ? kPartialFloats : 0));
     MM_TRY(launch_bn_bwd_apply(dt(), base + P.g[cur], nullptr, bnf(dbn0, base, 2), bnf(dbn0, base, 3), base + P.y0d, bnf(dbn0, base, 4),
                                bnf(dbn0, base, 5), bnf(dbn0, base, 6), base + P.dy1[ds], nullptr, nullptr, nullptr, nullptr, nullptr, npix, 128, s));
     MM_TRY(side_fork(s));
diff --git a/moving-mnist-vae_amd/csrc/vae_net.hpp b/moving-mnist-vae_amd/csrc/vae_net.hpp
--- a/moving-mnist-vae_amd/csrc/vae_net.hpp
+++ b/moving-mnist-vae_amd/csrc/vae_net.hpp
@@ -109,10 +109,10 @@
   int pack_up(const ConvW& w, const float* params, char* base, hipStream_t s);
   int run_down(const ConvW& w, char* base, int N, const void* L, int Hl, int Wl, void* S, int Hs, int Ws,
                const float* pro_s, const float* pro_b, int relu, float* stats, int accumulate, int out_dt, hipStream_t s,
-               const ConvW* w2 = nullptr, const void* x2 = nullptr);
+               const ConvW* w2 = nullptr, const void* x2 = nullptr, const BnSums* bns = nullptr, int* bns_rows = nullptr);
   int run_up(const ConvW& w, char* base, int N, const void* S, int Hs, int Ws, void* L, int Hl, int Wl,
              const float* pro_s, const float* pro_b, int relu, float* stats, int accumulate, hipStream_t s,
-             const ConvW* w2 = nullptr, const void* x2 = nullptr);
+             const ConvW* w2 = nullptr, const void* x2 = nullptr, const BnSums* bns = nullptr, int* bns_rows = nullptr);
   int run_wgrad(const ConvW& w, int N, const void* P, int Hs, int Ws, const float* proP_s, const float* proP_b,
                 const void* G, int Hl, int Wl, const float* proG_s, const float* proG_b, float* grads, hipStream_t s);
   bool tail_fwd_fused() const;
@@ -148,10 +148,13 @@
   const float* zeros(char* base) const { return reinterpret_cast<const float*>(base + plan_.cvec) + 256; }
   int fill_consts(char* base, hipStream_t s);
   int bn_backward_coefs(const Bn& bn, const float* params, float* grads, char* base, int nparts, int ny, int which, double count,
-                        hipStream_t s, float* dbias_conv = nullptr);
+                        hipStream_t s, float* dbias_conv = nullptr, long part_off = 0);
   BnBwdFinalizeArgs bwd_finalize_args(const Bn& bn, const float* params, float* grads, char* base, const float* partials, int nparts, int ny,
                                       int which, double count) const;
-  int bn_backward_coefs_join(const Bn& b2, const Bn& bs, const float* params, float* grads, char* base, int nparts, double count, hipStream_t s);
+  int bn_backward_coefs_join(const Bn& b2, const Bn& bs, const float* params, float* grads, char* base, int nparts, double count, hipStream_t s,
+                             long part_off = 0);
+  BnSums bn_sums(char* base, const Bn& b0, const void* y0, float* part) const;
+  BnSums bn_sums_join(char* base, const Block& B, const void* xin, float* part) const;
 };
 
 }
```
